# syzhang092218-source/dgppo

Measured on AMD Instinct MI355X. Metric: env-steps/sec whole node, LidarSpread n=8 4096 envs, 1/2/4/8 GPUs, higher is better.
Workload: dtype f32

## Files before the change

dgppo_amd/csrc/attn.hip:

```cpp
#include "nn_attn.h"

static int32_t attn_check(const dgppo_env_cfg* cfg, int F, int H, int Kp, int G, AttnArgs& a) {
  int32_t rc = dgppo_validate_cfg(cfg);
  if (rc) return rc;
  a.t = make_topo(*cfg);
  DGPPO_REQUIRE(F >= 1 && F <= 64 && H >= 1 && H <= 8, "attn: bad F=%d H=%d", F, H);
  DGPPO_REQUIRE(Kp >= F + H * (F + 4) + 1, "attn: Kp=%d too small", Kp);
  DGPPO_REQUIRE(G >= 0, "attn: G < 0");
  a.F = F; a.H = H; a.Kp = Kp; a.G = G;
  return 0;
}

enum class AttnFamily { SLOT8, BD, MFMA, VALU, TILED };
size_t attn_image_bytes(const Topo& t, int F, int H, bool bwd) {
  if (bwd)
    return sizeof(float) * ((size_t)t.Ns * (F + 1) + (size_t)t.n * H * (F + 1) + (size_t)t.n * t.S * 4 + 2 * (size_t)t.n * t.S * H +
                            (size_t)t.n * H * (F + 5));
  return sizeof(float) * ((size_t)t.Ns * (F + 1) + (size_t)t.n * H * (F + 1) + (size_t)t.n * t.S * 5 + (size_t)t.n * t.S * H);
}
static AttnFamily attn_family(const Topo& t, int F, int H, int Kp, bool bwd, bool dXa) {
  int PS = 0;
  bool hits = false;
  if (attn_image_bytes(t, F, H, bwd) > 64 * 1024) return AttnFamily::TILED;
  if ((Kp & 3) == 0 && attn_slot8_shape(t, F, H) && !(bwd && dXa)) return AttnFamily::SLOT8;
// ... 26 lines not shown
}
static void attn_set_bwd(AttnArgs& a, const float* dzcat, const float* attn, const float* qt, const float* Xa, const float* Xo,
                         const float* efeat, float* dqt, float* dXa, float* dXo) {
  a.dzcat = dzcat; a.attn = (float*)attn; a.qt = qt; a.Xa = Xa; a.Xo = Xo; a.efeat = efeat; a.dqt = dqt; a.dXa = dXa; a.dXo = dXo;
}

extern "C" int32_t dgppo_attn_fwd(const dgppo_env_cfg* cfg, int32_t F, int32_t H, int32_t Kp, const float* qt,
                                  const float* Xa, const float* Xo, const float* efeat, const float* emask, float* zcat,
                                  float* attn, int32_t G, void* stream) {
  AttnArgs a{};
  int32_t rc = attn_check(cfg, F, H, Kp, G, a);
  if (rc) return rc;
  if (G == 0) return 0;
  DGPPO_REQUIRE(qt && Xa && efeat && emask && zcat, "attn_fwd: NULL operand");
  DGPPO_REQUIRE(a.t.Ns == a.t.n || Xo, "attn_fwd: Xo is NULL");
  attn_set_fwd(a, qt, Xa, Xo, efeat, emask, zcat, attn);
  return attn_launch(attn_family(a.t, F, H, Kp, false, false), a, stream, false, "attn_fwd");
}

extern "C" int32_t dgppo_attn_bwd(const dgppo_env_cfg* cfg, int32_t F, int32_t H, int32_t Kp, const float* dzcat,
                                  const float* attn, const float* qt, const float* Xa, const float* Xo,
                                  const float* efeat, float* dqt, float* dXa, float* dXo, int32_t relu_xo, int32_t G,
                                  void* stream) {
  AttnArgs a{};
  int32_t rc = attn_check(cfg, F, H, Kp, G, a);
  if (rc) return rc;
  if (G == 0) return 0;
  DGPPO_REQUIRE(dzcat && attn && qt && Xa && efeat && dqt, "attn_bwd: NULL operand");
  DGPPO_REQUIRE(a.t.Ns == a.t.n || Xo, "attn_bwd: Xo is NULL");
  DGPPO_REQUIRE(!(dXo && !dXa), "attn_bwd: dXo needs dXa");
  attn_set_bwd(a, dzcat, attn, qt, Xa, Xo, efeat, dqt, dXa, dXo);
  const AttnFamily fam = attn_family(a.t, F, H, Kp, true, dXa != nullptr);
  a.relu_xo = (relu_xo && dXo && fam == AttnFamily::BD) ? 1 : 0;
  rc = attn_launch(fam, a, stream, true, "attn_bwd");
  if (rc) return rc;
  if (relu_xo && dXo && !a.relu_xo)
    return dgppo_relu_bwd(dXo, Xo, (int64_t)G * (a.t.Ns - a.t.n) * F, stream);
  return 0;
}

static bool attn_xo_ok(const Topo& t, int F, int H, int Kp) {
  return t.Ns > t.n && attn_family(t, F, H, Kp, true, true) == AttnFamily::BD;
}
extern "C" int32_t dgppo_attn_xo_supported(const dgppo_env_cfg* cfg, int32_t F, int32_t H, int32_t Kp) {
  AttnArgs a{};
  if (attn_check(cfg, F, H, Kp, 0, a)) return 0;
  return attn_xo_ok(a.t, F, H, Kp) ? 1 : 0;
}
static int32_t attn_set_xo(AttnArgs& a, const float* Xo_raw, const float* Wo, int ldwo, const float* bo, const char* who) {
  DGPPO_REQUIRE(attn_xo_ok(a.t, a.F, a.H, a.Kp), "%s: no fused kernel for this topology (ask dgppo_attn_xo_supported)", who);
  a.Xo_raw = Xo_raw; a.Wo = Wo; a.ldwo = ldwo; a.bo = bo;
  return 0;
}
extern "C" int32_t dgppo_attn_fwd_xo(const dgppo_env_cfg* cfg, int32_t F, int32_t H, int32_t Kp, const float* qt, const float* Xa,
                                     const float* Xo_raw, const float* Wo, int32_t ldwo, const float* bo, const float* efeat,
                                     const float* emask, float* zcat, float* attn, int32_t G, void* stream) {
  AttnArgs a{};
  int32_t rc = attn_check(cfg, F, H, Kp, G, a);
  if (rc) return rc;
  if (G == 0) return 0;
  DGPPO_REQUIRE(qt && Xa && Xo_raw && Wo && bo && efeat && emask && zcat, "attn_fwd_xo: NULL operand");
  DGPPO_REQUIRE(ldwo >= 32, "attn_fwd_xo: ldwo=%d < 32", ldwo);
  rc = attn_set_xo(a, Xo_raw, Wo, ldwo, bo, "attn_fwd_xo");
  if (rc) return rc;
  attn_set_fwd(a, qt, Xa, nullptr, efeat, emask, zcat, attn);
  return attn_launch(AttnFamily::BD, a, stream, false, "attn_fwd_xo");
}
extern "C" int32_t dgppo_attn_bwd_xo(const dgppo_env_cfg* cfg, int32_t F, int32_t H, int32_t Kp, const float* dzcat,
                                     const float* attn, const float* qt, const float* Xa, const float* Xo_raw, const float* Wo,
                                     int32_t ldwo, const float* bo, const float* efeat, float* dqt, float* dXa, float* dXo,
                                     int32_t relu_xo, int32_t G, void* stream) {
  AttnArgs a{};
  int32_t rc = attn_check(cfg, F, H, Kp, G, a);
  if (rc) return rc;
  if (G == 0) return 0;
  DGPPO_REQUIRE(dzcat && attn && qt && Xa && Xo_raw && Wo && bo && efeat && dqt, "attn_bwd_xo: NULL operand");
  DGPPO_REQUIRE(ldwo >= 32, "attn_bwd_xo: ldwo=%d < 32", ldwo);
  DGPPO_REQUIRE(!(dXo && !dXa), "attn_bwd_xo: dXo needs dXa");
  rc = attn_set_xo(a, Xo_raw, Wo, ldwo, bo, "attn_bwd_xo");
  if (rc) return rc;
  attn_set_bwd(a, dzcat, attn, qt, Xa, nullptr, efeat, dqt, dXa, dXo);
  a.relu_xo = (relu_xo && dXo) ? 1 : 0;
  return attn_launch(AttnFamily::BD, a, stream, true, "attn_bwd_xo");
}

static bool attn_rows_ok(const dgppo_env_cfg& c, const Topo& t, int F, int H, int Kp) {
  return attn_slot8_rows_ok(c, t, F, H) && attn_family(t, F, H, Kp, false, false) == AttnFamily::SLOT8 &&
         attn_family(t, F, H, Kp, true, false) == AttnFamily::SLOT8;
}
extern "C" int32_t dgppo_attn_rows_supported(const dgppo_env_cfg* cfg, int32_t F, int32_t H) {
  AttnArgs a{};
  const int Kp = (F + H * (F + 4) + 1 + 3) / 4 * 4;
  if (F < 1 || H < 1 || attn_check(cfg, F, H, Kp, 0, a)) return 0;
  return attn_rows_ok(*cfg, a.t, F, H, Kp) ? 1 : 0;
}
extern "C" int32_t dgppo_attn_fwd_rows(const dgppo_env_cfg* cfg, int32_t F, int32_t H, int32_t Kp, const float* qt,
                                       const float* Xa, const float* Xo, const float* emask, float* zcat, float* attn,
                                       int32_t G, void* stream) {
  AttnArgs a{};
  int32_t rc = attn_check(cfg, F, H, Kp, G, a);
  if (rc) return rc;
  DGPPO_REQUIRE(attn_rows_ok(*cfg, a.t, F, H, Kp), "attn_fwd_rows: no such kernel for this configuration (ask dgppo_attn_rows_supported)");
  if (G == 0) return 0;
  DGPPO_REQUIRE(qt && Xa && emask && zcat, "attn_fwd_rows: NULL operand");
  DGPPO_REQUIRE(a.t.Ns == a.t.n || Xo, "attn_fwd_rows: Xo is NULL");
  attn_set_fwd(a, qt, Xa, Xo, nullptr, emask, zcat, attn);
  return attn_launch(AttnFamily::SLOT8, a, stream, false, "attn_fwd_rows");
}
extern "C" int32_t dgppo_attn_bwd_rows(const dgppo_env_cfg* cfg, int32_t F, int32_t H, int32_t Kp, const float* dzcat,
                                       const float* attn, const float* qt, const float* emask, const float* Xa, const float* Xo,
                                       float* dqt, int32_t G, void* stream) {
  AttnArgs a{};
  int32_t rc = attn_check(cfg, F, H, Kp, G, a);
  if (rc) return rc;
  DGPPO_REQUIRE(attn_rows_ok(*cfg, a.t, F, H, Kp), "attn_bwd_rows: no such kernel for this configuration (ask dgppo_attn_rows_supported)");
  if (G == 0) return 0;
  DGPPO_REQUIRE(dzcat && Xa && dqt, "attn_bwd_rows: NULL operand");
  DGPPO_REQUIRE(attn || (qt && emask), "attn_bwd_rows: without attn the weights need qt and emask");
  DGPPO_REQUIRE(a.t.Ns == a.t.n || Xo, "attn_bwd_rows: Xo is NULL");
  attn_set_bwd(a, dzcat, attn, qt, Xa, Xo, nullptr, dqt, nullptr, nullptr);
  a.emask = emask;
  return attn_launch(AttnFamily::SLOT8, a, stream, true, "attn_bwd_rows");
}

extern "C" int64_t dgppo_attn_xo_workspace_bytes(int32_t G) { return G < 0 ? 0 : (int64_t)G * ABD_DW_STRIDE * (int64_t)sizeof(float); }
extern "C" int32_t dgppo_attn_bwd_xo_dw(const dgppo_env_cfg* cfg, int32_t F, int32_t H, int32_t Kp, const float* dzcat,
                                        const float* attn, const float* qt, const float* Xa, const float* Xo_raw, const float* Wo,
                                        int32_t ldwo, const float* bo, const float* efeat, float* dqt, float* dXa, float* dWo,
                                        int32_t lddwo, float* dbo, float* workspace, int64_t workspace_bytes, int32_t G,
                                        void* stream) {
  AttnArgs a{};
  int32_t rc = attn_check(cfg, F, H, Kp, G, a);
  if (rc) return rc;
  if (G == 0) return 0;
  DGPPO_REQUIRE(dzcat && attn && qt && Xa && Xo_raw && Wo && bo && efeat && dqt && dXa && dWo && dbo && workspace,
                "attn_bwd_xo_dw: NULL operand");
  DGPPO_REQUIRE(ldwo >= 32 && lddwo >= 32, "attn_bwd_xo_dw: ldwo=%d lddwo=%d < 32", ldwo, lddwo);
  DGPPO_REQUIRE(workspace_bytes >= dgppo_attn_xo_workspace_bytes(G) && (reinterpret_cast<uintptr_t>(workspace) & 15) == 0,
                "attn_bwd_xo_dw: workspace too small or not 16-byte aligned");
  rc = attn_set_xo(a, Xo_raw, Wo, ldwo, bo, "attn_bwd_xo_dw");
  if (rc) return rc;
  attn_set_bwd(a, dzcat, attn, qt, Xa, nullptr, efeat, dqt, dXa, nullptr);
  a.relu_xo = 1;
  a.dwo_slab = workspace;
  const bool launched = launch_attn_bd(a, (hipStream_t)stream, true);
  DGPPO_REQUIRE(launched, "attn_bwd_xo_dw: dispatch failed");
  launch_attn_xo_dw_reduce(workspace, G, dWo, lddwo, dbo, (hipStream_t)stream);
  DGPPO_LAUNCH_CHECK();
  return 0;
}
```

dgppo_amd/csrc/attn_bd.hip:

```cpp
#include "nn_attn.h"

#ifdef DGPPO_STAMPS
__device__ unsigned long long g_astamps[32];
#define ASTAMP(i) do { if (blockIdx.x == 0 && threadIdx.x == 0) g_astamps[i] = __builtin_amdgcn_s_memtime(); } while (0)
extern "C" int32_t dgppo_debug_stamps_attn(unsigned long long* out) {
  return (int32_t)hipMemcpyFromSymbol(out, HIP_SYMBOL(g_astamps), sizeof(unsigned long long) * 32);
}
#else
#define ASTAMP(i)
#endif

#define ABD_XL 36
#define ABD_DZL 40
__device__ inline f32x4g mfma4(float a_, float b_, f32x4g c_) { return __builtin_amdgcn_mfma_f32_4x4x1f32(a_, b_, c_, 0, 0, 0); }
__device__ inline const float* f4e(const float4& v) { return reinterpret_cast<const float*>(&v); }

__device__ inline int opaque_zero(int bits) {
  asm("v_and_b32 %0, 0, %0" : "+v"(bits));
  return bits;
}
__device__ inline int f4bits(const float4& v) { return __float_as_int(v.x) | __float_as_int(v.y) | __float_as_int(v.z) | __float_as_int(v.w); }

template <int PS, bool HITS> struct AbdLds {
  static constexpr int NSP = PS * 8, PC = NSP + (HITS ? 8 : 0), PL = PC + 4;
// ... 44 lines not shown
      v[ct] = __builtin_amdgcn_mfma_f32_16x16x4f32(ar[0], x.wo[0][ct], v[ct], 0, 0, 0);
      v[ct] = __builtin_amdgcn_mfma_f32_16x16x4f32(ar[1], x.wo[1][ct], v[ct], 0, 0, 0);
    }
  };
  if (first) {
#pragma unroll
    for (int t = 0; t < GT; ++t) {
      f32x4g v[2];
      tile(x.ag[t], v);
#pragma unroll
      for (int ct = 0; ct < 2; ++ct)
#pragma unroll
        for (int r = 0; r < 4; ++r) {
          const int o = t * 16 + lq * 4 + r;
          if (o < n_shared_other) XS[(n + o) * ABD_XL + ct * 16 + li] = relu_nan(v[ct][r] + x.bo[ct]);
        }
    }
  }
  if constexpr (HITS) {
#pragma unroll
    for (int t = 0; t < 4; ++t) {
      f32x4g v[2];
      tile(x.ah[t], v);
#pragma unroll
      for (int ct = 0; ct < 2; ++ct)
#pragma unroll
        for (int r = 0; r < 4; ++r) {
          const int hr = t * 16 + lq * 4 + r;
          XH[hr * ABD_XL + (hr >> 3) * 8 + ct * 16 + li] = relu_nan(v[ct][r] + x.bo[ct]);
        }
    }
  }
}
template <int GT> __device__ inline int abd_xo_bits(const AbdXoRegs<GT>& x, bool hits) {
  int b = 0;
#pragma unroll
  for (int t = 0; t < GT; ++t) b |= __float_as_int(x.ag[t][0]) | __float_as_int(x.ag[t][1]);
  if (hits) {
#pragma unroll
    for (int t = 0; t < 4; ++t) b |= __float_as_int(x.ah[t][0]) | __float_as_int(x.ah[t][1]);
  }
  b |= __float_as_int(x.wo[0][0]) | __float_as_int(x.wo[0][1]) | __float_as_int(x.wo[1][0]) | __float_as_int(x.wo[1][1]);
  b |= __float_as_int(x.bo[0]) | __float_as_int(x.bo[1]);
  return b;
}

template <int PS, bool HITS>
__device__ __forceinline__ int abd_slot(const Topo& t, int NSH, int ic, int p, int sub) {
  if (HITS && p == PS) return t.n + t.gs + sub;
  const int j = p * 8 + sub;
  return (j < NSH) ? slot_of(t, j, ic) : -1;
}

template <int PS, bool HITS, int AB, bool XOF>
__global__ void __launch_bounds__(128) attn_fwd_bd_kernel(AttnArgs a) {
  extern __shared__ float4 abd_sm[];
  using L = AbdLds<PS, HITS>;
  constexpr int F = 32, NSP = L::NSP, PC = L::PC, PL = L::PL, NPR = PS + (HITS ? 1 : 0), Wd = F + 4;
  const Topo& t = a.t;
  const int lane = threadIdx.x & 63, wave = threadIdx.x >> 6;
  const int g = __builtin_amdgcn_readfirstlane(blockIdx.x * 2 + wave);
  if (g >= a.G) return;
  const int n = t.n, S = t.S, Ns = t.Ns, H = a.H, Kp = a.Kp;
  const int NSH = HITS ? t.n + t.ng : Ns;
  const int kc = F + H * Wd;
  float* XS = reinterpret_cast<float*>(abd_sm) + wave * L::FWD;
  float* XH = XS + L::XS;
  float* QP = XH + L::XH;
  const float4* Xa4 = reinterpret_cast<const float4*>(a.Xa + (size_t)g * n * F);
  const float4* Xo4 = reinterpret_cast<const float4*>(a.Xo + (size_t)g * (Ns - n) * F);
  const float4* qt4 = reinterpret_cast<const float4*>(a.qt + (size_t)g * n * H * F);
  float* zc = a.zcat + (size_t)g * n * Kp;
  const int il = lane >> 3, sub = lane & 7, g2 = (lane >> 2) & 1, c = lane & 3, hA = lane & 3;
  ASTAMP(0);
  float4 vs[PS];
#pragma unroll
  for (int p = 0; p < PS; ++p) {
    const int row = p * 8 + il;
    const int ra = row < n ? row : n - 1, ro = (row < NSH ? row : NSH - 1) - n;
    const float4* src = (XOF || row < n || NSH == n) ? Xa4 + ra * 8 + sub : Xo4 + ro * 8 + sub;
    vs[p] = *src;
  }
  constexpr int GT = (NSP + 15) / 16;
  AbdXoRegs<GT> xo;
  const float* raw = XOF ? a.Xo_raw + (size_t)g * (Ns - n) * ABD_KR : nullptr;
  const int li_ = lane & 15, lq_ = lane >> 4;
  const float* mk = a.emask + (size_t)g * n * S;
  const float4* ef4 = reinterpret_cast<const float4*>(a.efeat + (size_t)g * n * S * 4);
  float* at = a.attn + (size_t)g * n * S * H;
#pragma unroll
  for (int ab = 0; ab < AB; ++ab) {
    const int i = ab * 8 + il;
    const bool live = i < n;
    const int ic = live ? i : n - 1;
    float4 vh[HITS ? 8 : 1], vq[4];
    if constexpr (XOF) abd_xo_load<GT, HITS>(xo, a, raw, NSH - n, t.ng, ab * 64, n * 8, li_, lq_, ab == 0);
    if constexpr (HITS && !XOF) {
#pragma unroll
      for (int k = 0; k < 8; ++k) {
        int hb = ab * 64 + k * 8 + il;
        hb = hb < n * 8 ? hb : n * 8 - 1;
        vh[k] = Xo4[(t.ng + hb) * 8 + sub];
      }
    }
#pragma unroll
    for (int k = 0; k < 4; ++k) {
      const int row = k * 8 + il;
      int ri = ab * 8 + (row >> 2), rh = row & 3;
      ri = ri < n ? ri : n - 1; rh = rh < H ? rh : H - 1;
      vq[k] = qt4[(ri * H + rh) * 8 + sub];
    }
    int slot[NPR];
    float mkv[NPR];
    float4 efv[NPR];
#pragma unroll
    for (int p = 0; p < NPR; ++p) {
      const int sl = abd_slot<PS, HITS>(t, NSH, ic, p, sub);
      slot[p] = live ? sl : -1;
      const int sc = sl < 0 ? 0 : sl;
      mkv[p] = mk[ic * S + sc];
      efv[p] = ef4[ic * S + sc];
    }
    ASTAMP(1);
    int pin = 0;
#pragma unroll
    for (int p = 0; p < NPR; ++p) pin |= __float_as_int(mkv[p]) | f4bits(efv[p]);
    if constexpr (XOF) pin |= abd_xo_bits<GT>(xo, HITS);
    const int pin0 = opaque_zero(pin);
    if (ab == 0) {
#pragma unroll
      for (int p = 0; p < PS; ++p) {
        float4 v = vs[p];
        if (XOF && p * 8 + il >= n) v = make_float4(0.f, 0.f, 0.f, 0.f);
        *reinterpret_cast<float4*>(XS + pin0 + (p * 8 + il) * ABD_XL + sub * 4) = v;
      }
    }
    if constexpr (XOF) abd_xo_emit<GT, HITS>(xo, XS + pin0, XH + pin0, n, NSH - n, li_, lq_, ab == 0);
    if constexpr (HITS && !XOF) {
#pragma unroll
      for (int k = 0; k < 8; ++k) *reinterpret_cast<float4*>(XH + pin0 + (k * 8 + il) * ABD_XL + k * 8 + sub * 4) = vh[k];
    }
#pragma unroll
    for (int k = 0; k < 4; ++k) *reinterpret_cast<float4*>(QP + pin0 + (k * 8 + il) * ABD_XL + sub * 4) = vq[k];
#pragma unroll
    for (int p = 0; p < NPR; ++p) mkv[p] = (slot[p] >= 0) ? mkv[p] : 0.0f;
    if constexpr (HITS) {
      if (mkv[PS] == 0.0f) {
#pragma unroll
        for (int k = 0; k < 8; ++k) *reinterpret_cast<float4*>(XH + lane * ABD_XL + il * 8 + k * 4) = make_float4(0.f, 0.f, 0.f, 0.f);
      }
    }
    ASTAMP(2);
    f32x4g acc[NPR];
#pragma unroll
    for (int p = 0; p < NPR; ++p) acc[p] = f32x4g{0.f, 0.f, 0.f, 0.f};
    {
      const float* qrow = QP + (il * 4 + hA) * ABD_XL;
#pragma unroll
      for (int k = 0; k < 8; ++k) {
        const float4 q = *reinterpret_cast<const float4*>(qrow + k * 4);
        float4 x[NPR];
#pragma unroll
        for (int p = 0; p < NPR; ++p) {
          if (HITS && p == PS) x[p] = *reinterpret_cast<const float4*>(XH + lane * ABD_XL + il * 8 + k * 4);
          else x[p] = *reinterpret_cast<const float4*>(XS + (p * 8 + sub) * ABD_XL + k * 4);
        }
#pragma unroll
        for (int u = 0; u < 4; ++u)
#pragma unroll
          for (int p = 0; p < NPR; ++p) acc[p] = mfma4(f4e(q)[u], f4e(x[p])[u], acc[p]);
      }
    }
    ASTAMP(3);
    float* PT = QP;
#pragma unroll
    for (int h = 0; h < 4; ++h) {
      if (h < H) {
        float l[NPR];
        float mx = -INFINITY;
#pragma unroll
        for (int p = 0; p < NPR; ++p) { l[p] = (mkv[p] != 0.0f) ? acc[p][h] : -INFINITY; mx = fmaxf(mx, l[p]); }
// ... 22 lines not shown
#pragma unroll
        for (int p = 0; p < NPR; ++p) acc[p][h] = 0.0f;
      }
#pragma unroll
      for (int p = 0; p < NPR; ++p) PT[(il * 4 + h) * PL + p * 8 + sub] = acc[p][h];
    }
    ASTAMP(4);
    {
      float pa[PC];
#pragma unroll
      for (int k = 0; k < PC / 4; ++k) {
        const float4 v = *reinterpret_cast<const float4*>(PT + (il * 4 + hA) * PL + k * 4);
        pa[k * 4] = v.x; pa[k * 4 + 1] = v.y; pa[k * 4 + 2] = v.z; pa[k * 4 + 3] = v.w;
      }
      f32x4g az[4];
#pragma unroll
      for (int q = 0; q < 4; ++q) az[q] = f32x4g{0.f, 0.f, 0.f, 0.f};
      const int fq = (g2 * 4 + c) * 4;
#pragma unroll
      for (int kk = 0; kk < NSP; ++kk) {
        const float4 b = *reinterpret_cast<const float4*>(XS + kk * ABD_XL + fq);
#pragma unroll
        for (int q = 0; q < 4; ++q) az[q] = mfma4(pa[kk], f4e(b)[q], az[q]);
      }
      if constexpr (HITS) {
#pragma unroll
        for (int m = 0; m < 8; ++m) {
          const float4 b = *reinterpret_cast<const float4*>(XH + (il * 8 + m) * ABD_XL + il * 8 + fq);
#pragma unroll
          for (int q = 0; q < 4; ++q) az[q] = mfma4(pa[NSP + m], f4e(b)[q], az[q]);
        }
      }
      if (live) {
#pragma unroll
        for (int h = 0; h < 4; ++h)
          if (h < H) *reinterpret_cast<float4*>(zc + i * Kp + F + h * Wd + fq) = make_float4(az[0][h], az[1][h], az[2][h], az[3][h]);
      }
    }
  }
  ASTAMP(5);
#pragma unroll
  for (int p = 0; p < PS; ++p) {
    const int row = p * 8 + il;
    if (row < n) *reinterpret_cast<float4*>(zc + row * Kp + sub * 4) = *reinterpret_cast<const float4*>(XS + row * ABD_XL + sub * 4);
  }
  {
    const int wpad = Kp - kc;
    for (int i = lane; i < n; i += 64)
      for (int cc = 0; cc < wpad; ++cc) zc[i * Kp + kc + cc] = (cc == 0) ? ones_col(a.t, mk + i * S) : 0.0f;
  }
  ASTAMP(6);
}

template <int PS, bool HITS, bool XOF>
struct AbdFwdRegs {
  float4 vs[PS], vq[4], vh[(HITS && !XOF) ? 8 : 1];
  AbdXoRegs<(PS * 8 + 15) / 16> xo;
  float mkv[PS + (HITS ? 1 : 0)];
  float4 efv[PS + (HITS ? 1 : 0)];
};
template <int PS, bool HITS, bool XOF>
__global__ void __launch_bounds__(128) attn_fwd_bdp_kernel(AttnArgs a) {
  extern __shared__ float4 abd_sm[];
  using L = AbdLds<PS, HITS>;
  constexpr int F = 32, NSP = L::NSP, PC = L::PC, PL = L::PL, NPR = PS + (HITS ? 1 : 0), Wd = F + 4, GT = (NSP + 15) / 16;
  const Topo& t = a.t;
  const int lane = threadIdx.x & 63, wave = threadIdx.x >> 6;
  int g = __builtin_amdgcn_readfirstlane(blockIdx.x * 2 + wave);
  const int stride = gridDim.x * 2;
  if (g >= a.G) return;
  const int n = t.n, S = t.S, Ns = t.Ns, H = a.H, Kp = a.Kp;
  const int NSH = HITS ? t.n + t.ng : Ns;
  const int kc = F + H * Wd;
  float* XS = reinterpret_cast<float*>(abd_sm) + wave * L::FWD;
  float* XH = XS + L::XS;
  float* QP = XH + L::XH;
  const int il = lane >> 3, sub = lane & 7, g2 = (lane >> 2) & 1, c = lane & 3, hA = lane & 3;
  const int li_ = lane & 15, lq_ = lane >> 4;
  const int i = il;
  const bool live = i < n;
  const int ic = live ? i : n - 1;
  int slot[NPR], sc[NPR];
#pragma unroll
  for (int p = 0; p < NPR; ++p) {
    const int sl = abd_slot<PS, HITS>(t, NSH, ic, p, sub);
    slot[p] = live ? sl : -1;
    sc[p] = sl < 0 ? 0 : sl;
  }
  using Regs = AbdFwdRegs<PS, HITS, XOF>;
  auto load = [&](int gg, Regs& R) {
    const float4* Xa4 = reinterpret_cast<const float4*>(a.Xa + (size_t)gg * n * F);
    const float4* Xo4 = reinterpret_cast<const float4*>(a.Xo + (size_t)gg * (Ns - n) * F);
    const float4* qt4 = reinterpret_cast<const float4*>(a.qt + (size_t)gg * n * H * F);
#pragma unroll
    for (int p = 0; p < PS; ++p) {
      const int row = p * 8 + il;
      const int ra = row < n ? row : n - 1, ro = (row < NSH ? row : NSH - 1) - n;
      const float4* src = (XOF || row < n || NSH == n) ? Xa4 + ra * 8 + sub : Xo4 + ro * 8 + sub;
      R.vs[p] = *src;
    }
    if constexpr (XOF) abd_xo_load<GT, HITS>(R.xo, a, a.Xo_raw + (size_t)gg * (Ns - n) * ABD_KR, NSH - n, t.ng, 0, n * 8, li_, lq_, true);
    if constexpr (HITS && !XOF) {
#pragma unroll
      for (int k = 0; k < 8; ++k) {
        int hb = k * 8 + il;
        hb = hb < n * 8 ? hb : n * 8 - 1;
        R.vh[k] = Xo4[(t.ng + hb) * 8 + sub];
      }
    }
#pragma unroll
    for (int k = 0; k < 4; ++k) {
      const int row = k * 8 + il;
      int ri = row >> 2, rh = row & 3;
      ri = ri < n ? ri : n - 1; rh = rh < H ? rh : H - 1;
      R.vq[k] = qt4[(ri * H + rh) * 8 + sub];
    }
    const float* mk = a.emask + (size_t)gg * n * S;
    const float4* ef4 = reinterpret_cast<const float4*>(a.efeat + (size_t)gg * n * S * 4);
#pragma unroll
    for (int p = 0; p < NPR; ++p) {
      R.mkv[p] = mk[ic * S + sc[p]];
      R.efv[p] = ef4[ic * S + sc[p]];
    }
  };
  auto stage = [&](Regs& R) {
    int pin = 0;
#pragma unroll
    for (int p = 0; p < NPR; ++p) pin |= __float_as_int(R.mkv[p]) | f4bits(R.efv[p]);
    if constexpr (XOF) pin |= abd_xo_bits<GT>(R.xo, HITS);
    const int pin0 = opaque_zero(pin);
#pragma unroll
    for (int p = 0; p < PS; ++p) {
      float4 v = R.vs[p];
      if (XOF && p * 8 + il >= n) v = make_float4(0.f, 0.f, 0.f, 0.f);
      *reinterpret_cast<float4*>(XS + pin0 + (p * 8 + il) * ABD_XL + sub * 4) = v;
    }
    if constexpr (XOF) abd_xo_emit<GT, HITS>(R.xo, XS + pin0, XH + pin0, n, NSH - n, li_, lq_, true);
    if constexpr (HITS && !XOF) {
#pragma unroll
      for (int k = 0; k < 8; ++k) *reinterpret_cast<float4*>(XH + pin0 + (k * 8 + il) * ABD_XL + k * 8 + sub * 4) = R.vh[k];
    }
#pragma unroll
    for (int k = 0; k < 4; ++k) *reinterpret_cast<float4*>(QP + pin0 + (k * 8 + il) * ABD_XL + sub * 4) = R.vq[k];
#pragma unroll
    for (int p = 0; p < NPR; ++p) R.mkv[p] = (slot[p] >= 0) ? R.mkv[p] : 0.0f;
    if constexpr (HITS) {
      if (R.mkv[PS] == 0.0f) {
#pragma unroll
        for (int k = 0; k < 8; ++k) *reinterpret_cast<float4*>(XH + lane * ABD_XL + il * 8 + k * 4) = make_float4(0.f, 0.f, 0.f, 0.f);
      }
    }
  };
  auto compute = [&](int gg, const Regs& R) {
    float* zc = a.zcat + (size_t)gg * n * Kp;
    float* at = a.attn + (size_t)gg * n * S * H;
    f32x4g acc[NPR];
#pragma unroll
    for (int p = 0; p < NPR; ++p) acc[p] = f32x4g{0.f, 0.f, 0.f, 0.f};
    {
      const float* qrow = QP + (il * 4 + hA) * ABD_XL;
#pragma unroll
      for (int k = 0; k < 8; ++k) {
        const float4 q = *reinterpret_cast<const float4*>(qrow + k * 4);
        float4 x[NPR];
#pragma unroll
        for (int p = 0; p < NPR; ++p) {
          if (HITS && p == PS) x[p] = *reinterpret_cast<const float4*>(XH + lane * ABD_XL + il * 8 + k * 4);
          else x[p] = *reinterpret_cast<const float4*>(XS + (p * 8 + sub) * ABD_XL + k * 4);
        }
#pragma unroll
        for (int u = 0; u < 4; ++u)
#pragma unroll
          for (int p = 0; p < NPR; ++p) acc[p] = mfma4(f4e(q)[u], f4e(x[p])[u], acc[p]);
      }
    }
    float* PT = QP;
#pragma unroll
    for (int h = 0; h < 4; ++h) {
      if (h < H) {
        float l[NPR];
        float mx = -INFINITY;
#pragma unroll
        for (int p = 0; p < NPR; ++p) { l[p] = (R.mkv[p] != 0.0f) ? acc[p][h] : -INFINITY; mx = fmaxf(mx, l[p]); }
// ... 32 lines not shown
        const float4 v = *reinterpret_cast<const float4*>(PT + (il * 4 + hA) * PL + k * 4);
        pa[k * 4] = v.x; pa[k * 4 + 1] = v.y; pa[k * 4 + 2] = v.z; pa[k * 4 + 3] = v.w;
      }
      f32x4g az[4];
#pragma unroll
      for (int q = 0; q < 4; ++q) az[q] = f32x4g{0.f, 0.f, 0.f, 0.f};
      const int fq = (g2 * 4 + c) * 4;
#pragma unroll
      for (int kk = 0; kk < NSP; ++kk) {
        const float4 b = *reinterpret_cast<const float4*>(XS + kk * ABD_XL + fq);
#pragma unroll
        for (int q = 0; q < 4; ++q) az[q] = mfma4(pa[kk], f4e(b)[q], az[q]);
      }
      if constexpr (HITS) {
#pragma unroll
        for (int m = 0; m < 8; ++m) {
          const float4 b = *reinterpret_cast<const float4*>(XH + (il * 8 + m) * ABD_XL + il * 8 + fq);
#pragma unroll
          for (int q = 0; q < 4; ++q) az[q] = mfma4(pa[NSP + m], f4e(b)[q], az[q]);
        }
      }
      if (live) {
#pragma unroll
        for (int h = 0; h < 4; ++h)
          if (h < H) *reinterpret_cast<float4*>(zc + i * Kp + F + h * Wd + fq) = make_float4(az[0][h], az[1][h], az[2][h], az[3][h]);
      }
    }
#pragma unroll
    for (int p = 0; p < PS; ++p) {
      const int row = p * 8 + il;
      if (row < n) *reinterpret_cast<float4*>(zc + row * Kp + sub * 4) = *reinterpret_cast<const float4*>(XS + row * ABD_XL + sub * 4);
    }
    {
      const int wpad = Kp - kc;
      for (int ii = lane; ii < n; ii += 64)
        for (int cc = 0; cc < wpad; ++cc) zc[ii * Kp + kc + cc] = (cc == 0) ? ones_col(a.t, a.emask + ((size_t)gg * n + ii) * a.t.S) : 0.0f;
    }
  };
  Regs cur;
  load(g, cur);
  for (;;) {
    stage(cur);
    const int gn = g + stride;
    const bool more = gn < a.G;
    Regs nxt;
    if (more) load(gn, nxt);
    compute(g, cur);
    if (!more) break;
    cur = nxt;
    g = gn;
  }
}

template <int PS, bool HITS, int AB, bool XOF>
__global__ void __launch_bounds__(64) attn_bwd_bd_kernel(AttnArgs a) {
  extern __shared__ float4 abd_sm[];
  using L = AbdLds<PS, HITS>;
  constexpr int F = 32, NSP = L::NSP, PC = L::PC, PL = L::PL, PTL = L::PTL, NPR = PS + (HITS ? 1 : 0), Wd = F + 4;
  constexpr int RTS = (NSP + 15) / 16;
  const Topo& t = a.t;
  const int lane = threadIdx.x & 63;
  const int g = blockIdx.x;
  if (g >= a.G) return;
  const int n = t.n, S = t.S, Ns = t.Ns, H = a.H, Kp = a.Kp;
  const int NSH = HITS ? t.n + t.ng : Ns;
  float* XS = reinterpret_cast<float*>(abd_sm);
  float* XH = XS + L::XS;
  float* DZ = XH + L::XH;
  float* PT = DZ + L::DZ;
  float* DL = PT + L::PT;
  const float4* Xa4 = reinterpret_cast<const float4*>(a.Xa + (size_t)g * n * F);
  const float4* Xo4 = reinterpret_cast<const float4*>(a.Xo + (size_t)g * (Ns - n) * F);
  const float* qt = a.qt + (size_t)g * n * H * F;
  const float* dzc = a.dzcat + (size_t)g * n * Kp;
  const bool want_dx = a.dXa != nullptr;
  const int il = lane >> 3, sub = lane & 7, g2 = (lane >> 2) & 1, c = lane & 3, hA = lane & 3;
  const int li = lane & 15, lq = lane >> 4;
  float4 vs[PS];
#pragma unroll
  for (int p = 0; p < PS; ++p) {
    const int row = p * 8 + il;
    const int ra = row < n ? row : n - 1, ro = (row < NSH ? row : NSH - 1) - n;
    const float4* src = (XOF || row < n || NSH == n) ? Xa4 + ra * 8 + sub : Xo4 + ro * 8 + sub;
    vs[p] = *src;
  }
  constexpr int GT = (NSP + 15) / 16;
  AbdXoRegs<GT> xo;
  const float* raw = XOF ? a.Xo_raw + (size_t)g * (Ns - n) * ABD_KR : nullptr;
  const int li_ = lane & 15, lq_ = lane >> 4;
  float dir[RTS][2][4];
#pragma unroll
  for (int rt = 0; rt < RTS; ++rt)
#pragma unroll
    for (int ft = 0; ft < 2; ++ft)
#pragma unroll
      for (int r = 0; r < 4; ++r) {
        const int node = rt * 16 + lq * 4 + r;
        dir[rt][ft][r] = dzc[(node < n ? node : n - 1) * Kp + ft * 16 + li];
      }
  f32x4g dxs[RTS][2];
#pragma unroll
  for (int rt = 0; rt < RTS; ++rt)
#pragma unroll
    for (int ft = 0; ft < 2; ++ft) dxs[rt][ft] = f32x4g{0.f, 0.f, 0.f, 0.f};
  f32x4g dwacc[2] = {f32x4g{0.f, 0.f, 0.f, 0.f}, f32x4g{0.f, 0.f, 0.f, 0.f}};
  float rbg[NSP / 4];
  const float4* ef4 = reinterpret_cast<const float4*>(a.efeat + (size_t)g * n * S * 4);
  const float* at = a.attn + (size_t)g * n * S * H;
#pragma unroll
  for (int ab = 0; ab < AB; ++ab) {
    const int i = ab * 8 + il;
    const bool live = i < n;
    const int ic = live ? i : n - 1;
    float4 vh[HITS ? 8 : 1], vz[5];
    if constexpr (XOF) abd_xo_load<GT, HITS>(xo, a, raw, NSH - n, t.ng, ab * 64, n * 8, li_, lq_, ab == 0);
    float rbh[HITS ? 16 : 1];
    if constexpr (XOF && HITS) {
#pragma unroll
      for (int s_ = 0; s_ < 16; ++s_) {
        int hb = ab * 64 + s_ * 4 + lq;
        hb = hb < n * 8 ? hb : n * 8 - 1;
        rbh[s_] = raw[(t.ng + hb) * ABD_KR + (li & 7)];
      }
    }
    if constexpr (XOF) {
      if (ab == 0) {
#pragma unroll
        for (int s_ = 0; s_ < NSP / 4; ++s_) {
          int o = s_ * 4 + lq;
          o = o < NSH - n ? o : NSH - n - 1;
          o = o < 0 ? 0 : o;
          rbg[s_] = raw[o * ABD_KR + (li & 7)];
        }
      }
    }
    if constexpr (HITS && !XOF) {
#pragma unroll
      for (int k = 0; k < 8; ++k) {
        int hb = ab * 64 + k * 8 + il;
        hb = hb < n * 8 ? hb : n * 8 - 1;
        vh[k] = Xo4[(t.ng + hb) * 8 + sub];
      }
    }
#pragma unroll
    for (int k = 0; k < 5; ++k) {
      int tt = k * 64 + lane;
      tt = tt < 288 ? tt : 287;
      const int row = tt / 9, ch = tt - row * 9;
      int ri = ab * 8 + (row >> 2), rh = row & 3;
      ri = ri < n ? ri : n - 1; rh = rh < H ? rh : H - 1;
      vz[k] = *reinterpret_cast<const float4*>(dzc + ri * Kp + F + rh * Wd + ch * 4);
    }
    int slot[NPR];
    float4 efv[NPR];
    float av[NPR][4];
#pragma unroll
    for (int p = 0; p < NPR; ++p) {
      const int sl = abd_slot<PS, HITS>(t, NSH, ic, p, sub);
      slot[p] = live ? sl : -1;
      const int sc = sl < 0 ? 0 : sl;
      efv[p] = ef4[ic * S + sc];
#pragma unroll
      for (int h = 0; h < 4; ++h) av[p][h] = at[(ic * S + sc) * H + (h < H ? h : H - 1)];
    }
    float4 q8[4][2];
    if constexpr (HITS) {
#pragma unroll
      for (int h = 0; h < 4; ++h) {
        const float4* qr = reinterpret_cast<const float4*>(qt + (size_t)(ic * H + (h < H ? h : H - 1)) * F + c * 8);
        q8[h][0] = qr[0]; q8[h][1] = qr[1];
      }
    }
    float bQ[8][2];
#pragma unroll
    for (int ks = 0; ks < 8; ++ks) {
      const int ri = ab * 8 + ks;
      const float* qr = qt + (size_t)((ri < n ? ri : n - 1) * H + (lq < H ? lq : H - 1)) * F;
#pragma unroll
      for (int ft = 0; ft < 2; ++ft) bQ[ks][ft] = qr[ft * 16 + li];
    }
    int pin = 0;
#pragma unroll
    for (int p = 0; p < NPR; ++p) {
      pin |= f4bits(efv[p]);
#pragma unroll
      for (int h = 0; h < 4; ++h) pin |= __float_as_int(av[p][h]);
    }
    if constexpr (HITS) {
#pragma unroll
      for (int h = 0; h < 4; ++h) pin |= f4bits(q8[h][0]) | f4bits(q8[h][1]);
    }
#pragma unroll
    for (int ks = 0; ks < 8; ++ks) pin |= __float_as_int(bQ[ks][0]) | __float_as_int(bQ[ks][1]);
    if (ab == 0) {
#pragma unroll
      for (int rt = 0; rt < RTS; ++rt)
#pragma unroll
        for (int ft = 0; ft < 2; ++ft)
#pragma unroll
          for (int r = 0; r < 4; ++r) pin |= __float_as_int(dir[rt][ft][r]);
    }
    if constexpr (XOF) pin |= abd_xo_bits<GT>(xo, HITS);
    if constexpr (XOF && HITS) {
#pragma unroll
      for (int s_ = 0; s_ < 16; ++s_) pin |= __float_as_int(rbh[s_]);
    }
    if constexpr (XOF) {
      if (ab == 0) {
#pragma unroll
        for (int s_ = 0; s_ < NSP / 4; ++s_) pin |= __float_as_int(rbg[s_]);
      }
    }
    const int pin0 = opaque_zero(pin);
    if (ab == 0) {
#pragma unroll
      for (int p = 0; p < PS; ++p) {
        float4 v = vs[p];
        if (XOF && p * 8 + il >= n) v = make_float4(0.f, 0.f, 0.f, 0.f);
        *reinterpret_cast<float4*>(XS + pin0 + (p * 8 + il) * ABD_XL + sub * 4) = v;
      }
    }
    if constexpr (XOF) abd_xo_emit<GT, HITS>(xo, XS + pin0, XH + pin0, n, NSH - n, li_, lq_, ab == 0);
    if constexpr (HITS && !XOF) {
#pragma unroll
      for (int k = 0; k < 8; ++k) *reinterpret_cast<float4*>(XH + pin0 + (k * 8 + il) * ABD_XL + k * 8 + sub * 4) = vh[k];
    }
#pragma unroll
    for (int k = 0; k < 5; ++k) {
      const int tt = k * 64 + lane, row = tt / 9, ch = tt - row * 9;
      if (tt < 288) *reinterpret_cast<float4*>(DZ + pin0 + row * ABD_DZL + ch * 4) = vz[k];
    }
#pragma unroll
    for (int p = 0; p < NPR; ++p)
#pragma unroll
      for (int h = 0; h < 4; ++h) av[p][h] = (slot[p] >= 0 && h < H) ? av[p][h] : 0.0f;
    if constexpr (HITS) {
      if (av[PS][0] == 0.0f && av[PS][1] == 0.0f && av[PS][2] == 0.0f && av[PS][3] == 0.0f) {
#pragma unroll
        for (int k = 0; k < 8; ++k) *reinterpret_cast<float4*>(XH + lane * ABD_XL + il * 8 + k * 4) = make_float4(0.f, 0.f, 0.f, 0.f);
      }
    }
    f32x4g acc[NPR];
#pragma unroll
    for (int p = 0; p < NPR; ++p) acc[p] = f32x4g{0.f, 0.f, 0.f, 0.f};
    {
      const float* zrow = DZ + (il * 4 + hA) * ABD_DZL;
#pragma unroll
      for (int k = 0; k < 8; ++k) {
        const float4 q = *reinterpret_cast<const float4*>(zrow + k * 4);
        float4 x[NPR];
#pragma unroll
        for (int p = 0; p < NPR; ++p) {
          if (HITS && p == PS) x[p] = *reinterpret_cast<const float4*>(XH + lane * ABD_XL + il * 8 + k * 4);
          else x[p] = *reinterpret_cast<const float4*>(XS + (p * 8 + sub) * ABD_XL + k * 4);
        }
#pragma unroll
        for (int u = 0; u < 4; ++u)
#pragma unroll
          for (int p = 0; p < NPR; ++p) acc[p] = mfma4(f4e(q)[u], f4e(x[p])[u], acc[p]);
      }
    }
#pragma unroll
    for (int h = 0; h < 4; ++h) {
      const float4 dze = *reinterpret_cast<const float4*>(DZ + (il * 4 + h) * ABD_DZL + F);
      float dot = 0.0f;
#pragma unroll
// ... 136 lines not shown
          const int node = rt * 16 + lq * 4 + r;
          xm[rt][ft][r] = (node < NSP) ? XS[node * ABD_XL + ft * 16 + li] : 0.0f;
        }
#pragma unroll
    for (int rt = 0; rt < RTS; ++rt)
#pragma unroll
      for (int ft = 0; ft < 2; ++ft)
#pragma unroll
        for (int r = 0; r < 4; ++r) {
          const int node = rt * 16 + lq * 4 + r, f = ft * 16 + li;
          float v = dxs[rt][ft][r];
          if (node < n) a.dXa[((size_t)g * n + node) * F + f] = v + dir[rt][ft][r];
          else if (XOF && a.dwo_slab != nullptr) {
            if (node < NSP) XS[node * ABD_XL + f] = (node < NSH && xm[rt][ft][r] > 0.0f) ? v : 0.0f;
          } else if (node < NSH && a.dXo != nullptr) {
            if (a.relu_xo) v = (xm[rt][ft][r] > 0.0f) ? v : 0.0f;
            a.dXo[((size_t)g * (Ns - n) + (node - n)) * F + f] = v;
          }
        }
    if constexpr (XOF) {
      if (a.dwo_slab != nullptr) {
        const int nsho = NSH - n;
#pragma unroll
        for (int s_ = 0; s_ < NSP / 4; ++s_) {
          const int o = s_ * 4 + lq;
          const float bv = li < 8 ? rbg[s_] : (li == 8 ? 1.0f : 0.0f);
#pragma unroll
          for (int ft = 0; ft < 2; ++ft) {
            const int node = n + o;
            const float av_ = (o < nsho && node < NSP) ? XS[(node < NSP ? node : NSP - 1) * ABD_XL + ft * 16 + li] : 0.0f;
            dwacc[ft] = __builtin_amdgcn_mfma_f32_16x16x4f32(av_, bv, dwacc[ft], 0, 0, 0);
          }
        }
        if (li <= 8) {
          float* o = a.dwo_slab + (size_t)g * ABD_DW_STRIDE + li * 32 + lq * 4;
#pragma unroll
          for (int ft = 0; ft < 2; ++ft)
            *reinterpret_cast<float4*>(o + ft * 16) = make_float4(dwacc[ft][0], dwacc[ft][1], dwacc[ft][2], dwacc[ft][3]);
        }
      }
    }
  }
}

bool attn_bd_shape(const Topo& t, int F, int H, int& PS, bool& hits) {
  if (F != 32 || H < 1 || H > 4 || t.n > 16) return false;
  const int n_priv = t.Ns - t.n - t.ng;
  hits = t.lidar && n_priv > 0;
  if (hits && (t.per != 8 || n_priv != t.n * 8)) return false;
  const int nsh = hits ? t.n + t.ng : t.Ns;
  PS = (nsh + 7) / 8;
  return PS >= 1 && PS <= 4;
}
template <int PS, bool HITS, int AB, bool XOF>
static void launch_attn_bd_x(const AttnArgs& a, hipStream_t s, bool bwd) {
  using L = AbdLds<PS, HITS>;
  if (bwd) { hipLaunchKernelGGL((attn_bwd_bd_kernel<PS, HITS, AB, XOF>), dim3(a.G), dim3(64), sizeof(float) * L::BWD, s, a); return; }
  if constexpr (AB == 1) {
    static thread_local int cap = 0;
    if (cap == 0) {
      int per_cu = 0, dev = 0, cus = 256;
      if (hipOccupancyMaxActiveBlocksPerMultiprocessor(&per_cu, reinterpret_cast<const void*>(&attn_fwd_bdp_kernel<PS, HITS, XOF>), 128,
                                                       sizeof(float) * 2 * L::FWD) != hipSuccess || per_cu < 1) per_cu = 1;
      if (hipGetDevice(&dev) != hipSuccess || hipDeviceGetAttribute(&cus, hipDeviceAttributeMultiprocessorCount, dev) != hipSuccess ||
          cus < 1) cus = 256;
      cap = per_cu * cus;
    }
    if ((a.G + 1) / 2 > 2 * cap) {
      hipLaunchKernelGGL((attn_fwd_bdp_kernel<PS, HITS, XOF>), dim3(cap), dim3(128), sizeof(float) * 2 * L::FWD, s, a);
      return;
    }
  }
  hipLaunchKernelGGL((attn_fwd_bd_kernel<PS, HITS, AB, XOF>), dim3((a.G + 1) / 2), dim3(128), sizeof(float) * 2 * L::FWD, s, a);
}
template <int PS, bool HITS, int AB>
static void launch_attn_bd_one(const AttnArgs& a, hipStream_t s, bool bwd) {
  if (a.Xo_raw != nullptr) launch_attn_bd_x<PS, HITS, AB, true>(a, s, bwd);
  else launch_attn_bd_x<PS, HITS, AB, false>(a, s, bwd);
}
bool launch_attn_bd(const AttnArgs& a, hipStream_t s, bool bwd) {
  int PS = 0;
  bool hits = false;
  if (!attn_bd_shape(a.t, a.F, a.H, PS, hits)) return false;
  const int AB = (a.t.n + 7) / 8;
  switch ((PS * 2 + (hits ? 1 : 0)) * 4 + AB) {
#define DGPPO_BD(P, HT, B) case ((P) * 2 + (HT)) * 4 + (B): launch_attn_bd_one<P, (HT) != 0, B>(a, s, bwd); return true;
    DGPPO_BD(1, 0, 1) DGPPO_BD(1, 1, 1) DGPPO_BD(2, 0, 1) DGPPO_BD(2, 1, 1) DGPPO_BD(2, 0, 2) DGPPO_BD(2, 1, 2)
    DGPPO_BD(3, 0, 1) DGPPO_BD(3, 1, 1) DGPPO_BD(3, 0, 2) DGPPO_BD(3, 1, 2)
    DGPPO_BD(4, 0, 1) DGPPO_BD(4, 1, 1) DGPPO_BD(4, 0, 2) DGPPO_BD(4, 1, 2)
#undef DGPPO_BD
    default: return false;
  }
}

__global__ void __launch_bounds__(320) attn_xo_dw_reduce_kernel(const float* slab, int G, float* dWo, int lddwo, float* dbo) {
  const int e = threadIdx.x;
  if (e >= 288) return;
  const int per = (G + gridDim.x - 1) / gridDim.x;
  const int g0 = blockIdx.x * per, g1 = min(G, g0 + per);
  float sacc[8] = {0.f, 0.f, 0.f, 0.f, 0.f, 0.f, 0.f, 0.f};
  int g = g0;
  for (; g + 7 < g1; g += 8) {
#pragma unroll
    for (int u = 0; u < 8; ++u) sacc[u] += slab[(size_t)(g + u) * ABD_DW_STRIDE + e];
  }
  for (; g < g1; ++g) sacc[0] += slab[(size_t)g * ABD_DW_STRIDE + e];
  const float sum = ((sacc[0] + sacc[1]) + (sacc[2] + sacc[3])) + ((sacc[4] + sacc[5]) + (sacc[6] + sacc[7]));
  if (g0 >= g1) return;
  if (e < 256) atomicAdd(dWo + (size_t)(e >> 5) * lddwo + (e & 31), sum);
  else atomicAdd(dbo + (e - 256), sum);
}
void launch_attn_xo_dw_reduce(const float* slab, int G, float* dWo, int lddwo, float* dbo, hipStream_t s) {
  int blocks = (G + 31) / 32;
  blocks = blocks < 1 ? 1 : (blocks > 1024 ? 1024 : blocks);
  hipLaunchKernelGGL(attn_xo_dw_reduce_kernel, dim3(blocks), dim3(320), 0, s, slab, G, dWo, lddwo, dbo);
}
```

dgppo_amd/csrc/attn_slot8.hip:

```cpp
#include "nn_attn.h"


template <int SJ>
__device__ inline void slot8_weights(const float4 (&q)[2], const float4 (&x)[SJ][2], const bool (&ok)[SJ], float (&w)[SJ]) {
#pragma clang fp contract(off)
  float mx = -INFINITY;
#pragma unroll
  for (int j = 0; j < SJ; ++j) {
    float acc = q[0].x * x[j][0].x;
    acc = fmaf(q[0].y, x[j][0].y, acc); acc = fmaf(q[0].z, x[j][0].z, acc); acc = fmaf(q[0].w, x[j][0].w, acc);
    acc = fmaf(q[1].x, x[j][1].x, acc); acc = fmaf(q[1].y, x[j][1].y, acc);
    acc = fmaf(q[1].z, x[j][1].z, acc); acc = fmaf(q[1].w, x[j][1].w, acc);
    w[j] = ok[j] ? acc : -INFINITY;
    mx = fmaxf(mx, w[j]);
  }
  mx = grp8_max(mx);
  float den = 0.0f;
#pragma unroll
  for (int j = 0; j < SJ; ++j) {
    const float ev = (w[j] == -INFINITY) ? 0.0f : __expf(w[j] - mx);
    w[j] = ev;
    den += ev;
  }
  den = grp8_sum(den);
  const float inv = (den > 0.0f) ? 1.0f / den : 0.0f;
#pragma unroll
  for (int j = 0; j < SJ; ++j) w[j] *= inv;
}
__device__ inline float4 slot8_edge(const Topo& t, int sl, float4 xi, float4 xs) {
  const bool hit = t.lidar && sl >= t.n + t.gs;
  return make_float4(__fsub_rn(xi.x, xs.x), __fsub_rn(xi.y, xs.y), hit ? 0.0f : __fsub_rn(xi.z, xs.z), hit ? 0.0f : __fsub_rn(xi.w, xs.w));
}

template <int H, int NPA, int SJ, bool ROWS>
__global__ void __launch_bounds__(256) attn_fwd_slot8_kernel(AttnArgs a) {
  constexpr int F = 8, Wd = F + 4;
  const Topo& t = a.t;
  const int lane = threadIdx.x & 63, wave = threadIdx.x >> 6, sub = lane & 7, grp = lane >> 3;
  const int g = __builtin_amdgcn_readfirstlane(blockIdx.x * 4 + wave);
  if (g >= a.G) return;
  const int n = t.n, S = t.S, Ns = t.Ns, Kp = a.Kp, kc = F + H * Wd;
  const float* Xa = a.Xa + (size_t)g * n * F;
  const float* Xo = a.Xo + (size_t)g * (Ns - n) * F - (size_t)n * F;
  const float* qt = a.qt + (size_t)g * n * H * F;
  const float* ef = ROWS ? nullptr : a.efeat + (size_t)g * n * S * 4;
  const float* mk = a.emask + (size_t)g * n * S;
  float* zc = a.zcat + (size_t)g * n * Kp;
  float* at = a.attn + (size_t)g * n * S * H;
  for (int idx = lane; idx < n * 2; idx += 64)
    *reinterpret_cast<float4*>(zc + (idx >> 1) * Kp + 4 * (idx & 1)) = reinterpret_cast<const float4*>(Xa)[idx];
  for (int i = lane; i < n; i += 64)
    for (int c = kc; c < Kp; ++c) zc[i * Kp + c] = (c == kc) ? ones_col(a.t, mk + i * S) : 0.0f;
#pragma unroll
  for (int p = 0; p < NPA; ++p) {
    const int ia = grp + 8 * p;
    const bool live = ia < n;
    const int i = live ? ia : n - 1;
    float4 q[H][2], x[SJ][2], e[SJ];
    float m[SJ];
    bool ok[SJ];
#pragma unroll
    for (int h = 0; h < H; ++h) {
      const float4* qp = reinterpret_cast<const float4*>(qt + (i * H + h) * F);
      q[h][0] = qp[0]; q[h][1] = qp[1];
    }
    float4 xi;
    if constexpr (ROWS) xi = *reinterpret_cast<const float4*>(Xa + i * F);
#pragma unroll
    for (int j = 0; j < SJ; ++j) {
      int sl = sub + 8 * j;
      sl = sl < S ? sl : S - 1;
      const int nd = sender_node(t, i, sl);
      const float4* xp = reinterpret_cast<const float4*>((nd < n ? Xa : Xo) + (size_t)nd * F);
      x[j][0] = xp[0]; x[j][1] = xp[1];
      if constexpr (ROWS) e[j] = slot8_edge(t, sl, xi, x[j][0]);
      else e[j] = reinterpret_cast<const float4*>(ef)[i * S + sl];
      m[j] = mk[i * S + sl];
    }
#pragma unroll
    for (int j = 0; j < SJ; ++j) ok[j] = live && (sub + 8 * j) < S && m[j] != 0.0f;
    float av[H][SJ];
#pragma unroll
    for (int h = 0; h < H; ++h) slot8_weights<SJ>(q[h], x, ok, av[h]);
#pragma unroll
    for (int j = 0; j < SJ; ++j) {
      const int sl = sub + 8 * j;
      if (live && sl < S) {
#pragma unroll
        for (int h = 0; h < H; ++h) if (a.attn != nullptr) at[(i * S + sl) * H + h] = av[h][j];
      }
    }
#pragma unroll
    for (int h = 0; h < H; ++h) {
      float z[Wd];
#pragma unroll
      for (int c = 0; c < Wd; ++c) z[c] = 0.0f;
#pragma unroll
      for (int j = 0; j < SJ; ++j) {
        const float w = av[h][j];
        if (w != 0.0f) {
          z[0] = fmaf(w, x[j][0].x, z[0]); z[1] = fmaf(w, x[j][0].y, z[1]); z[2] = fmaf(w, x[j][0].z, z[2]); z[3] = fmaf(w, x[j][0].w, z[3]);
          z[4] = fmaf(w, x[j][1].x, z[4]); z[5] = fmaf(w, x[j][1].y, z[5]); z[6] = fmaf(w, x[j][1].z, z[6]); z[7] = fmaf(w, x[j][1].w, z[7]);
          z[8] = fmaf(w, e[j].x, z[8]); z[9] = fmaf(w, e[j].y, z[9]); z[10] = fmaf(w, e[j].z, z[10]); z[11] = fmaf(w, e[j].w, z[11]);
        }
      }
#pragma unroll
      for (int c = 0; c < Wd; ++c) z[c] = grp8_sum(z[c]);
      if (live && sub == h) {
        float4* o = reinterpret_cast<float4*>(zc + i * Kp + F + h * Wd);
        o[0] = make_float4(z[0], z[1], z[2], z[3]);
        o[1] = make_float4(z[4], z[5], z[6], z[7]);
        o[2] = make_float4(z[8], z[9], z[10], z[11]);
      }
    }
  }
}

template <int H, int NPA, int SJ, bool ROWS, bool RECOMP>
__global__ void __launch_bounds__(256) attn_bwd_slot8_kernel(AttnArgs a) {
  constexpr int F = 8, Wd = F + 4;
  const Topo& t = a.t;
  const int lane = threadIdx.x & 63, wave = threadIdx.x >> 6, sub = lane & 7, grp = lane >> 3;
  const int g = __builtin_amdgcn_readfirstlane(blockIdx.x * 4 + wave);
  if (g >= a.G) return;
  const int n = t.n, S = t.S, Ns = t.Ns, Kp = a.Kp;
  const float* Xa = a.Xa + (size_t)g * n * F;
  const float* Xo = a.Xo + (size_t)g * (Ns - n) * F - (size_t)n * F;
  const float* ef = ROWS ? nullptr : a.efeat + (size_t)g * n * S * 4;
  const float* at = RECOMP ? nullptr : a.attn + (size_t)g * n * S * H;
  const float* qt = RECOMP ? a.qt + (size_t)g * n * H * F : nullptr;
  const float* mk = RECOMP ? a.emask + (size_t)g * n * S : nullptr;
  const float* dzc = a.dzcat + (size_t)g * n * Kp;
  float* dq = a.dqt + (size_t)g * n * H * F;
#pragma unroll
  for (int p = 0; p < NPA; ++p) {
    const int ia = grp + 8 * p;
    const bool live = ia < n;
    const int i = live ? ia : n - 1;
    float4 dz[H][3], x[SJ][2], e[SJ];
    float av[H][SJ];
    float m[SJ];
    float4 xi;
    if constexpr (ROWS) xi = *reinterpret_cast<const float4*>(Xa + i * F);
#pragma unroll
    for (int j = 0; j < SJ; ++j) {
      int sl = sub + 8 * j;
      const bool in = live && sl < S;
      sl = sl < S ? sl : S - 1;
      const int nd = sender_node(t, i, sl);
      const float4* xp = reinterpret_cast<const float4*>((nd < n ? Xa : Xo) + (size_t)nd * F);
      x[j][0] = xp[0]; x[j][1] = xp[1];
      if constexpr (ROWS) e[j] = slot8_edge(t, sl, xi, x[j][0]);
      else e[j] = reinterpret_cast<const float4*>(ef)[i * S + sl];
      if constexpr (RECOMP) {
        m[j] = mk[i * S + sl];
      } else {
#pragma unroll
        for (int h = 0; h < H; ++h) {
          const float w = at[(i * S + sl) * H + h];
          av[h][j] = in ? w : 0.0f;
        }
      }
    }
    if constexpr (RECOMP) {
      bool ok[SJ];
#pragma unroll
      for (int j = 0; j < SJ; ++j) ok[j] = live && (sub + 8 * j) < S && m[j] != 0.0f;
#pragma unroll
      for (int h = 0; h < H; ++h) {
        float4 q[2];
        const float4* qp = reinterpret_cast<const float4*>(qt + (i * H + h) * F);
        q[0] = qp[0]; q[1] = qp[1];
        slot8_weights<SJ>(q, x, ok, av[h]);
      }
      __builtin_amdgcn_sched_barrier(0);
    }
#pragma unroll
    for (int h = 0; h < H; ++h) {
      const float4* zp = reinterpret_cast<const float4*>(dzc + i * Kp + F + h * Wd);
      dz[h][0] = zp[0]; dz[h][1] = zp[1]; dz[h][2] = zp[2];
    }
#pragma unroll
    for (int h = 0; h < H; ++h) {
      float dA[SJ];
      float dot = 0.0f;
#pragma unroll
      for (int j = 0; j < SJ; ++j) {
        float acc = 0.0f;
        if (av[h][j] != 0.0f) {
          acc = dz[h][0].x * x[j][0].x;
          acc = fmaf(dz[h][0].y, x[j][0].y, acc); acc = fmaf(dz[h][0].z, x[j][0].z, acc); acc = fmaf(dz[h][0].w, x[j][0].w, acc);
          acc = fmaf(dz[h][1].x, x[j][1].x, acc); acc = fmaf(dz[h][1].y, x[j][1].y, acc);
          acc = fmaf(dz[h][1].z, x[j][1].z, acc); acc = fmaf(dz[h][1].w, x[j][1].w, acc);
          acc = fmaf(dz[h][2].x, e[j].x, acc); acc = fmaf(dz[h][2].y, e[j].y, acc);
          acc = fmaf(dz[h][2].z, e[j].z, acc); acc = fmaf(dz[h][2].w, e[j].w, acc);
          dot = fmaf(av[h][j], acc, dot);
        }
        dA[j] = acc;
      }
      dot = grp8_sum(dot);
      float o[F];
#pragma unroll
      for (int c = 0; c < F; ++c) o[c] = 0.0f;
#pragma unroll
      for (int j = 0; j < SJ; ++j) {
// ... 51 lines not shown
```

dgppo_amd/csrc/env_step.hip:

```cpp
#include "env_step.h"

template <int SD>
__global__ void env_step_kernel(StepArgs a) {
  extern __shared__ float smem[];
  const dgppo_env_cfg& c = a.cfg;
  const int b = blockIdx.x;
  const int tid = threadIdx.x, nt = blockDim.x;
  const int n = c.n_agents, ng = c.n_goals, no = c.n_obs, R = c.n_rays, k = c.top_k;
  const bool lidar = cfg_is_lidar(c), spread = cfg_is_spread(c);
  const int ostride = lidar ? DGPPO_RECT_STRIDE : SD;
  const int n_on = cfg_obs_nodes(c);
  const int kk = lidar ? (no > 0 ? k : 0) : 0;
  constexpr int ND = SD + 3;

  float* s_seg = smem;
  float* s_agent = s_seg + (lidar ? no * 16 : 0);
  float* s_next = s_agent + n * SD;
  float* s_goal = s_next + n * SD;
  float* s_act = s_goal + ng * SD;
  float* s_obst = s_act + n * 2;
  float* s_hpre = s_obst + no * ostride;
  float* s_hnext = s_hpre + n * kk * 2;
  float* s_alpha = s_hnext + n * kk * 2;
  float* s_fa = s_alpha + (lidar ? n * R : 0);
// ... 666 lines not shown
    }
    case FAMILY_GENERIC: {
      int work = cfg->n_agents * (lidar ? cfg->n_rays : 1);
      const int E = cfg_num_edges(*cfg);
      if (gout && E > work) work = E;
      int threads = ((work + 63) / 64) * 64;
      if (threads < 64) threads = 64;
      if (threads > 512) threads = 512;
      if (cfg->state_dim == 5) hipLaunchKernelGGL(env_step_kernel<5>, dim3(B), dim3(threads), smem, s, a);
      else hipLaunchKernelGGL(env_step_kernel<4>, dim3(B), dim3(threads), smem, s, a);
      break;
    }
  }
  DGPPO_LAUNCH_CHECK();
  return 0;
}

extern "C" int32_t dgppo_env_step(const dgppo_env_cfg* cfg, const float* agent, const float* action, const float* goal,
                                  const float* obst, const float* hits, const float* ray_cos, const float* ray_sin,
                                  float* next_agent, float* next_hits, float* reward, float* cost,
                                  const dgppo_graph_out* gout, int32_t B, void* stream) {
  if (!cfg) { dgppo_set_error("cfg is NULL"); return -1; }
  const int mode = action ? MODE_STEP : MODE_SENSE;
  return launch_step(cfg, mode, agent, action, goal, obst, hits, ray_cos, ray_sin, next_agent, next_hits, reward, cost,
                     gout, B, stream);
}

static bool act_step_ok(const dgppo_env_cfg& c, int Fp, int H) {
  const bool lidar32 = cfg_is_lidar(c) && cfg_is_base_kind(c) && c.n_obs > 0 && c.n_rays == 32;
  return lidar32 && c.top_k == 8 && c.eye_offset >= c.comm_radius && c.node_dim <= 8 && Fp == 8 && H == 3 && lidar_wave_has_act_instance(c);
}

extern "C" int32_t dgppo_env_act_step_feats_supported(const dgppo_env_cfg* cfg, int32_t Fp, int32_t H) {
  if (!cfg || dgppo_validate_cfg(cfg) != 0 || cfg_is_vmas(*cfg)) return 0;
  return act_step_ok(*cfg, Fp, H) ? 1 : 0;
}

extern "C" int32_t dgppo_env_act_step_feats(const dgppo_env_cfg* cfg, const float* agent, const float* goal, const float* obst,
                                            const float* hits, const float* ray_cos, const float* ray_sin, const float* ms,
                                            const float* eps, int32_t sample, float* action, float* log_pi, float* next_agent,
                                            float* next_hits, float* reward, float* cost, float* Xa, float* Xo, float* efeat,
                                            float* emask, int32_t Fp, const float* Mcat, const float* cvec, float* qt0, int32_t H,
                                            int32_t max_blocks, int32_t B, void* stream) {
  if (!cfg) { dgppo_set_error("cfg is NULL"); return -1; }
  int32_t rc = dgppo_validate_cfg(cfg);
  if (rc) return rc;
  DGPPO_REFUSE_VMAS(cfg, "dgppo_env_act_step_feats", "dgppo_vmas_step");
  DGPPO_REQUIRE(act_step_ok(*cfg, Fp, H), "env_act_step_feats: no kernel for this configuration, Fp=%d, H=%d (ask dgppo_env_act_step_feats_supported)", Fp, H);
  DGPPO_REQUIRE(B >= 0 && max_blocks >= 0, "env_act_step_feats: B and max_blocks must be >= 0 (got %d, %d)", B, max_blocks);
  if (B == 0) return 0;
  DGPPO_REQUIRE(agent && goal && obst && hits && ray_cos && ray_sin, "env_act_step_feats: NULL state operand");
  DGPPO_REQUIRE(ms && action && next_agent && next_hits && reward && cost, "env_act_step_feats: NULL operand");
  DGPPO_REQUIRE(!sample || (eps && log_pi), "env_act_step_feats(sample): eps and log_pi must not be NULL");
  DGPPO_REQUIRE(!Xa || (Xo && efeat && emask), "env_act_step_feats: Xa needs Xo, efeat and emask");
  DGPPO_REQUIRE(!qt0 || (Mcat && cvec), "env_act_step_feats: qt0 needs Mcat and cvec");
  auto al16 = [](const void* p) { return (((uintptr_t)p) & 15) == 0; };
  DGPPO_REQUIRE(al16(agent) && al16(goal) && al16(obst) && al16(hits) && al16(next_agent) && al16(next_hits),
                "env_act_step_feats: the record operands must be 16-byte aligned");
  DGPPO_REQUIRE(al16(Xa) && al16(Xo) && al16(efeat) && al16(emask) && al16(qt0),
                "env_act_step_feats: Xa, Xo, efeat, emask and qt0 must be 16-byte aligned");
  DGPPO_REQUIRE((((uintptr_t)ms | (uintptr_t)eps | (uintptr_t)action | (uintptr_t)log_pi | (uintptr_t)Mcat | (uintptr_t)cvec) & 3) == 0,
                "env_act_step_feats: operands must be 4-byte aligned");
  StepArgs a;
  a.cfg = *cfg;
  a.agent = agent; a.action = nullptr; a.goal = goal; a.obst = obst; a.hits = hits;
  a.ray_cos = ray_cos; a.ray_sin = ray_sin;
  a.next_agent = next_agent; a.next_hits = next_hits; a.reward = reward; a.cost = cost;
  a.has_graph = 0;
  a.g = dgppo_graph_out{};
  a.mode = MODE_STEP;
  a.B = B;
  a.rcp_n = fdiv_rcp(cfg->n_agents); a.rcp_k = fdiv_rcp(cfg->top_k); a.rcp_no = fdiv_rcp(cfg->n_obs);
  a.rcp_no4 = fdiv_rcp(4 * cfg->n_obs);
  a.thr2_comm = sqrt_threshold(cfg->comm_radius);
  a.thr2_lidar = sqrt_threshold(cfg->lidar_mask_radius);
  ActFeatArgs f;
  f.ms = ms; f.eps = eps; f.action = action; f.log_pi = log_pi; f.sample = sample ? 1 : 0;
  f.Xa = Xa; f.Xo = Xo; f.efeat = efeat; f.emask = emask; f.Mcat = Mcat; f.cvec = cvec; f.qt0 = qt0; f.max_blocks = max_blocks;
  launch_lidar_wave_act(a, f, (hipStream_t)stream);
  DGPPO_LAUNCH_CHECK();
  return 0;
}

extern "C" int32_t dgppo_graph_materialize(const dgppo_env_cfg* cfg, const float* agent, const float* goal,
                                           const float* obst, const float* hits, const dgppo_graph_out* gout, int32_t B,
                                           void* stream) {
  if (!cfg) { dgppo_set_error("cfg is NULL"); return -1; }
  return launch_step(cfg, MODE_GRAPH, agent, nullptr, goal, obst, hits, nullptr, nullptr, nullptr, nullptr, nullptr, nullptr,
                     gout, B, stream);
}
```

dgppo_amd/csrc/env_wave.hip:

```cpp
#include "env_step.h"
#include "nn_head.h"
#include <type_traits>

#ifndef DGPPO_WAVE_WPE
#define DGPPO_WAVE_WPE 5
#endif
#ifndef DGPPO_WAVE_WPE_COMPACT
#define DGPPO_WAVE_WPE_COMPACT 6
#endif
#ifndef DGPPO_WAVE_UNROLL_O
#define DGPPO_WAVE_UNROLL_O 8
#endif
#ifndef DGPPO_WAVE_UNROLL_P3
#define DGPPO_WAVE_UNROLL_P3 1
#endif
#define DGPPO_PRAGMA_(x) _Pragma(#x)
#define DGPPO_PRAGMA(x) DGPPO_PRAGMA_(x)

namespace {

#define WSYNC() asm volatile("" ::: "memory")
#ifdef DGPPO_STAMPS
__device__ unsigned long long g_wstamps[64];
__device__ unsigned long long g_wspan[3 * 8192];
// ... 783 lines not shown
        const int node = 2 * NA + q;
        if (has_graph) { L.nodes[node * ND] = hx; L.nodes[node * ND + 1] = hy; }
      }
    }
    WSYNC();
    PHASE("P4_compact", 7);
    if (a.next_hits != nullptr) {
      float4* o4 = reinterpret_cast<float4*>(a.next_hits + (size_t)b * NA * K * 2);
      for (int i = lane; i < NA * K * 2 / 4; i += 64) o4[i] = reinterpret_cast<const float4*>(L.hits)[i];
    }
    if constexpr (FUSE) {
      if (f.Xa != nullptr) {
#pragma unroll
        for (int q0 = 0; q0 < 2 * NA * K; q0 += 64) {
          const int q = q0 + lane;
          if (q < 2 * NA * K) {
            const int h = q >> 1, col0 = (q & 1) * 4;
            float v[4];
#pragma unroll
            for (int k = 0; k < 4; ++k) {
              const int col = col0 + k;
              v[k] = (col < 2) ? L.hits[h * 2 + (col < 2 ? col : 0)] : ((col == SD) ? 1.0f : 0.0f);
            }
            *reinterpret_cast<float4*>(f.Xo + ((size_t)b * (NA + NA * K) + NA + h) * ACT_FP + col0) = make_float4(v[0], v[1], v[2], v[3]);
          }
        }
        constexpr int S = NA + GS + K, NE = NA * S;
        static_assert(NE % 4 == 0, "masks leave as float4");
#pragma unroll
        for (int base = 0; base < NE; base += 64) {
          const int idx = base + lane;
          bool mask = false;
          if (idx < NE) {
            const int i = idx / S, s = idx - i * S;
            const float4 fi = reinterpret_cast<const float4*>(fa_ptr)[i];
            const float px = L.next[i * SD], py = L.next[i * SD + 1];
            float4 e;
            if (s < NA) {
              const float4 fj = reinterpret_cast<const float4*>(fa_ptr)[s];
              e = make_float4(fi.x - fj.x, fi.y - fj.y, fi.z - fj.z, fi.w - fj.w);
              const float dx = px - L.next[s * SD], dy = py - L.next[s * SD + 1];
              mask = (i != s) && (dx * dx + dy * dy < a.thr2_comm);
            } else if (s < NA + GS) {
              const int gi = SPREAD ? (s - NA) : i;
              const float4 fg = reinterpret_cast<const float4*>(fg_ptr)[gi];
              e = make_float4(fi.x - fg.x, fi.y - fg.y, fi.z - fg.z, fi.w - fg.w);
              mask = true;
            } else {
              const int m = s - NA - GS;
              const float lx = px - L.hits[(i * K + m) * 2], ly = py - L.hits[(i * K + m) * 2 + 1];
              e = make_float4(lx, ly, 0.0f, 0.0f);
              mask = lx * lx + ly * ly < a.thr2_lidar;
            }
            reinterpret_cast<float4*>(f.efeat)[(size_t)b * NE + idx] = e;
          }
          const unsigned long long bits = __builtin_amdgcn_ballot_w64(mask);
          const int i4 = base + 4 * lane;
          if (lane < 16 && i4 < NE) {
            const unsigned mb = (unsigned)(bits >> (4 * lane));
            *reinterpret_cast<float4*>(f.emask + (size_t)b * NE + i4) =
                make_float4((mb & 1u) ? 1.0f : 0.0f, (mb & 2u) ? 1.0f : 0.0f, (mb & 4u) ? 1.0f : 0.0f, (mb & 8u) ? 1.0f : 0.0f);
          }
        }
      }
      WSYNC();
    }
    if (!has_graph) continue;
    PHASE("P5_graph", 8);
    {
      float4* edges = reinterpret_cast<float4*>(a.g.edges) + (size_t)b * E;
      int32_t* recv = a.g.receivers + (size_t)b * E;
      int32_t* send = a.g.senders + (size_t)b * E;
#pragma unroll
      for (int q0 = 0; q0 < NA * K; q0 += 64) {
        const int q = q0 + lane;
        if (q < NA * K) {
          const int i = q / K;
          const float lx = L.next[i * SD] - L.hits[q * 2], ly = L.next[i * SD + 1] - L.hits[q * 2 + 1];
          const bool mask = lx * lx + ly * ly < a.thr2_lidar;
          edges[NA * NA + NA * GS + q] = make_float4(lx, ly, 0.0f, 0.0f);
          recv[NA * NA + NA * GS + q] = mask ? i : PAD;
          send[NA * NA + NA * GS + q] = mask ? 2 * NA + q : PAD;
        }
      }
      float* nodes = a.g.nodes + (size_t)b * N * ND;
#pragma unroll
      for (int q0 = 0; q0 < N * ND; q0 += 64) {
        const int q = q0 + lane;
        if (q < N * ND) nodes[q] = L.nodes[q];
      }
      if constexpr (SD == 4) {
        float4* st4 = reinterpret_cast<float4*>(a.g.states + (size_t)b * N * SD);
#pragma unroll
        for (int q0 = 0; q0 < N; q0 += 64) {
          const int node = q0 + lane;
          if (node < N) {
            const float* row = L.nodes + node * ND;
            st4[node] = (node == PAD) ? make_float4(-1.0f, -1.0f, -1.0f, -1.0f) : make_float4(row[0], row[1], row[2], row[3]);
          }
        }
      } else {
        float* st = a.g.states + (size_t)b * N * SD;
#pragma unroll
        for (int q0 = 0; q0 < N * SD; q0 += 64) {
          const int q = q0 + lane;
          if (q < N * SD) {
            const int node = q / SD, d = q - node * SD;
// ... 123 lines not shown
```

dgppo_amd/csrc/graph_feats.hip:

```cpp
#include "graph_topo.h"

struct FeatArgs {
  dgppo_env_cfg cfg;
  Topo t;
  const float* agent; long agent_se, agent_st;
  const float* goal;
  const float* obst;
  const float* hits; long hits_se, hits_st;
  const int32_t* env_ids;
  int n_env, n_time;
  float* Xa;
  float* Xo;
  float* efeat;
  float* emask;
  int Fp;
  int vecX, vecM;
  uint32_t rcp_fp, rcp_fq, rcp_S;
};

#define GF_PF 8
#define GF_WAVE_SYNC()                                  \
  do {                                                  \
    __builtin_amdgcn_fence(__ATOMIC_SEQ_CST, "wavefront"); \
    __builtin_amdgcn_wave_barrier();                    \
// ... 72 lines not shown
        node_src(nd, src, ns, one);
        float v[4];
#pragma unroll
        for (int k = 0; k < 4; ++k) {
          const int col = col0 + k;
          v[k] = (col < ns) ? src[col] : ((col == one) ? 1.0f : 0.0f);
        }
        float* dst = (nd < n) ? a.Xa + ((size_t)g * n + nd) * Fp + col0 : a.Xo + ((size_t)g * (t.Ns - n) + (nd - n)) * Fp + col0;
        *reinterpret_cast<float4*>(dst) = make_float4(v[0], v[1], v[2], v[3]);
      }
    } else {
      for (int idx = lane; idx < t.Ns * Fp; idx += 64) {
        const int nd = (int)__umulhi((uint32_t)idx, a.rcp_fp), col = idx - nd * Fp;
        const float* src; int ns, one;
        node_src(nd, src, ns, one);
        const float v = (col < ns) ? src[col] : ((col == one) ? 1.0f : 0.0f);
        if (nd < n) a.Xa[((size_t)g * n + nd) * Fp + col] = v;
        else a.Xo[((size_t)g * (t.Ns - n) + (nd - n)) * Fp + col] = v;
      }
    }
    const int nE = n * S;
    for (int base = 0; base < nE; base += 64) {
      const int idx = base + lane;
      bool mask = false;
      if (idx < nE) {
        const int i = (int)__umulhi((uint32_t)idx, a.rcp_S), s = idx - i * S;
        float4 f;
        const float4 fi = feat4<SD>(s_ag + i * SD);
        const float px = s_ag[i * SD], py = s_ag[i * SD + 1];
        if (s < n) {
          const float4 fj = feat4<SD>(s_ag + s * SD);
          f = make_float4(__fsub_rn(fi.x, fj.x), __fsub_rn(fi.y, fj.y), __fsub_rn(fi.z, fj.z), __fsub_rn(fi.w, fj.w));
          float d = __fadd_rn(dist_rn(__fsub_rn(px, s_ag[s * SD]), __fsub_rn(py, s_ag[s * SD + 1])), (i == s) ? c.eye_offset : 0.0f);
          mask = d < c.comm_radius;
        } else if (s < n + t.gs) {
          const int gi = t.spread ? (s - n) : i;
          const float4 fg = feat4<SD>(s_go + gi * SD);
          f = make_float4(__fsub_rn(fi.x, fg.x), __fsub_rn(fi.y, fg.y), __fsub_rn(fi.z, fg.z), __fsub_rn(fi.w, fg.w));
          mask = true;
        } else {
          const int m = s - n - t.gs;
          if (t.lidar) {
            const float* hp = s_ob + (i * t.per + m) * 2;
            const float lx = __fsub_rn(px, hp[0]), ly = __fsub_rn(py, hp[1]);
            f = make_float4(lx, ly, 0.0f, 0.0f);
            mask = dist_rn(lx, ly) < c.lidar_mask_radius;
          } else {
            const float* xo = s_ob + m * SD;
            const float* xi = s_ag + i * SD;
            f = make_float4(__fsub_rn(xi[0], xo[0]), __fsub_rn(xi[1], xo[1]), __fsub_rn(xi[2], xo[2]), __fsub_rn(xi[3], xo[3]));
            mask = dist_rn(__fsub_rn(xi[0], xo[0]), __fsub_rn(xi[1], xo[1])) < c.obs_mask_radius;
          }
        }
        reinterpret_cast<float4*>(a.efeat)[(size_t)g * nE + idx] = f;
        if (!a.vecM) a.emask[(size_t)g * nE + idx] = mask ? 1.0f : 0.0f;
      }
      if (a.vecM) {
        const unsigned long long bits = __ballot(mask);
        const int i4 = base + 4 * lane;
        if (lane < 16 && i4 < nE) {
          const unsigned b = (unsigned)(bits >> (4 * lane));
          *reinterpret_cast<float4*>(a.emask + (size_t)g * nE + i4) =
              make_float4((b & 1u) ? 1.0f : 0.0f, (b & 2u) ? 1.0f : 0.0f, (b & 4u) ? 1.0f : 0.0f, (b & 8u) ? 1.0f : 0.0f);
        }
      }
    }
    GF_WAVE_SYNC();
    if (!more) break;
    g = gn;
    gn += stride;
  }
#undef GF_EACH
#undef GF_REQUEST
#undef GF_COMMIT
}

static int feats_grid_cap(const void* fn, int wpb, size_t smem) {
  static thread_local const void* k_fn = nullptr;
  static thread_local int k_wpb = 0, k_cap = 0;
  static thread_local size_t k_smem = 0;
  if (fn == k_fn && wpb == k_wpb && smem == k_smem) return k_cap;
  int per_cu = 0, dev = 0, cus = 256;
  if (hipOccupancyMaxActiveBlocksPerMultiprocessor(&per_cu, fn, 64 * wpb, smem) != hipSuccess || per_cu < 1) per_cu = 1;
  if (hipGetDevice(&dev) != hipSuccess ||
      hipDeviceGetAttribute(&cus, hipDeviceAttributeMultiprocessorCount, dev) != hipSuccess || cus < 1) cus = 256;
  k_fn = fn; k_wpb = wpb; k_smem = smem; k_cap = per_cu * cus;
  return k_cap;
}

extern "C" int32_t dgppo_graph_feats(const dgppo_env_cfg* cfg, const float* agent, int64_t agent_se, int64_t agent_st,
                                     const float* goal, const float* obst, const float* hits, int64_t hits_se,
                                     int64_t hits_st, const int32_t* env_ids, int32_t n_env, int32_t n_time, float* Xa,
                                     float* Xo, float* efeat, float* emask, int32_t Fp, void* stream) {
  int32_t rc = dgppo_validate_cfg(cfg);
  if (rc) return rc;
  DGPPO_REFUSE_VMAS(cfg, "dgppo_graph_feats", "dgppo_vmas_graph_feats");
  DGPPO_REQUIRE(n_env >= 0 && n_time >= 0, "graph_feats: negative counts");
  if (n_env == 0 || n_time == 0) return 0;
  DGPPO_REQUIRE(agent && goal && Xa && efeat && emask, "graph_feats: NULL operand");
  DGPPO_REQUIRE(Fp >= cfg->node_dim && Fp <= 32, "graph_feats: Fp must be in [node_dim, 32]");
  FeatArgs a;
  a.cfg = *cfg; a.t = make_topo(*cfg);
  const int n_on = a.t.Ns - a.t.n - a.t.ng;
  DGPPO_REQUIRE(n_on == 0 || Xo, "graph_feats: Xo is NULL");
  DGPPO_REQUIRE(a.t.Ns == a.t.n || Xo, "graph_feats: Xo is NULL");
  if (n_on > 0) {
    if (a.t.lidar) DGPPO_REQUIRE(hits, "graph_feats: hits is NULL");
    else DGPPO_REQUIRE(obst, "graph_feats: obst is NULL");
  }
  DGPPO_REQUIRE(((uintptr_t)efeat & 15) == 0, "graph_feats: efeat must be 16-byte aligned");
  a.agent = agent; a.agent_se = agent_se; a.agent_st = agent_st; a.goal = goal; a.obst = obst;
  a.hits = hits; a.hits_se = hits_se; a.hits_st = hits_st; a.env_ids = env_ids; a.n_env = n_env; a.n_time = n_time;
  a.Xa = Xa; a.Xo = Xo; a.efeat = efeat; a.emask = emask; a.Fp = Fp;
  a.rcp_fp = (uint32_t)((0x100000000ull + (uint64_t)Fp - 1) / (uint64_t)Fp);
  a.rcp_S = (uint32_t)((0x100000000ull + (uint64_t)a.t.S - 1) / (uint64_t)a.t.S);
  DGPPO_REQUIRE(Fp >= 2 && a.t.S >= 2 && (long)a.t.Ns * Fp < 65536 && (long)a.t.n * a.t.S < 65536, "graph_feats: sizes out of range");
  a.vecX = (Fp % 4 == 0 && ((uintptr_t)Xa & 15) == 0 && ((uintptr_t)Xo & 15) == 0) ? 1 : 0;
  a.vecM = ((a.t.n * a.t.S) % 4 == 0 && ((uintptr_t)emask & 15) == 0) ? 1 : 0;
  a.rcp_fq = a.vecX ? (uint32_t)((0x100000000ull + (uint64_t)(Fp / 4) - 1) / (uint64_t)(Fp / 4)) : 0u;
  const int SD = cfg->state_dim;
  const size_t rec = sizeof(float) * ((size_t)a.t.n * SD + (size_t)a.t.ng * SD + (size_t)n_on * (a.t.lidar ? 2 : SD));
  int wpb = 4;
  while (wpb > 1 && rec * wpb > 65536) wpb >>= 1;
  const long G = (long)n_env * n_time;
  const void* fn = SD == 5 ? reinterpret_cast<const void*>(&graph_feats_kernel<5>) : reinterpret_cast<const void*>(&graph_feats_kernel<4>);
  const int cap = feats_grid_cap(fn, wpb, rec * wpb);
  const long wgs = (G + wpb - 1) / wpb;
  const dim3 grid((unsigned)(wgs < cap ? wgs : cap)), block(64 * wpb);
  if (SD == 5) hipLaunchKernelGGL(graph_feats_kernel<5>, grid, block, rec * wpb, (hipStream_t)stream, a);
  else hipLaunchKernelGGL(graph_feats_kernel<4>, grid, block, rec * wpb, (hipStream_t)stream, a);
  DGPPO_LAUNCH_CHECK();
  return 0;
}
```

dgppo_amd/csrc/nn_attn.h:

```cpp
#pragma once
#include "graph_topo.h"

__device__ inline int slot_of(const Topo& t, int nd, int i) {
  if (nd < t.n) return nd;
  if (nd < t.n + t.ng) {
    const int g = nd - t.n;
    return t.spread ? t.n + g : (g == i ? t.n : -1);
  }
  const int q = nd - t.n - t.ng;
  if (t.lidar) return (q / t.per == i) ? t.n + t.gs + (q - i * t.per) : -1;
  return t.n + t.gs + q;
}

__device__ inline float ones_col(const Topo& t, const float* mrow) {
  if (t.gs > 0) return 1.0f;
  for (int s = 0; s < t.S; ++s)
    if (mrow[s] != 0.0f) return 1.0f;
  return 0.0f;
}

#define ABD_DW_STRIDE 320
struct AttnArgs {
  Topo t;
  int F, H, Kp;
  const float* qt;
  const float* Xa;
  const float* Xo;
  const float* efeat;
  const float* emask;
  float* zcat;
  float* attn;
  const float* dzcat;
  float* dqt;
  float* dXa;
  float* dXo;
  int relu_xo;
  int G;
  const float* Xo_raw; const float* Wo; const float* bo; int ldwo;
  float* dwo_slab;
  int TI;
};

using f32x4g = __attribute__((ext_vector_type(4))) float;

template <typename FA, typename FB, typename FC>
__device__ inline void mfma_tiles(int RTn, int CTn, int K4, int wave, int lane, FA fa, FB fb, FC fc) {
  const int li = lane & 15, lq = lane >> 4;
  for (int tile = wave; tile < RTn * CTn; tile += 4) {
    const int rt = tile / CTn, ct = tile - rt * CTn;
    f32x4g acc = {0.f, 0.f, 0.f, 0.f};
    int k4 = 0;
    for (; k4 + 4 <= K4; k4 += 4) {
      float av[4], bv[4];
#pragma unroll
      for (int u = 0; u < 4; ++u) { av[u] = fa(rt * 16 + li, (k4 + u) * 4 + lq); bv[u] = fb((k4 + u) * 4 + lq, ct * 16 + li); }
#pragma unroll
      for (int u = 0; u < 4; ++u) acc = __builtin_amdgcn_mfma_f32_16x16x4f32(av[u], bv[u], acc, 0, 0, 0);
    }
    for (; k4 < K4; ++k4) acc = __builtin_amdgcn_mfma_f32_16x16x4f32(fa(rt * 16 + li, k4 * 4 + lq), fb(k4 * 4 + lq, ct * 16 + li), acc, 0, 0, 0);
#pragma unroll
    for (int r = 0; r < 4; ++r) fc(rt * 16 + lq * 4 + r, ct * 16 + li, acc[r]);
  }
}

__device__ inline void put4(float* d, float4 v) { d[0] = v.x; d[1] = v.y; d[2] = v.z; d[3] = v.w; }

template <int CTRL> __device__ inline float dpp_f(float v) {
  return __int_as_float(__builtin_amdgcn_update_dpp(0, __float_as_int(v), CTRL, 0xf, 0xf, false));
}
__device__ inline float grp8_sum(float v) {
  v += dpp_f<0xB1>(v);
  v += dpp_f<0x4E>(v);
  v += dpp_f<0x141>(v);
  return v;
}
__device__ inline float grp8_max(float v) {
  v = fmaxf(v, dpp_f<0xB1>(v));
  v = fmaxf(v, dpp_f<0x4E>(v));
  v = fmaxf(v, dpp_f<0x141>(v));
  return v;
}

#pragma GCC visibility push(hidden)
size_t attn_image_bytes(const Topo& t, int F, int H, bool bwd);
size_t attn_mfma_smem(const Topo& t, int F, int H, bool bwd);
void launch_attn_wg(const AttnArgs& a, hipStream_t s, bool bwd, bool mfma);
bool attn_slot8_shape(const Topo& t, int F, int H);
bool attn_slot8_rows_ok(const dgppo_env_cfg& c, const Topo& t, int F, int H);
bool launch_attn_slot8(const AttnArgs& a, hipStream_t s, bool bwd);
bool attn_bd_shape(const Topo& t, int F, int H, int& PS, bool& hits);
bool launch_attn_bd(const AttnArgs& a, hipStream_t s, bool bwd);
void launch_attn_xo_dw_reduce(const float* slab, int G, float* dWo, int lddwo, float* dbo, hipStream_t s);
int32_t launch_attn_tiled(AttnArgs& a, hipStream_t s, bool bwd);
#pragma GCC visibility pop
```

dgppo_amd/engine.py:

```python
from __future__ import annotations

import dataclasses
from typing import Callable, Dict, Optional

import numpy as np
import os
import torch

from . import _native as N
from . import nets
from . import ops_algo as OA
from . import ops_env as OE
from . import ops_nn as K
from .utils import checkpoint as CK


@dataclasses.dataclass
class Hyper:
    gamma: float = 0.99
    gae_lambda: float = 0.95
    clip_eps: float = 0.25
    coef_ent: float = 1e-2
    max_grad_norm: float = 2.0
    lr_actor: float = 3e-4
# ... 75 lines not shown


class OptState:
    def __init__(self, n: int, device):
        self.m = torch.zeros(n, device=device)
        self.v = torch.zeros(n, device=device)
        self.state = torch.zeros(N.OPT_STATE_FLOATS, device=device)


class Engine:
    def __init__(self, cfg: N.EnvCfg, hyper: Hyper, device, T: int = 128,
                 allreduce: Optional[Callable[[torch.Tensor], None]] = None, world: int = 1, prepass_graphs: int = 1 << 20,
                 use_graphs: bool = False, multi_stream: bool = False, algo: str = "dgppo", rank: int = 0,
                 fused_step: bool = True, lean_attn0: bool = True):
        self.cfg, self.hp, self.device, self.T = cfg, hyper, device, T
        assert algo in ("dgppo", "informarl", "hcbfcrpo", "informarl_lagr"), algo
        self.algo = algo
        self.use_graphs = use_graphs and os.environ.get("DGPPO_HIPGRAPH", "1") != "0"
        self.multi_stream = multi_stream and os.environ.get("DGPPO_MULTI_STREAM", "1") != "0"
        self._side_streams = None
        self.fused_step = bool(fused_step) and OE.act_step_feats_supported(cfg, nets.input_width(cfg), nets.H_HEADS)
        self.lean_attn0 = bool(lean_attn0)
        self._ro_cache: Dict[tuple, dict] = {}
        self._upd_graph: dict = {}
        self.n_cost = cfg.n_cost
        spec = [("policy", "policy", hyper.actor_gnn_layers, 2), ("Vl", "Vl", hyper.Vl_gnn_layers, 1)]
        if algo == "dgppo":
            spec.append(("Vh", "Vh", hyper.Vh_gnn_layers, self.n_cost))
        elif algo == "informarl_lagr":
            spec.append(("Vh", "Vhg", hyper.Vh_gnn_layers, self.n_cost))
        def rnn_kw(name):
            if not hyper.use_rnn:
                return dict(rnn="none", rnn_layers=0)
            if name == "Vh" and algo == "dgppo":
                return dict(rnn="gru", rnn_layers=1)
            return dict(rnn="lstm" if hyper.use_lstm else "gru", rnn_layers=hyper.rnn_layers)
        sizes = [nets.make_layout(kind, cfg.node_dim, layers, n_out, **rnn_kw(k)).size for k, kind, layers, n_out in spec]
        offs, tot = [], 0
        for sz in sizes:
            offs.append(tot)
            tot += (sz + 3) // 4 * 4
        self.flat_grads = torch.zeros(tot + 4 * 8, device=device)
        self.n_reduced = tot + 3 * 8
        self.stats = self.flat_grads[tot:tot + 32].view(4, 8)
        built = {k: nets.Net(kind, cfg, layers, n_out, device, grads=self.flat_grads[o:o + sz], lean_attn0=self.lean_attn0, **rnn_kw(k))
                 for (k, kind, layers, n_out), o, sz in zip(spec, offs, sizes)}
        if algo == "informarl_lagr":
            self.lagr = torch.full((cfg.n_agents, self.n_cost), float(hyper.lagr_init), device=device)
            self.lagr_sums = torch.zeros(cfg.n_agents * self.n_cost, device=device)
        self.policy, self.Vl, self.Vh = built["policy"], built["Vl"], built.get("Vh")
        self.HC = self.policy.carry_dim
        self.opt = {k: OptState(net.layout.size, device) for k, net in self.nets.items()}
        self.arena = nets.Arena(device)
        self.allreduce = allreduce
        self.world, self.rank = int(world), int(rank)
        assert self.world >= 1 and (allreduce is not None or self.world == 1), "world > 1 needs an allreduce"
        assert 0 <= self.rank < self.world, f"rank {rank} outside world {world}"
        self.prepass_graphs = int(os.environ.get("DGPPO_PREPASS_GRAPHS", prepass_graphs))
        self.lam_pow = OA.lam_pow_table(hyper.gae_lambda, T, device)
        self.eps_hat = torch.zeros(cfg.n_agents, 2, device=device)
        self.reset_failed = torch.zeros(1, dtype=torch.int32, device=device)
        self.grad_hook: Optional[Callable[[str, nets.Net, int], None]] = None
        self._mb = 0

    @property
    def nets(self) -> Dict[str, nets.Net]:
        d = {"policy": self.policy, "Vl": self.Vl}
        if self.Vh is not None:
            d["Vh"] = self.Vh
        return d

    def set_entropy_noise(self, seed: int):
        OE.randn(seed, 0, self.eps_hat.view(-1))

    _CFG_IDENTITY = ("kind", "n_agents", "n_obs", "n_rays", "top_k", "node_dim", "n_cost")

    def _identity(self) -> dict:
        ident = {"algo": CK.encode_str(self.algo)}
        ident.update({f"cfg.{k}": int(getattr(self.cfg, k)) for k in self._CFG_IDENTITY})
        for f in dataclasses.fields(Hyper):
            v = getattr(self.hp, f.name)
            ident[f"hyper.{f.name}"] = int(v) if isinstance(v, (bool, int)) else float(v)
        ident["T"], ident["world"] = int(self.T), int(self.world)
        ident.update({f"size.{k}": int(net.layout.size) for k, net in self.nets.items()})
        return ident

    def _state_tensors(self) -> Dict[str, torch.Tensor]:
        t = {}
        for k, net in self.nets.items():
            opt = self.opt[k]
            t.update({f"{k}/params": net.params, f"{k}/m": opt.m, f"{k}/v": opt.v, f"{k}/state": opt.state})
        t["eps_hat"] = self.eps_hat
        if self.algo == "informarl_lagr":
            t["lagr"] = self.lagr
        return t

    def state_dict(self) -> dict:
        out = {"identity": self._identity()}
        for path, x in self._state_tensors().items():
            node = out
            *dirs, leaf = path.split("/")
            for d in dirs:
                node = node.setdefault(d, {})
            node[leaf] = x.detach().cpu().numpy().copy()
        return out

    def load_state_dict(self, d: dict) -> None:
        mine, theirs = self._identity(), d.get("identity", {})
        show = lambda v: repr(CK.decode_str(v)) if isinstance(v, np.ndarray) else repr(v)
        for k, v in mine.items():
            if k not in theirs:
                raise ValueError(f"state dict does not fit this engine: it has no identity field '{k}'")
            if not np.array_equal(np.asarray(v), np.asarray(theirs[k])):
                raise ValueError(f"state dict does not fit this engine: '{k}' is {show(theirs[k])} there, {show(v)} here")
        src = {}
        for path, x in self._state_tensors().items():
            node = d
            for part in path.split("/"):
                node = node.get(part) if isinstance(node, dict) else None
            if not isinstance(node, np.ndarray) or node.dtype != np.float32 or node.shape != tuple(x.shape):
                raise ValueError(f"state dict does not fit this engine: '{path}' is not a float32 array of shape {tuple(x.shape)}")
            src[path] = node
        for path, x in self._state_tensors().items():
            x.copy_(torch.from_numpy(src[path]).to(self.device))
        for net in self.nets.values():
            net.prepare()

    def _feats(self, tag, st: OE.State, n_env, n_time=1, slots=1, env_ids=None):
        f = nets.GraphFeats(self.cfg, n_env * n_time, self.arena, tag)
        return f.compute_record(st.step, slots, st.env, env_ids, n_env, n_time)

    def _rollout_steps(self, ro: RolloutData, eps, B: int, stochastic: bool, start: int = 0):
        cfg, T, n = self.cfg, ro.T, self.cfg.n_agents
        tag = "ro" if stochastic else "rod"
        if self.fused_step:
            pol, R = self.policy, B * n
            feats = self._feats(tag, ro.states_tm[start], B)
            Mcat, cvec = pol.pp("gnn0.Mcat"), pol.pp("gnn0.cvec")
            qt0 = pol.arena.get(f"{tag}.qt0", R, Mcat.shape[1])
            K.dense_fwd(feats.Xa, Mcat, cvec, qt0)
            for t in range(start, T):
                act = pol.forward(feats, n_seq=R, T=1, h0=ro.rnn_tm[t].view(R, self.HC), tag=tag,
                                  hs_out=ro.rnn_tm[t + 1].view(R, self.HC), train=False, qt0=qt0)
                nxt = dict(Xa=feats.Xa, Xo=feats.Xo, efeat=feats.efeat, emask=feats.emask, Fp=feats.Fp, Mcat=Mcat, cvec=cvec,
                           qt0=qt0, H=nets.H_HEADS) if t + 1 < T else {}
                OE.act_step_feats(cfg, ro.states_tm[t], act["ms"], eps[t] if stochastic else None, ro.action_tm[t],
                                  ro.log_pi_tm[t] if stochastic else None, ro.states_tm[t + 1], ro.reward_tm[t], ro.cost_tm[t],
                                  **nxt)
                feats.edges_from_rows = cfg.state_dim == 4
            return
        for t in range(start, T):
            feats = self._feats(tag, ro.states_tm[t], B)
            act = self.policy.forward(feats, n_seq=B * n, T=1, h0=ro.rnn_tm[t].view(B * n, self.HC), tag=tag,
                                      hs_out=ro.rnn_tm[t + 1].view(B * n, self.HC), train=False)
            a_t = ro.action_tm[t].view(B * n, 2)
            if stochastic:
                K.policy_head(act["ms"], eps[t], None, a_t, ro.log_pi_tm[t].view(B * n), None, n, 0)
            else:
                K.policy_head(act["ms"], None, None, a_t, None, None, n, 1)
            OE.step(cfg, ro.states_tm[t], ro.action_tm[t], ro.states_tm[t + 1], ro.reward_tm[t], ro.cost_tm[t])

    def rollout(self, seeds: torch.Tensor, stochastic: bool, noise_seed: int = 0) -> RolloutData:
        cfg, T = self.cfg, self.T
        B = int(seeds.shape[0])
        n = cfg.n_agents
        slot = None
        if self.use_graphs:
            slot = self._ro_cache.setdefault((B, stochastic), {"ro": None, "graph": None, "gen": -1, "calls": 0})
            if slot["ro"] is None:
                slot["ro"] = RolloutData(cfg, B, T, self.device, stochastic, self.HC)
            ro = slot["ro"]
            ro._env_major = False
        else:
            ro = RolloutData(cfg, B, T, self.device, stochastic, self.HC)
        OE.reset(cfg, seeds, ro.states_tm[0], self.reset_failed)
        ro.rnn_tm[0].zero_()
        eps = None
        if stochastic:
            eps = self.arena.get("ro.eps", T, B * n, 2)
            OE.randn_rows(noise_seed, eps.view(T, B * n * 2), self.world * B * n * 2, self.rank * B * n * 2)
        if slot is None:
            self._rollout_steps(ro, eps, B, stochastic)
# ... 897 lines not shown
```

dgppo_amd/nets.py:

```python
from __future__ import annotations

import math
from typing import Dict, List, Optional, Tuple

import numpy as np
import torch

from . import _native as N
from . import ops_nn as K

H_HEADS = 3
MSG_DIM = 32
OUT_DIM = 64
HID = 64


def _ceil4(x):
    return (x + 3) // 4 * 4


class Layout:
    def __init__(self):
        self.entries: Dict[str, Tuple[int, Tuple[int, ...]]] = {}
        self.size = 0
# ... 19 lines not shown
                        ("We", (4, hd)), ("Wu", (f, d)), ("bu", (d,))):
            L.add(f"gnn{l}.{nm}", *shp)
        f = d
    for i in (1, 2):
        L.add(f"mlp.W{i}", 2 * HID if (kind == "Vhg" and i == 1) else HID, HID)
        L.add(f"mlp.b{i}", HID)
        L.add(f"mlp.g{i}", HID)
        L.add(f"mlp.be{i}", HID)
    assert rnn in ("gru", "lstm", "none"), rnn
    for l in range(rnn_layers if rnn == "lstm" else 0):
        L.add(f"lstm{l}.Wi", HID, 4 * HID)
        L.add(f"lstm{l}.Wh", HID, 4 * HID)
        L.add(f"lstm{l}.bh", 4 * HID)
    for l in range(rnn_layers if rnn == "gru" else 0):
        pre = "gru" if l == 0 else f"gru{l}"
        L.add(f"{pre}.Wi", HID, 3 * HID)
        L.add(f"{pre}.bi", 3 * HID)
        L.add(f"{pre}.Wh", HID, 3 * HID)
        L.add(f"{pre}.bhn", HID)
    if kind == "policy":
        L.add("head.Ws", HID, HID)
        L.add("head.bs", HID)
        L.add("head.Wms", HID, 2 * n_out)
        L.add("head.bms", 2 * n_out)
    else:
        L.add("head.Wo", HID, n_out)
        L.add("head.bo", n_out)
    return L


class Arena:

    def __init__(self, device):
        self.device = device
        self.bufs: Dict[str, torch.Tensor] = {}
        self.generation = 0

    def get(self, name: str, *shape, dtype=torch.float32, zero=False) -> torch.Tensor:
        n = math.prod(shape)
        b = self.bufs.get(name)
        if b is None or b.numel() < n or b.dtype != dtype:
            if b is not None:
                self.generation += 1
            b = torch.empty(max(n, 1), dtype=dtype, device=self.device)
            self.bufs[name] = b
        v = b[:n].view(shape)
        if zero:
            v.zero_()
        return v


class GraphFeats:

    def __init__(self, cfg: N.EnvCfg, G: int, arena: Arena, tag: str):
        self.cfg, self.G = cfg, G
        n, S = cfg.n_agents, cfg.fan_in
        self.n_other = cfg.num_nodes - 1 - n
        self.Fp = input_width(cfg)
        self.Xa = arena.get(f"{tag}.Xa0", G * n, self.Fp)
        self.Xo = arena.get(f"{tag}.Xo0", max(G * self.n_other, 1), self.Fp)[:G * self.n_other]
        self.efeat = arena.get(f"{tag}.efeat", G * n, S, 4)
        self.emask = arena.get(f"{tag}.emask", G * n, S)
        self.edges_from_rows = False

    def compute(self, agent, agent_se, agent_st, goal, obst, hits, hits_se, hits_st, env_ids, n_env, n_time):
        assert n_env * n_time == self.G
        K.graph_feats(self.cfg, agent, agent_se, agent_st, goal, obst, hits, hits_se, hits_st, env_ids, n_env, n_time,
                      self.Xa, self.Xo if self.n_other > 0 else None, self.efeat, self.emask, self.Fp)
        self.edges_from_rows = self.cfg.state_dim == 4
        return self

    def compute_record(self, step, slots: int, env, env_ids, n_env, n_time):
        cfg, n = self.cfg, self.cfg.n_agents
        se, st = slots, int(slots > 1)
        if cfg.is_vmas:
            return self.compute_vmas(step["agent"], se * n * 4, st * n * 4, step["body"], se * 4, st * 4, env["scene"], env_ids,
                                     n_env, n_time)
        ia, ih = n * cfg.state_dim, n * cfg.top_k * 2
        return self.compute(step["agent"], se * ia, st * ia, env["goal"], env.get("obst"), step.get("hits"), se * ih, st * ih,
                            env_ids, n_env, n_time)

    def compute_sweep(self, step, env, frame_ids, n_frames, agent_id, xs, ys, ray_cos=None, ray_sin=None, hits_out=None,
                      frame_max=None):
        cfg, n = self.cfg, self.cfg.n_agents
        if cfg.is_vmas:
            raise ValueError("compute_sweep: VMASReverseTransport has no sweep entry point")
        K.graph_feats_sweep(cfg, step["agent"], n * cfg.state_dim, env["goal"], env.get("obst"), step.get("hits"),
                            n * cfg.top_k * 2, ray_cos, ray_sin, frame_ids, n_frames, agent_id, xs, ys, self.Xa,
                            self.Xo if self.n_other > 0 else None, self.efeat, self.emask, self.Fp, hits_out, frame_max)
        self.edges_from_rows = False
        return self

    def compute_action_sweep(self, step, env, frame_ids, n_frames, agent_id, us, vs, frame_max=None):
        cfg, n = self.cfg, self.cfg.n_agents
        if cfg.is_vmas:
            raise ValueError("compute_action_sweep: VMASReverseTransport has no sweep entry point")
        K.graph_feats_action_sweep(cfg, step["agent"], n * cfg.state_dim, env["goal"], env.get("obst"), step.get("hits"),
                                   n * cfg.top_k * 2, frame_ids, n_frames, agent_id, us, vs, self.Xa,
                                   self.Xo if self.n_other > 0 else None, self.efeat, self.emask, self.Fp, frame_max)
        self.edges_from_rows = False
        return self

    def compute_team_action_sweep(self, st, nst, a_pol, us, vs):
        if self.cfg.is_vmas:
            raise ValueError("compute_team_action_sweep: VMASReverseTransport has no sweep entry point")
        K.graph_feats_team_action_sweep(self.cfg, st.step["agent"], nst.step["agent"], st.env["goal"], st.env.get("obst"),
                                        nst.step.get("hits"), a_pol, us, vs, self.Xa, self.Xo if self.n_other > 0 else None,
                                        self.efeat, self.emask, self.Fp)
        self.edges_from_rows = False
        return self

    def compute_vmas(self, agent, agent_se, agent_st, body, body_se, body_st, scene, env_ids, n_env, n_time):
        assert n_env * n_time == self.G
        K.vmas_graph_feats(self.cfg, agent, agent_se, agent_st, body, body_se, body_st, scene, env_ids, n_env, n_time,
                           self.Xa, self.efeat, self.emask, self.Fp)
        self.edges_from_rows = False
        return self


def input_width(cfg: N.EnvCfg) -> int:
    return _ceil4(cfg.node_dim) if cfg.is_vmas else 8


class Net:

    def __init__(self, kind: str, cfg: N.EnvCfg, gnn_layers: int, n_out: int, device, grads: Optional[torch.Tensor] = None,
                 rnn: str = "gru", rnn_layers: int = 1, lean_attn0: bool = True):
        assert kind in ("policy", "Vl", "Vh", "Vhg")
        self.kind, self.cfg, self.gnn_layers, self.n_out, self.device = kind, cfg, gnn_layers, n_out, device
        self.rnn, self.rnn_layers = rnn, (rnn_layers if rnn != "none" else 0)
        self.lean_attn0 = bool(lean_attn0) and K.attn_rows_supported(cfg, input_width(cfg), H_HEADS)
        self.carry_dim = HID * max(self.rnn_layers, 1) * (2 if rnn == "lstm" else 1)
        self.layout = make_layout(kind, cfg.node_dim, gnn_layers, n_out, rnn, rnn_layers)
        self.params = torch.zeros(self.layout.size, device=device)
        if grads is None:
            grads = torch.zeros(self.layout.size, device=device)
        assert grads.shape == (self.layout.size,) and grads.is_contiguous() and grads.data_ptr() % 16 == 0
        self.grads = grads
        self.arena = Arena(device)
        self.ws_arena = Arena(device)
        self._views: Dict[tuple, torch.Tensor] = {}
        self.dims = []
        f = cfg.node_dim
        for l in range(gnn_layers):
            d = OUT_DIM if l == gnn_layers - 1 else MSG_DIM
            fp = input_width(cfg) if l == 0 else f
            kp = _ceil4(fp + H_HEADS * (fp + 4) + 1)
            self.dims.append((f, fp, d, kp))
            f = d
        self.prep_layout = Layout()
        for l, (f, fp, d, kp) in enumerate(self.dims):
            self.prep_layout.add(f"gnn{l}.Mcat", fp, H_HEADS * fp)
            self.prep_layout.add(f"gnn{l}.cvec", H_HEADS * fp)
            self.prep_layout.add(f"gnn{l}.Wout", kp, d)
        self.prep = torch.zeros(self.prep_layout.size, device=device)
        self.prep_grads = torch.zeros(self.prep_layout.size, device=device)

    def _cached(self, kind: str, layout, flat, name):
        key = (kind, name)
        v = self._views.get(key)
        if v is None:
            v = self._views[key] = layout.view(flat, name)
        return v

    def p(self, name):
        return self._cached("p", self.layout, self.params, name)

    def g(self, name):
        return self._cached("g", self.layout, self.grads, name)

    def pp(self, name):
        return self._cached("pp", self.prep_layout, self.prep, name)

    def pg(self, name):
        return self._cached("pg", self.prep_layout, self.prep_grads, name)

    def prepare(self):
        for l, (f, fp, d, kp) in enumerate(self.dims):
            q = lambda nm: self.p(f"gnn{l}.{nm}")
            K.gnn_prep(q("Wq"), q("bq"), q("Wk"), q("Wv"), q("bv"), q("We"), q("Wu"), self.pp(f"gnn{l}.Mcat"),
                       self.pp(f"gnn{l}.cvec"), self.pp(f"gnn{l}.Wout"), f, fp, d, H_HEADS, kp)

    def _xo_fusable(self, l: int) -> bool:
        if l != 0 or self.gnn_layers != 2:
            return False
        key = "_xo_ok"
        if not hasattr(self, key):
            f1, fp1, d1, kp1 = self.dims[1]
            setattr(self, key, self.dims[0][1] == 8 and self.dims[0][2] == 32 and fp1 == 32 and
                    K.attn_xo_supported(self.cfg, fp1, H_HEADS, kp1))
        return getattr(self, key)

    def zero_grads(self):
        self.grads.zero_()

    def forward(self, feats: GraphFeats, n_seq: int, T: int, h0: Optional[torch.Tensor], tag: str = "f",
                hs_out: Optional[torch.Tensor] = None, train: bool = True, qt0: Optional[torch.Tensor] = None):
        cfg, G, A = self.cfg, feats.G, self.arena
        n = cfg.n_agents
        R = G * n
        Ro = G * feats.n_other
        act = {"feats": feats, "G": G, "n_seq": n_seq, "T": T}
        Xa, Xo = feats.Xa, feats.Xo
        xo_fused = None
        for l, (f, fp, d, kp) in enumerate(self.dims):
            if l == 0 and qt0 is not None:
                assert tuple(qt0.shape) == (R, H_HEADS * fp), (tuple(qt0.shape), R, H_HEADS * fp)
                qt = qt0
            else:
                qt = A.get(f"{tag}.qt{l}", R, H_HEADS * fp)
                K.dense_fwd(Xa, self.pp(f"gnn{l}.Mcat"), self.pp(f"gnn{l}.cvec"), qt)
            zcat = A.get(f"{tag}.zcat{l}", R, kp)
            lean = l == 0 and self.lean_attn0 and feats.edges_from_rows
            attn = A.get(f"{tag}.attn{l}", R, cfg.fan_in, H_HEADS) if train and not lean else None
            if lean:
                K.attn_fwd_rows(cfg, fp, H_HEADS, kp, qt, Xa, Xo if Ro > 0 else None, feats.emask, zcat, None, G)
            elif xo_fused is not None:
                K.attn_fwd_xo(cfg, fp, H_HEADS, kp, qt, Xa, xo_fused[0], xo_fused[1], xo_fused[2], feats.efeat, feats.emask, zcat, attn, G)
            else:
                K.attn_fwd(cfg, fp, H_HEADS, kp, qt, Xa, Xo if Ro > 0 else None, feats.efeat, feats.emask, zcat, attn, G)
            act[f"xo_fused{l}"] = xo_fused
            xo_fused = None
            Xa_n = A.get(f"{tag}.Xa{l + 1}", R, d)
            K.dense_fwd(zcat, self.pp(f"gnn{l}.Wout"), self.p(f"gnn{l}.bu"), Xa_n, act=1)
            act[f"Xa{l}"], act[f"Xo{l}"], act[f"qt{l}"], act[f"zcat{l}"], act[f"attn{l}"] = Xa, Xo, qt, zcat, attn
            act[f"lean{l}"] = lean
            if l < self.gnn_layers - 1 and Ro > 0:
                if self._xo_fusable(l):
                    xo_fused = (Xo, self.pp(f"gnn{l}.Wout")[:fp], self.p(f"gnn{l}.bu"))
                    Xo = None
                else:
                    Xo_n = A.get(f"{tag}.Xo{l + 1}", Ro, d)
                    K.dense_fwd(Xo, self.pp(f"gnn{l}.Wout")[:fp], self.p(f"gnn{l}.bu"), Xo_n, act=1)
                    Xo = Xo_n
            Xa = Xa_n
        act[f"Xa{self.gnn_layers}"] = Xa
        if self.kind == "Vl":
            pooled = A.get(f"{tag}.pool", G, OUT_DIM)
            K.mean_agents(Xa, pooled, G, n, OUT_DIM)
            x, Rh, n_inner = pooled, G, 1
        else:
            x, Rh, n_inner = Xa, R, n
        if self.kind == "Vhg":
            pooled = A.get(f"{tag}.pool", G, OUT_DIM)
            K.mean_agents(Xa, pooled, G, n, OUT_DIM)
            xcat = A.get(f"{tag}.xcat", R, 2 * OUT_DIM)
            xcat[:, :OUT_DIM].copy_(Xa)
            xcat.view(G, n, 2 * OUT_DIM)[:, :, OUT_DIM:].copy_(pooled.view(G, 1, OUT_DIM).expand(G, n, OUT_DIM))
            x = xcat
        act["Rh"], act["n_inner"], act["mlp_in"] = Rh, n_inner, x
        gi = A.get(f"{tag}.gi", Rh, 3 * HID)
        if self.kind == "Vhg" or self.rnn != "gru":
            sv = {nm: A.get(f"{tag}.{nm}", Rh, w) for nm, w in (("p1", HID), ("y1", HID), ("st1", 2), ("p2", HID), ("y2", HID), ("st2", 2))}
            K.dense_fwd(x, self.p("mlp.W1"), self.p("mlp.b1"), sv["p1"])
            K.ln_relu_fwd(sv["p1"], self.p("mlp.g1"), self.p("mlp.be1"), sv["y1"], sv["st1"])
            K.dense_fwd(sv["y1"], self.p("mlp.W2"), self.p("mlp.b2"), sv["p2"])
            K.ln_relu_fwd(sv["p2"], self.p("mlp.g2"), self.p("mlp.be2"), sv["y2"], sv["st2"])
            if self.rnn == "gru":
                K.dense_fwd(sv["y2"], self.p("gru.Wi"), self.p("gru.bi"), gi)
            act.update(sv)
        else:
            saves = None
            if train:
                saves = tuple(A.get(f"{tag}.{nm}{i}", Rh, w) for i in (1, 2) for nm, w in (("p", HID), ("y", HID), ("st", 2)))
                for i in (1, 2):
                    act[f"p{i}"], act[f"y{i}"], act[f"st{i}"] = saves[3 * (i - 1):3 * i]
            K.mlp_gi_fwd(x, self.p("mlp.W1"), self.p("mlp.b1"), self.p("mlp.g1"), self.p("mlp.be1"), self.p("mlp.W2"),
                         self.p("mlp.b2"), self.p("mlp.g2"), self.p("mlp.be2"), self.p("gru.Wi"), self.p("gru.bi"), gi, saves)
        assert n_seq * T == Rh, (n_seq, T, Rh)
        L, CD = self.rnn_layers, self.carry_dim
        h0_blocks = isinstance(h0, K.H0Blocks)
        if h0_blocks:
            assert self.rnn == "gru" and L == 1 and T == 1 and not train and self.kind != "policy", \
                "a blocked h0 serves the one-cell GRU value nets' T = 1 inference pass"
        elif h0 is not None:
            assert tuple(h0.shape) == (n_seq, CD), (tuple(h0.shape), n_seq, CD)
        if hs_out is not None:
            assert tuple(hs_out.shape) == (Rh, CD), (tuple(hs_out.shape), Rh, CD)
        act["gi"] = gi
# ... 187 lines not shown
                dx = A.get(f"{tag}.dy" if l == 0 else f"{tag}.dx{l}", Rh, HID)
                K.dense_fwd(dgi, self.p(f"{pre}.Wi"), None, dx, trans_w=True)
                dhs = dx
            dy = dhs
        x_in = {1: act["mlp_in"], 2: act["y1"]}
        top = act[f"Xa{self.gnn_layers}"]
        if fused_trunk:
            dy = A.get(f"{tag}.dyy1", Rh, HID)
            K.mlp_gi_bwd_w(dgi0, self.p("gru.Wi"), self.p("mlp.W2"), self.p("mlp.W1"), self.p("mlp.g2"), self.p("mlp.g1"),
                           act["p2"], act["y2"], act["st2"], act["p1"], act["y1"], act["st1"], x_in[1],
                           top if self.kind in ("policy", "Vh") else None, dy,
                           self.g("mlp.g2"), self.g("mlp.be2"), self.g("mlp.g1"), self.g("mlp.be1"),
                           self.g("mlp.W2"), self.g("mlp.b2"), self.g("mlp.W1"), self.g("mlp.b1"))
        for i in (() if fused_trunk else (2, 1)):
            dpre = A.get(f"{tag}.dpre{i}", Rh, HID)
            K.ln_relu_bwd(act[f"p{i}"], act[f"y{i}"], act[f"st{i}"], self.p(f"mlp.g{i}"), dy, dpre, self.g(f"mlp.g{i}"),
                          self.g(f"mlp.be{i}"))
            K.dense_bwd_w(x_in[i], dpre, self.g(f"mlp.W{i}"), self.g(f"mlp.b{i}"))
            dy = A.get(f"{tag}.dyy{i}", Rh, HID if not (self.kind == "Vhg" and i == 1) else 2 * HID)
            K.dense_fwd(dpre, self.p(f"mlp.W{i}"), None, dy, trans_w=True,
                        relu_mask=top if (i == 1 and self.kind in ("policy", "Vh")) else None)
        if self.kind == "Vl":
            dXa = A.get(f"{tag}.dXaL", R, OUT_DIM)
            K.mean_agents(dy, dXa, G, n, OUT_DIM, backward=True, relu_mask=top)
        elif self.kind == "Vhg":
            dXa = A.get(f"{tag}.dXaL", R, OUT_DIM)
            dXa.copy_(dy[:, :OUT_DIM])
            dglob = A.get(f"{tag}.dglob", R, OUT_DIM)
            dglob.copy_(dy[:, OUT_DIM:])
            dpool = A.get(f"{tag}.dpool", G, OUT_DIM)
            K.mean_agents(dglob, dpool, G, n, OUT_DIM)
            K.mean_agents(dpool, dXa, G, n, OUT_DIM, backward=2, relu_mask=top)
        else:
            dXa = dy
        dXo = None
        for l in range(self.gnn_layers - 1, -1, -1):
            f, fp, d, kp = self.dims[l]
            dz = A.get(f"{tag}.dz{l}", R, kp)
            K.dense_bwd_xw(act[f"zcat{l}"], dXa, self.pp(f"gnn{l}.Wout"), dz, self.pg(f"gnn{l}.Wout"), self.g(f"gnn{l}.bu"))
            if dXo is not None:
                K.dense_bwd_w(act[f"Xo{l}"], dXo, self.pg(f"gnn{l}.Wout")[:fp], self.g(f"gnn{l}.bu"))
            dqt = A.get(f"{tag}.dqt{l}", R, H_HEADS * fp)
            need_dx = l > 0
            dXa_l = A.get(f"{tag}.dXa{l}", R, fp) if need_dx else None
            dXo_prev = dXo
            dXo_l = A.get(f"{tag}.dXo{l}", Ro, fp) if (need_dx and Ro > 0) else None
            more_dXo = dXo_prev is not None and dXo_l is not None
            xf = act.get(f"xo_fused{l}")
            if act.get(f"lean{l}"):
                K.attn_bwd_rows(cfg, fp, H_HEADS, kp, dz, None, act[f"qt{l}"], feats.emask, act[f"Xa{l}"],
                                act[f"Xo{l}"] if Ro > 0 else None, dqt, G)
            elif xf is not None and dXa_l is not None and not more_dXo:
                ws = A.get(f"{tag}.xo_ws", K.attn_xo_workspace_floats(G), 1).view(-1)
                K.attn_bwd_xo_dw(cfg, fp, H_HEADS, kp, dz, act[f"attn{l}"], act[f"qt{l}"], act[f"Xa{l}"], xf[0], xf[1], xf[2],
                                 feats.efeat, dqt, dXa_l, self.pg(f"gnn{l - 1}.Wout")[:self.dims[l - 1][1]], self.g(f"gnn{l - 1}.bu"), ws, G)
                dXo_l = None
            elif xf is not None:
                K.attn_bwd_xo(cfg, fp, H_HEADS, kp, dz, act[f"attn{l}"], act[f"qt{l}"], act[f"Xa{l}"], xf[0], xf[1], xf[2],
                              feats.efeat, dqt, dXa_l, dXo_l, G, relu_xo=(dXo_l is not None and not more_dXo))
            else:
                K.attn_bwd(cfg, fp, H_HEADS, kp, dz, act[f"attn{l}"], act[f"qt{l}"], act[f"Xa{l}"],
                           act[f"Xo{l}"] if Ro > 0 else None, feats.efeat, dqt, dXa_l, dXo_l, G,
                           relu_xo=(dXo_l is not None and not more_dXo))
            if need_dx:
                K.dense_bwd_xw(act[f"Xa{l}"], dqt, self.pp(f"gnn{l}.Mcat"), dXa_l, self.pg(f"gnn{l}.Mcat"), self.pg(f"gnn{l}.cvec"),
                               accumulate_mask=True)
            else:
                K.dense_bwd_w(act[f"Xa{l}"], dqt, self.pg(f"gnn{l}.Mcat"), self.pg(f"gnn{l}.cvec"))
            if need_dx:
                if more_dXo:
                    K.dense_fwd(dXo_prev, self.pp(f"gnn{l}.Wout")[:fp], None, dXo_l, accumulate=True, trans_w=True,
                                relu_mask=act[f"Xo{l}"])
            dXa, dXo = dXa_l, dXo_l

    def load_tree(self, tree: dict):
        t = tree["params"]
        to = lambda x: torch.as_tensor(np.asarray(x), dtype=torch.float32).to(self.device)
        if self.kind == "policy":
            base, gnn, head_name = t["PolicyNet_0"], t["PolicyNet_0"]["GraphTransformerGNN_0"], "PolicyGNNHead"
        else:
            base, gnn, head_name = t, t["GraphTransformerGNN_0"], "ValueGNNHead"
        for l in range(self.gnn_layers):
            gl = gnn[f"GraphTransformer_{l}"]
            for nm, dn, key in (("Wq", "Dense_0", "kernel"), ("bq", "Dense_0", "bias"), ("Wk", "Dense_1", "kernel"),
                                ("bk", "Dense_1", "bias"), ("Wv", "Dense_2", "kernel"), ("bv", "Dense_2", "bias"),
                                ("We", "Dense_3", "kernel"), ("Wu", "Dense_4", "kernel"), ("bu", "Dense_4", "bias")):
                self.p(f"gnn{l}.{nm}").copy_(to(gl[dn][key]))
        hd = base[head_name]
        for i in (1, 2):
            self.p(f"mlp.W{i}").copy_(to(hd[f"Dense_{i - 1}"]["kernel"]))
            self.p(f"mlp.b{i}").copy_(to(hd[f"Dense_{i - 1}"]["bias"]))
            self.p(f"mlp.g{i}").copy_(to(hd[f"LayerNorm_{i - 1}"]["scale"]))
            self.p(f"mlp.be{i}").copy_(to(hd[f"LayerNorm_{i - 1}"]["bias"]))
        for l in range(self.rnn_layers if self.rnn == "lstm" else 0):
            lc = base["RNN_0"][f"LSTMCell_{3 * l + 2}"]
            self.p(f"lstm{l}.Wi").copy_(torch.cat([to(lc[k]["kernel"]) for k in ("ii", "if", "ig", "io")], dim=1))
            self.p(f"lstm{l}.Wh").copy_(torch.cat([to(lc[k]["kernel"]) for k in ("hi", "hf", "hg", "ho")], dim=1))
            self.p(f"lstm{l}.bh").copy_(torch.cat([to(lc[k]["bias"]) for k in ("hi", "hf", "hg", "ho")]))
        for l in range(self.rnn_layers if self.rnn == "gru" else 0):
            pre = "gru" if l == 0 else f"gru{l}"
            gr = base["RNN_0"][f"GRUCell_{2 * l + 1}"]
            self.p(f"{pre}.Wi").copy_(torch.cat([to(gr[k]["kernel"]) for k in ("ir", "iz", "in")], dim=1))
            self.p(f"{pre}.bi").copy_(torch.cat([to(gr[k]["bias"]) for k in ("ir", "iz", "in")]))
            self.p(f"{pre}.Wh").copy_(torch.cat([to(gr[k]["kernel"]) for k in ("hr", "hz", "hn")], dim=1))
            self.p(f"{pre}.bhn").copy_(to(gr["hn"]["bias"]))
        if self.kind == "policy":
            self.p("head.Ws").copy_(to(t["ScaleHid"]["kernel"]))
            self.p("head.bs").copy_(to(t["ScaleHid"]["bias"]))
            self.p("head.Wms").copy_(torch.cat([to(t["OutputDenseMean"]["kernel"]), to(t["OutputDenseStdTrans"]["kernel"])], 1))
# ... 48 lines not shown
```

dgppo_amd/ops_env.py:

```python
from __future__ import annotations

import ctypes as C
from typing import Dict, Optional

import numpy as np
import torch

from . import _native as N


STEP_FIELDS, ENV_FIELDS = ("agent", "hits", "body"), ("goal", "obst", "scene")


def record_fields(cfg: N.EnvCfg) -> tuple[Dict[str, tuple], Dict[str, tuple]]:
    n, sd = cfg.n_agents, cfg.state_dim
    if cfg.is_vmas:
        return {"agent": (n, 4), "body": (4,)}, {"scene": (8,)}
    step, env = {"agent": (n, sd)}, {"goal": (cfg.n_goals, sd)}
    if cfg.is_lidar and cfg.n_obs > 0:
        step["hits"] = (n, cfg.top_k, 2)
    if cfg.n_obs > 0:
        env["obst"] = (cfg.n_obs, cfg.obst_stride)
    return step, env

# ... 201 lines not shown
def sense(cfg: N.EnvCfg, st: State, graph: Optional[Dict[str, torch.Tensor]] = None):
    s, e = st.step, st.env
    if "hits" not in s:
        s["hits"] = torch.empty(s["agent"].shape[:-2] + record_fields(cfg)[0]["hits"], device=s["agent"].device)
    rc, rs = _rays(cfg, s["agent"].device)
    env_step(cfg, s["agent"], None, e["goal"], e.get("obst"), None, rc, rs, None, s["hits"], None, None, graph)


def reset(cfg: N.EnvCfg, seeds: torch.Tensor, st: State, n_failed: torch.Tensor = None,
          graph: Optional[Dict[str, torch.Tensor]] = None):
    if cfg.is_vmas:
        vmas_reset(cfg, seeds, st.agent, st.body, st.scene, n_failed)
    else:
        env_reset(cfg, seeds, st.agent, st.goal, st.obst, n_failed)
    if "hits" in st.step:
        sense(cfg, st, graph)
    elif graph is not None:
        materialize(cfg, st, graph)


def step(cfg: N.EnvCfg, st: State, action, nst: State, reward, cost, graph: Optional[Dict[str, torch.Tensor]] = None):
    s, e, ns = st.step, st.env, nst.step
    if cfg.is_vmas:
        return vmas_step(cfg, s["agent"], s["body"], e["scene"], action, ns["agent"], ns["body"], reward, cost, graph)
    rc, rs = _rays(cfg, s["agent"].device)
    env_step(cfg, s["agent"], action, e["goal"], e.get("obst"), s.get("hits"), rc, rs, ns["agent"], ns.get("hits"), reward,
             cost, graph)


def act_step_feats_supported(cfg: N.EnvCfg, Fp: int, H: int) -> bool:
    return bool(N.lib().dgppo_env_act_step_feats_supported(C.byref(cfg), C.c_int32(Fp), C.c_int32(H)))


def act_step_feats(cfg: N.EnvCfg, st: State, ms, eps, action, log_pi, nst: State, reward, cost, Xa=None, Xo=None, efeat=None,
                   emask=None, Fp: int = 8, Mcat=None, cvec=None, qt0=None, H: int = 3, max_blocks: int = 0):
    s, e, ns = st.step, st.env, nst.step
    agent = s["agent"]
    B, n = agent.shape[0], cfg.n_agents
    rc, rs = _rays(cfg, agent.device)
    sample = eps is not None
    N.expect_shape(ms, (B * n, 4), "ms")
    N.expect_shape(action, (B, n, 2), "action")
    N.expect_shape(ns["agent"], (B, n, cfg.state_dim), "next_agent")
    N.expect_shape(ns["hits"], (B, n, cfg.top_k, 2), "next_hits")
    N.expect_shape(reward, (B,), "reward")
    N.expect_shape(cost, (B, n, cfg.n_cost), "cost")
    if sample:
        N.expect_shape(eps, (B * n, 2), "eps")
        N.expect_shape(log_pi, (B, n), "log_pi")
    if Xa is not None:
        S = cfg.fan_in
        N.expect_shape(Xa, (B * n, Fp), "Xa")
        N.expect_shape(Xo, (B * (cfg.num_nodes - 1 - n), Fp), "Xo")
        N.expect_shape(efeat, (B * n, S, 4), "efeat")
        N.expect_shape(emask, (B * n, S), "emask")
    if qt0 is not None:
        N.expect_shape(Mcat, (Fp, H * Fp), "Mcat")
        N.expect_shape(cvec, (H * Fp,), "cvec")
        N.expect_shape(qt0, (B * n, H * Fp), "qt0")
    rc_ = N.lib().dgppo_env_act_step_feats(
        C.byref(cfg), N.ptr(agent, name="agent"), N.ptr(e["goal"], name="goal"), N.ptr(e.get("obst"), name="obst"),
        N.ptr(s.get("hits"), name="hits"), N.ptr(rc, name="ray_cos"), N.ptr(rs, name="ray_sin"), N.ptr(ms, name="ms"),
        N.ptr(eps, name="eps"), C.c_int32(1 if sample else 0), N.ptr(action, name="action"),
        N.ptr(log_pi if sample else None, name="log_pi"), N.ptr(ns["agent"], name="next_agent"),
        N.ptr(ns["hits"], name="next_hits"), N.ptr(reward, name="reward"), N.ptr(cost, name="cost"), N.ptr(Xa, name="Xa"),
        N.ptr(Xo if Xa is not None else None, name="Xo"), N.ptr(efeat if Xa is not None else None, name="efeat"),
        N.ptr(emask if Xa is not None else None, name="emask"), C.c_int32(Fp), N.ptr(Mcat, name="Mcat"),
        N.ptr(cvec, name="cvec"), N.ptr(qt0, name="qt0"), C.c_int32(H), C.c_int32(max_blocks), C.c_int32(B), N.stream_ptr())
    N.check(rc_, "dgppo_env_act_step_feats")


def sweep_fork(cfg: N.EnvCfg, step: Dict[str, torch.Tensor], env: Dict[str, torch.Tensor], frame_ids, n_frames: int,
               agent_id: int, xs, ys, out: State, carry=None, carry_st: int = 0, carry_out=None, frame_max=None):
    from . import ops_nn as K
    fn = "sweep_fork"
    if cfg.is_vmas:
        raise ValueError(f"{fn}: VMASReverseTransport has no sweep entry point")
    n, sd, k = cfg.n_agents, cfg.state_dim, cfg.top_k
    agent, hits, obst, goal = step["agent"], step.get("hits"), env.get("obst"), env["goal"]
    nx, ny, ids, ids_dev, last = K._sweep_grid(fn, cfg, frame_ids, n_frames, agent_id, xs, ys, frame_max)
    G = n_frames * ny * nx
    rc, rs = _rays(cfg, agent.device)
    cast = K._sweep_record(fn, cfg, agent, n * sd, obst, hits, n * k * 2, rc, rs, last, None, G)
    N.expect_shape(goal, (cfg.n_goals, sd), "goal")
    o_step, o_env = out.step, out.env
    for fields, held in zip(record_fields(cfg), (o_step, o_env)):
        for name, shape in fields.items():
            if held.get(name) is None:
                raise ValueError(f"{fn}: out has no {name}")
            N.expect_shape(held[name], (G,) + shape, f"out.{name}")
    HC = 0
    if carry is not None:
        if carry_out is None or carry_out.ndim != 2 or carry_out.shape[0] != G * n:
            raise ValueError(f"{fn}: carry_out must be [G * n, HC] = [{G * n}, HC]")
        HC = int(carry_out.shape[1])
        K._check_strided(fn, "carry", carry, 0, int(carry_st), (n, HC), None, 1, last + 1)
    if ids is not None:
        ids_dev = torch.from_numpy(ids.astype(np.int32)).to(agent.device)
    raw = lambda t_: C.c_void_p(t_.data_ptr())
    rc_ = N.lib().dgppo_env_sweep_fork(
        C.byref(cfg), raw(agent), n * sd, N.ptr(goal, name="goal"), N.ptr(obst, name="obst"), raw(hits) if cast else None,
        n * k * 2, N.ptr(rc if cast else None, name="ray_cos"), N.ptr(rs if cast else None, name="ray_sin"),
        N.ptr(ids_dev, torch.int32, "frame_ids"), n_frames, int(agent_id), N.ptr(xs, name="xs"), nx, N.ptr(ys, name="ys"), ny,
        raw(carry) if carry is not None else None, int(carry_st), HC, N.ptr(o_step["agent"], name="out.agent"),
        N.ptr(o_env["goal"], name="out.goal"), N.ptr(o_env.get("obst"), name="out.obst"),
        N.ptr(o_step.get("hits") if cast else None, name="out.hits"),
        N.ptr(carry_out if carry is not None else None, name="carry_out"), N.stream_ptr())
# ... 124 lines not shown
```

dgppo_amd/ops_nn.py:

```python
from __future__ import annotations

import ctypes as C
from typing import Optional

import numpy as np
import torch

from . import _native as N

FLOPS = [0.0]


def _mat(t: torch.Tensor, name: str):
    if t.dim() != 2:
        raise ValueError(f"{name} must be 2-D, got {tuple(t.shape)}")
    if not t.is_cuda:
        raise RuntimeError(f"{name} must live on the GPU (the HIP path has no CPU fallback)")
    if t.dtype != torch.float32:
        raise TypeError(f"{name} must be float32")
    if t.shape[1] > 1 and t.stride(1) != 1:
        raise ValueError(f"{name} must have unit inner stride")
    ld = t.stride(0) if t.shape[0] > 1 else max(t.shape[1], t.stride(0))
    return C.c_void_p(t.data_ptr()), int(ld), int(t.shape[0]), int(t.shape[1])

# ... 177 lines not shown

def dense_bwd_xw(X, dY, W, dX, dW, db=None, accumulate_mask: bool = False):
    xp, ldx, M, K = _mat(X, "X")
    yp, ldy, My, Ncol = _mat(dY, "dY")
    pp, ldp, Kp, Np = _mat(W, "W")
    dxp, lddx, Mx, Kx = _mat(dX, "dX")
    wp, ldw, Kw, Nw = _mat(dW, "dW")
    if My != M or (Kw, Nw) != (K, Ncol) or (Kp, Np) != (K, Ncol) or (Mx, Kx) != (M, K):
        raise ValueError(f"dense_bwd_xw: shape mismatch X{tuple(X.shape)} dY{tuple(dY.shape)} W{tuple(W.shape)} "
                         f"dX{tuple(dX.shape)} dW{tuple(dW.shape)}")
    if db is not None:
        N.expect_shape(db, (Ncol,), "db")
    FLOPS[0] += 4.0 * M * K * Ncol
    batch = BwdWBatch._active.get((X.device.index, torch.cuda.current_stream(X.device).cuda_stream))
    lib = N.lib()
    if batch is not None:
        lib.dgppo_dense_bwd_w_workspace_bytes.restype = C.c_int64
        ws = batch.region(min(int(lib.dgppo_dense_bwd_w_workspace_bytes(C.c_int32(K), C.c_int32(Ncol))), 64 << 20))
        d = ReduceDesc()
        pend = C.byref(d)
    else:
        ws = _bwd_w_workspace(X.device, K, Ncol)
        pend = None
    rc = lib.dgppo_dense_bwd_xw(xp, ldx, yp, ldy, pp, ldp, dxp, lddx, int(bool(accumulate_mask)), wp, ldw, _p(db, "db"), M, K,
                                Ncol, _p(ws, "workspace"), C.c_int64(ws.numel() * 4), pend, N.stream_ptr())
    N.check(rc, "dgppo_dense_bwd_xw")
    if batch is not None and d.pending:
        batch.descs.append(d)


def _check_strided(fn: str, name: str, t_, se: int, st: int, inner: tuple, env_ids, n_env: int, n_time: int):
    if not (t_.is_cuda and t_.dtype == torch.float32):
        raise ValueError(f"{fn}: {name} must be a float32 CUDA tensor")
    want, acc = [], 1
    for d in reversed(inner):
        want.append(acc)
        acc *= d
    if tuple(t_.shape[-len(inner):]) != tuple(inner) or list(t_.stride()[-len(inner):]) != want[::-1]:
        raise ValueError(f"{fn}: the trailing {inner} block of {name} must be dense (got shape {tuple(t_.shape)}, "
                         f"strides {t_.stride()})")
    avail = t_.untyped_storage().nbytes() // 4 - t_.storage_offset()
    if env_ids is None and (n_env - 1) * se + (n_time - 1) * st + acc > avail:
        raise ValueError(f"{fn}: {name}: the strides reach beyond its storage")


def graph_feats(cfg: N.EnvCfg, agent, agent_se, agent_st, goal, obst, hits, hits_se, hits_st, env_ids, n_env, n_time,
                Xa, Xo, efeat, emask, Fp):
    G = n_env * n_time
    n, S = cfg.n_agents, cfg.fan_in
    n_other = cfg.num_nodes - 1 - n
    N.expect_shape(Xa, (G * n, Fp), "Xa")
    if n_other > 0:
        N.expect_shape(Xo, (G * n_other, Fp), "Xo")
    N.expect_shape(efeat, (G * n, S, 4), "efeat")
    N.expect_shape(emask, (G * n, S), "emask")
    _check_strided("graph_feats", "agent", agent, agent_se, agent_st, (n, cfg.state_dim), env_ids, n_env, n_time)
    if hits is not None:
        _check_strided("graph_feats", "hits", hits, hits_se, hits_st, (n, cfg.top_k, 2), env_ids, n_env, n_time)
    rc = N.lib().dgppo_graph_feats(
        C.byref(cfg), C.c_void_p(agent.data_ptr()), C.c_int64(agent_se), C.c_int64(agent_st), _p(goal, "goal"),
        _p(obst, "obst") if (obst is not None and not cfg.is_lidar) else C.c_void_p(0),
        C.c_void_p(hits.data_ptr()) if hits is not None else C.c_void_p(0), C.c_int64(hits_se), C.c_int64(hits_st),
        _p(env_ids, "env_ids", torch.int32), C.c_int32(n_env), C.c_int32(n_time), _p(Xa, "Xa"), _p(Xo, "Xo"),
        _p(efeat, "efeat"), _p(emask, "emask"), C.c_int32(Fp), N.stream_ptr())
    N.check(rc, "dgppo_graph_feats")


def sweep_axis(x, name: str, device) -> torch.Tensor:
    if torch.is_tensor(x):
        t_ = x.to(device=device, dtype=torch.float32).contiguous()
        ok = t_.ndim == 1 and t_.numel() > 0 and bool(torch.isfinite(t_).all())
    else:
        a = np.ascontiguousarray(np.asarray(x, dtype=np.float32))
        ok = a.ndim == 1 and a.size > 0 and bool(np.isfinite(a).all())
        t_ = torch.from_numpy(a).to(device) if ok else None
    if not ok:
        raise ValueError(f"graph_feats_sweep: {name} must be a non-empty 1-D array of finite coordinates")
    return t_


def _sweep_grid(fn: str, cfg: N.EnvCfg, frame_ids, n_frames, agent_id, xs, ys, frame_max, names=("xs", "ys")):
    n = cfg.n_agents
    if not 0 <= int(agent_id) < n:
        raise ValueError(f"{fn}: agent_id {agent_id} outside [0, {n})")
    for name, t_ in zip(names, (xs, ys)):
        if not (torch.is_tensor(t_) and t_.is_cuda and t_.dtype == torch.float32 and t_.ndim == 1 and t_.is_contiguous()):
            raise ValueError(f"{fn}: {name} must be a dense 1-D float32 CUDA tensor (sweep_axis)")
        if t_.numel() == 0:
            raise ValueError(f"{fn}: {name} is empty")
    ids = ids_dev = None
    if torch.is_tensor(frame_ids):
        if frame_max is None or n_frames < 1 or tuple(frame_ids.shape) != (n_frames,):
            raise ValueError(f"{fn}: a device frame_ids needs its shape (n_frames,) and frame_max")
        ids_dev, last = frame_ids, int(frame_max)
    elif frame_ids is not None:
        ids = np.asarray(frame_ids, dtype=np.int64).reshape(-1)
        if ids.size != n_frames or n_frames == 0 or ids.min() < 0:
            raise ValueError(f"{fn}: frame_ids must hold n_frames >= 1 frame numbers >= 0")
        last = int(ids.max())
    else:
        if n_frames < 1:
            raise ValueError(f"{fn}: n_frames must be >= 1")
        last = n_frames - 1
    return int(xs.numel()), int(ys.numel()), ids, ids_dev, last


def _sweep_record(fn: str, cfg: N.EnvCfg, agent, agent_st, obst, hits, hits_st, ray_cos, ray_sin, last, hits_out, G) -> bool:
# ... 320 lines not shown


def _wo_ld(Wo):
    if Wo.dim() != 2 or Wo.shape[0] != 8 or Wo.shape[1] < 32 or Wo.stride(1) != 1:
        raise ValueError(f"Wo must be [8, >= 32] with contiguous rows, got {tuple(Wo.shape)} strides {Wo.stride()}")
    return int(Wo.stride(0))


def attn_fwd_xo(cfg, F, H, Kp, qt, Xa, Xo_raw, Wo, bo, efeat, emask, zcat, attn, G):
    n, S = cfg.n_agents, cfg.fan_in
    N.expect_shape(qt, (G * n, H * F), "qt")
    N.expect_shape(Xa, (G * n, F), "Xa")
    N.expect_shape(zcat, (G * n, Kp), "zcat")
    N.expect_shape(Xo_raw, (G * (cfg.num_nodes - 1 - n), 8), "Xo_raw")
    N.expect_shape(bo, (32,), "bo")
    if attn is not None:
        N.expect_shape(attn, (G * n, S, H), "attn")
    FLOPS[0] += 2.0 * G * n * H * S * (2 * F + 4) + 2.0 * G * (cfg.num_nodes - 1 - n) * 8 * 32
    rc = N.lib().dgppo_attn_fwd_xo(C.byref(cfg), F, H, Kp, _p(qt), _p(Xa), _p(Xo_raw), _wo_ptr(Wo),
                                   _wo_ld(Wo), _p(bo), _p(efeat), _p(emask), _p(zcat), _p(attn), G, N.stream_ptr())
    N.check(rc, "dgppo_attn_fwd_xo")


def attn_bwd_xo(cfg, F, H, Kp, dzcat, attn, qt, Xa, Xo_raw, Wo, bo, efeat, dqt, dXa, dXo, G, relu_xo: bool = False):
    n = cfg.n_agents
    N.expect_shape(dzcat, (G * n, Kp), "dzcat")
    N.expect_shape(dqt, (G * n, H * F), "dqt")
    N.expect_shape(Xo_raw, (G * (cfg.num_nodes - 1 - n), 8), "Xo_raw")
    if dXa is not None:
        N.expect_shape(dXa, (G * n, F), "dXa")
    FLOPS[0] += 4.0 * G * n * H * cfg.fan_in * (2 * F + 4) + 2.0 * G * (cfg.num_nodes - 1 - n) * 8 * 32
    rc = N.lib().dgppo_attn_bwd_xo(C.byref(cfg), F, H, Kp, _p(dzcat), _p(attn), _p(qt), _p(Xa), _p(Xo_raw),
                                   _wo_ptr(Wo), _wo_ld(Wo), _p(bo), _p(efeat), _p(dqt), _p(dXa), _p(dXo),
                                   int(relu_xo), G, N.stream_ptr())
    N.check(rc, "dgppo_attn_bwd_xo")


def attn_xo_workspace_floats(G: int) -> int:
    return int(N.lib().dgppo_attn_xo_workspace_bytes(int(G))) // 4


def attn_bwd_xo_dw(cfg, F, H, Kp, dzcat, attn, qt, Xa, Xo_raw, Wo, bo, efeat, dqt, dXa, dWo, dbo, workspace, G):
    n = cfg.n_agents
    N.expect_shape(dzcat, (G * n, Kp), "dzcat")
    N.expect_shape(dqt, (G * n, H * F), "dqt")
    N.expect_shape(dXa, (G * n, F), "dXa")
    N.expect_shape(Xo_raw, (G * (cfg.num_nodes - 1 - n), 8), "Xo_raw")
    N.expect_shape(dbo, (32,), "dbo")
    FLOPS[0] += 4.0 * G * n * H * cfg.fan_in * (2 * F + 4) + 4.0 * G * (cfg.num_nodes - 1 - n) * 8 * 32
    rc = N.lib().dgppo_attn_bwd_xo_dw(C.byref(cfg), F, H, Kp, _p(dzcat), _p(attn), _p(qt), _p(Xa), _p(Xo_raw), _wo_ptr(Wo), _wo_ld(Wo),
                                      _p(bo), _p(efeat), _p(dqt), _p(dXa), _wo_ptr(dWo), _wo_ld(dWo), _p(dbo), _p(workspace),
                                      C.c_int64(workspace.numel() * 4), G, N.stream_ptr())
    N.check(rc, "dgppo_attn_bwd_xo_dw")


def gnn_prep(Wq, bq, Wk, Wv, bv, We, Wu, Mcat, cvec, Wout, F, Fp, D, H, Kp):
    rc = N.lib().dgppo_gnn_prep(_p(Wq), _p(bq), _p(Wk), _p(Wv), _p(bv), _p(We), _p(Wu), _p(Mcat), _p(cvec), _p(Wout),
                                F, Fp, D, H, Kp, N.stream_ptr())
    N.check(rc, "dgppo_gnn_prep")


def gnn_unprep(dMcat, dcvec, dWout, Wq, bq, Wk, dWq, dbq, dWk, dWv, dbv, dWe, dWu, F, Fp, D, H, Kp):
    rc = N.lib().dgppo_gnn_unprep(_p(dMcat), _p(dcvec), _p(dWout), _p(Wq), _p(bq), _p(Wk), _p(dWq), _p(dbq), _p(dWk),
                                  _p(dWv), _p(dbv), _p(dWe), _p(dWu), F, Fp, D, H, Kp, N.stream_ptr())
    N.check(rc, "dgppo_gnn_unprep")


def ln_relu_fwd(x, gamma, beta, y, stats):
    M = x.shape[0]
    N.expect_shape(x, (M, 64), "x")
    N.expect_shape(y, (M, 64), "y")
    rc = N.lib().dgppo_ln_relu_fwd(_p(x), _p(gamma), _p(beta), _p(y), _p(stats), M, N.stream_ptr())
    N.check(rc, "dgppo_ln_relu_fwd")


def ln_relu_bwd(x, y, stats, gamma, dy, dx, dgamma, dbeta):
    M = x.shape[0]
    rc = N.lib().dgppo_ln_relu_bwd(_p(x), _p(y), _p(stats), _p(gamma), _p(dy), _p(dx), _p(dgamma), _p(dbeta), M,
                                   N.stream_ptr())
    N.check(rc, "dgppo_ln_relu_bwd")


def gru_fwd(gi, Wh, bhn, h0, hs, hprev, gates, n_seq, T, n_inner):
    rows = n_seq * T
    N.expect_shape(gi, (rows, 192), "gi")
    N.expect_shape(hs, (rows, 64), "hs")
    N.expect_shape(Wh, (64, 192), "Wh")
    if h0 is not None:
        N.expect_shape(h0, (n_seq, 64), "h0")
    FLOPS[0] += 2.0 * rows * 64 * 192
    rc = N.lib().dgppo_gru_fwd(_p(gi), _p(Wh), _p(bhn), _p(h0), _p(hs), _p(hprev), _p(gates), n_seq, T, n_inner,
                               N.stream_ptr())
    N.check(rc, "dgppo_gru_fwd")


class H0Blocks:

    def __init__(self, base: torch.Tensor, rows_per_block: int, block_stride: int, n_blocks: int):
        assert base.dtype == torch.float32 and base.is_cuda
        st = base.untyped_storage()
        last = base.storage_offset() + (n_blocks - 1) * block_stride + rows_per_block * 64
        assert n_blocks >= 1 and last * 4 <= st.nbytes(), "H0Blocks: the blocks leave the storage of base"
        self.base, self.rows_per_block, self.block_stride, self.n_blocks = base, int(rows_per_block), int(block_stride), int(n_blocks)

    @property
    def n_seq(self) -> int:
# ... 259 lines not shown
```

include/dgppo_hip.h:

```cpp
#ifndef DGPPO_HIP_H
#define DGPPO_HIP_H

#include <stdint.h>

#ifdef __cplusplus
extern "C" {
#endif

#define DGPPO_ABI_VERSION 3

enum {
  DGPPO_ENV_LIDAR_SPREAD = 0,
  DGPPO_ENV_LIDAR_TARGET = 1,
  DGPPO_ENV_LIDAR_BICYCLE_TARGET = 2,
  DGPPO_ENV_MPE_SPREAD = 3,
  DGPPO_ENV_MPE_TARGET = 4,
  DGPPO_ENV_LIDAR_LINE = 5,
  DGPPO_ENV_MPE_LINE = 6,
  DGPPO_ENV_MPE_FORMATION = 7,
  DGPPO_ENV_MPE_CORRIDOR = 8,
  DGPPO_ENV_MPE_CONNECT_SPREAD = 9,
  DGPPO_ENV_VMAS_REVERSE_TRANSPORT = 10
};
enum {
// ... 181 lines not shown
                            int32_t n_cost, const float* us, int32_t nu, const float* vs, int32_t nv, float dt, float alpha,
                            float margin, float* action, int32_t* index, int32_t* flag, float* h, void* stream);

int32_t dgppo_env_sweep_fork(const dgppo_env_cfg* cfg, const float* agent, int64_t agent_st, const float* goal,
                             const float* obst, const float* hits, int64_t hits_st, const float* ray_cos, const float* ray_sin,
                             const int32_t* frame_ids, int32_t n_frames, int32_t agent_id, const float* xs, int32_t nx,
                             const float* ys, int32_t ny, const float* carry, int64_t carry_st, int32_t HC, float* agent_out,
                             float* goal_out, float* obst_out, float* hits_out, float* carry_out, void* stream);

int32_t dgppo_constraint_return(const float* cost, int64_t cost_st, int32_t K, int32_t G, int32_t n_agents, int32_t nh,
                                float gamma, float one_minus_gamma, float* value, float* worst, void* stream);

int32_t dgppo_env_team_action_fork(const dgppo_env_cfg* cfg, const float* agent, const float* goal, const float* obst,
                                   const float* hits, const float* a_pol, const float* carry, int32_t HC, int32_t n_env,
                                   const float* us, int32_t nu, const float* vs, int32_t nv, float* agent_out, float* goal_out,
                                   float* obst_out, float* hits_out, float* action_out, float* carry_out, void* stream);

int32_t dgppo_lookahead_select(const float* cost, int64_t cost_st, int32_t K, int32_t n_env, int32_t n_agents, int32_t n_cost,
                               const float* a_pol, const float* us, int32_t nu, const float* vs, int32_t nv, float margin,
                               float* action, int32_t* index, int32_t* flag, float* s, void* stream);

int32_t dgppo_env_action_sweep_fork(const dgppo_env_cfg* cfg, const float* agent, int64_t agent_st, const float* goal,
                                    const float* obst, const float* hits, int64_t hits_st, const float* action, int64_t action_st,
                                    const float* carry, int64_t carry_st, int32_t HC, const int32_t* frame_ids, int32_t n_frames,
                                    int32_t agent_id, const float* us, int32_t nu, const float* vs, int32_t nv, float* agent_out,
                                    float* goal_out, float* obst_out, float* hits_out, float* action_out, float* carry_out,
                                    void* stream);

int32_t dgppo_attn_fwd(const dgppo_env_cfg* cfg, int32_t F, int32_t H, int32_t Kp, const float* qt, const float* Xa,
                       const float* Xo, const float* efeat, const float* emask, float* zcat, float* attn, int32_t G,
                       void* stream);
int32_t dgppo_attn_bwd(const dgppo_env_cfg* cfg, int32_t F, int32_t H, int32_t Kp, const float* dzcat,
                       const float* attn, const float* qt, const float* Xa, const float* Xo, const float* efeat,
                       float* dqt, float* dXa, float* dXo, int32_t relu_xo, int32_t G, void* stream);
int32_t dgppo_attn_rows_supported(const dgppo_env_cfg* cfg, int32_t F, int32_t H);
int32_t dgppo_attn_fwd_rows(const dgppo_env_cfg* cfg, int32_t F, int32_t H, int32_t Kp, const float* qt, const float* Xa,
                            const float* Xo, const float* emask, float* zcat, float* attn, int32_t G, void* stream);
int32_t dgppo_attn_bwd_rows(const dgppo_env_cfg* cfg, int32_t F, int32_t H, int32_t Kp, const float* dzcat, const float* attn,
                            const float* qt, const float* emask, const float* Xa, const float* Xo, float* dqt, int32_t G,
                            void* stream);
int32_t dgppo_attn_xo_supported(const dgppo_env_cfg* cfg, int32_t F, int32_t H, int32_t Kp);
int32_t dgppo_attn_fwd_xo(const dgppo_env_cfg* cfg, int32_t F, int32_t H, int32_t Kp, const float* qt, const float* Xa,
                          const float* Xo_raw, const float* Wo, int32_t ldwo, const float* bo, const float* efeat,
                          const float* emask, float* zcat, float* attn, int32_t G, void* stream);
int32_t dgppo_attn_bwd_xo(const dgppo_env_cfg* cfg, int32_t F, int32_t H, int32_t Kp, const float* dzcat,
                          const float* attn, const float* qt, const float* Xa, const float* Xo_raw, const float* Wo,
                          int32_t ldwo, const float* bo, const float* efeat, float* dqt, float* dXa, float* dXo,
                          int32_t relu_xo, int32_t G, void* stream);
int64_t dgppo_attn_xo_workspace_bytes(int32_t G);
int32_t dgppo_attn_bwd_xo_dw(const dgppo_env_cfg* cfg, int32_t F, int32_t H, int32_t Kp, const float* dzcat,
                             const float* attn, const float* qt, const float* Xa, const float* Xo_raw, const float* Wo,
                             int32_t ldwo, const float* bo, const float* efeat, float* dqt, float* dXa, float* dWo,
                             int32_t lddwo, float* dbo, float* workspace, int64_t workspace_bytes, int32_t G, void* stream);

int32_t dgppo_gnn_prep(const float* Wq, const float* bq, const float* Wk, const float* Wv, const float* bv,
                       const float* We, const float* Wu, float* Mcat, float* cvec, float* Wout, int32_t F, int32_t Fp,
                       int32_t D, int32_t H, int32_t Kp, void* stream);
int32_t dgppo_gnn_unprep(const float* dMcat, const float* dcvec, const float* dWout, const float* Wq, const float* bq,
                         const float* Wk, float* dWq, float* dbq, float* dWk, float* dWv, float* dbv, float* dWe,
                         float* dWu, int32_t F, int32_t Fp, int32_t D, int32_t H, int32_t Kp, void* stream);

int32_t dgppo_ln_relu_fwd(const float* x, const float* gamma, const float* beta, float* y, float* stats, int32_t M,
                          void* stream);
int32_t dgppo_ln_relu_bwd(const float* x, const float* y, const float* stats, const float* gamma, const float* dy,
                          float* dx, float* dgamma, float* dbeta, int32_t M, void* stream);

int32_t dgppo_gru_fwd(const float* gi, const float* Wh, const float* bhn, const float* h0, float* hs, float* hprev,
                      float* gates, int32_t n_seq, int32_t T, int32_t n_inner, void* stream);
int32_t dgppo_gru_fwd_h0_blocks(const float* gi, const float* Wh, const float* bhn, const float* h0,
                                int32_t rows_per_block, int64_t block_stride, float* hs, float* hprev, float* gates,
                                int32_t n_seq, int32_t T, int32_t n_inner, void* stream);
int32_t dgppo_gru_bwd(const float* dhs, const float* Wh, const float* hprev, const float* gates, float* dgi,
                      float* dgh, int32_t n_seq, int32_t T, int32_t n_inner, void* stream);
int32_t dgppo_gru_bwd_dhn(const float* dhs, const float* Wh, const float* hprev, const float* gates, float* dgi,
                          float* dhn, int32_t n_seq, int32_t T, int32_t n_inner, void* stream);
int64_t dgppo_gru_bwd_w_workspace_bytes(void);
int32_t dgppo_gru_bwd_w(const float* x, int32_t ldx, const float* hprev, int32_t ldh, const float* dgi, const float* dhn,
                        float* dWi, int32_t ldwi, float* dbi, float* dWh, int32_t ldwh, float* dbhn, int32_t M,
                        float* workspace, int64_t workspace_bytes, dgppo_reduce_desc* pending, void* stream);
int32_t dgppo_gru_bwd_w_t1(const float* x, int32_t ldx, const float* h0, int32_t ldh, const float* dhs, const float* gates,
                           float* dgi, float* dWi, int32_t ldwi, float* dbi, float* dWh, int32_t ldwh, float* dbhn, int32_t M,
                           float* workspace, int64_t workspace_bytes, dgppo_reduce_desc* pending, void* stream);

int32_t dgppo_lstm_fwd(const float* zi, const float* Wh, const float* bh, const float* c0, const float* h0, float* cs,
                       float* hs, float* cprev, float* hprev, float* gates, int32_t n_seq, int32_t T, int32_t n_inner,
                       void* stream);
int32_t dgppo_lstm_bwd(const float* dhs, const float* Wh, const float* cprev, const float* gates, float* dz,
                       int32_t n_seq, int32_t T, int32_t n_inner, void* stream);

int32_t dgppo_policy_head(const float* ms, const float* eps, const float* action_in, float* action, float* log_pi,
                          float* entropy, int32_t rows, int32_t n_agents, int32_t mode, const float* log_pi_old,
                          const float* adv, float* dms, float* stats, float clip_eps, float coef_ent, void* stream);

int32_t dgppo_value_loss(const float* v, const float* target, float* dv, float* stats, int32_t count, void* stream);
int32_t dgppo_mean_agents(const float* x, float* y, int32_t G, int32_t n, int32_t D, int32_t backward,
                          const float* relu_mask, void* stream);
int32_t dgppo_relu_bwd(float* dy, const float* y, int64_t count, void* stream);


int32_t dgppo_gae(const float* costs, const float* rewards, const float* Vh, const float* Vl, const float* lam_pow,
                  float gamma, float one_minus_gamma, float one_minus_lam, float* Qh, float* Ql, int32_t B, int32_t T,
                  int32_t n, int32_t nh, void* stream);
int32_t dgppo_advantage(const float* Ql, const float* Vl, const float* Vh, float dt, float alpha, float cbf_eps,
                        float cbf_weight, float* adv, float* stats, int32_t B, int32_t T, int32_t n, int32_t nh,
                        void* stream);
int32_t dgppo_advantage_lagr(const float* Ql, const float* Vl, const float* Qh, const float* Vh, const float* lagr,
// ... 27 lines not shown
```

Baseline: 4.597 million.

## Derive edge features from raw node rows inside fused BD attention kernels

Adds a ROWS mode to the fused BD attention forward and backward kernels. Per-edge features are computed on the fly from the raw sender and receiver rows (Xa_raw, Xo_raw) instead of being read from a materialized efeat tensor. This drops the efeat buffer traffic and possibly the kernel that builds it, at the cost of extra arithmetic and gathers in the kernel and new dispatch paths in the Python model code. The new path is used only when the configuration check passes for the topology.

```diff
diff --git a/dgppo_amd/csrc/attn.hip b/dgppo_amd/csrc/attn.hip
--- a/dgppo_amd/csrc/attn.hip
+++ b/dgppo_amd/csrc/attn.hip
@@ -102,36 +102,77 @@
   a.Xo_raw = Xo_raw; a.Wo = Wo; a.ldwo = ldwo; a.bo = bo;
   return 0;
 }
+static bool attn_xo_rows_ok(const dgppo_env_cfg& c, const Topo& t, int F, int H, int Kp) { return attn_xo_ok(t, F, H, Kp) && attn_bd_rows_ok(c); }
+static int32_t attn_set_xo_rows(AttnArgs& a, const float* Xa_raw, const char* who) {
+  DGPPO_REQUIRE(Xa_raw && (reinterpret_cast<uintptr_t>(Xa_raw) & 15) == 0 && (reinterpret_cast<uintptr_t>(a.Xo_raw) & 15) == 0,
+                "%s: Xa_raw and Xo_raw must be 16-byte aligned", who);
+  a.Xa_raw = Xa_raw;
+  return 0;
+}
+static int32_t attn_fwd_xo_any(const char* who, bool rows, const dgppo_env_cfg* cfg, int32_t F, int32_t H, int32_t Kp, const float* qt,
+                               const float* Xa, const float* Xa_raw, const float* Xo_raw, const float* Wo, int32_t ldwo, const float* bo,
+                               const float* efeat, const float* emask, float* zcat, float* attn, int32_t G, void* stream) {
+  AttnArgs a{};
+  int32_t rc = attn_check(cfg, F, H, Kp, G, a);
+  if (rc) return rc;
+  if (rows) DGPPO_REQUIRE(attn_xo_rows_ok(*cfg, a.t, F, H, Kp), "%s: no such kernel for this configuration (ask dgppo_attn_xo_rows_supported)", who);
+  if (G == 0) return 0;
+  DGPPO_REQUIRE(qt && Xa && Xo_raw && Wo && bo && (rows || efeat) && emask && zcat, "%s: NULL operand", who);
+  DGPPO_REQUIRE(ldwo >= 32, "%s: ldwo=%d < 32", who, ldwo);
+  rc = attn_set_xo(a, Xo_raw, Wo, ldwo, bo, who);
+  if (rc) return rc;
+  if (rows && (rc = attn_set_xo_rows(a, Xa_raw, who))) return rc;
+  attn_set_fwd(a, qt, Xa, nullptr, rows ? nullptr : efeat, emask, zcat, attn);
+  return attn_launch(AttnFamily::BD, a, stream, false, who);
+}
+static int32_t attn_bwd_xo_any(const char* who, bool rows, const dgppo_env_cfg* cfg, int32_t F, int32_t H, int32_t Kp, const float* dzcat,
+                               const float* attn, const float* qt, const float* Xa, const float* Xa_raw, const float* Xo_raw,
+                               const float* Wo, int32_t ldwo, const float* bo, const float* efeat, float* dqt, float* dXa, float* dXo,
+                               int32_t relu_xo, int32_t G, void* stream) {
+  AttnArgs a{};
+  int32_t rc = attn_check(cfg, F, H, Kp, G, a);
+  if (rc) return rc;
+  if (rows) DGPPO_REQUIRE(attn_xo_rows_ok(*cfg, a.t, F, H, Kp), "%s: no such kernel for this configuration (ask dgppo_attn_xo_rows_supported)", who);
+  if (G == 0) return 0;
+  DGPPO_REQUIRE(dzcat && attn && qt && Xa && Xo_raw && Wo && bo && (rows || efeat) && dqt, "%s: NULL operand", who);
+  DGPPO_REQUIRE(ldwo >= 32, "%s: ldwo=%d < 32", who, ldwo);
+  DGPPO_REQUIRE(!(dXo && !dXa), "%s: dXo needs dXa", who);
+  rc = attn_set_xo(a, Xo_raw, Wo, ldwo, bo, who);
+  if (rc) return rc;
+  if (rows && (rc = attn_set_xo_rows(a, Xa_raw, who))) return rc;
+  attn_set_bwd(a, dzcat, attn, qt, Xa, nullptr, rows ? nullptr : efeat, dqt, dXa, dXo);
+  a.relu_xo = (relu_xo && dXo) ? 1 : 0;
+  return attn_launch(AttnFamily::BD, a, stream, true, who);
+}
 extern "C" int32_t dgppo_attn_fwd_xo(const dgppo_env_cfg* cfg, int32_t F, int32_t H, int32_t Kp, const float* qt, const float* Xa,
                                      const float* Xo_raw, const float* Wo, int32_t ldwo, const float* bo, const float* efeat,
                                      const float* emask, float* zcat, float* attn, int32_t G, void* stream) {
-  AttnArgs a{};
-  int32_t rc = attn_check(cfg, F, H, Kp, G, a);
-  if (rc) return rc;
-  if (G == 0) return 0;
-  DGPPO_REQUIRE(qt && Xa && Xo_raw && Wo && bo && efeat && emask && zcat, "attn_fwd_xo: NULL operand");
-  DGPPO_REQUIRE(ldwo >= 32, "attn_fwd_xo: ldwo=%d < 32", ldwo);
-  rc = attn_set_xo(a, Xo_raw, Wo, ldwo, bo, "attn_fwd_xo");
-  if (rc) return rc;
-  attn_set_fwd(a, qt, Xa, nullptr, efeat, emask, zcat, attn);
-  return attn_launch(AttnFamily::BD, a, stream, false, "attn_fwd_xo");
+  return attn_fwd_xo_any("attn_fwd_xo", false, cfg, F, H, Kp, qt, Xa, nullptr, Xo_raw, Wo, ldwo, bo, efeat, emask, zcat, attn, G, stream);
 }
 extern "C" int32_t dgppo_attn_bwd_xo(const dgppo_env_cfg* cfg, int32_t F, int32_t H, int32_t Kp, const float* dzcat,
                                      const float* attn, const float* qt, const float* Xa, const float* Xo_raw, const float* Wo,
                                      int32_t ldwo, const float* bo, const float* efeat, float* dqt, float* dXa, float* dXo,
                                      int32_t relu_xo, int32_t G, void* stream) {
-  AttnArgs a{};
-  int32_t rc = attn_check(cfg, F, H, Kp, G, a);
-  if (rc) return rc;
-  if (G == 0) return 0;
-  DGPPO_REQUIRE(dzcat && attn && qt && Xa && Xo_raw && Wo && bo && efeat && dqt, "attn_bwd_xo: NULL operand");
-  DGPPO_REQUIRE(ldwo >= 32, "attn_bwd_xo: ldwo=%d < 32", ldwo);
-  DGPPO_REQUIRE(!(dXo && !dXa), "attn_bwd_xo: dXo needs dXa");
-  rc = attn_set_xo(a, Xo_raw, Wo, ldwo, bo, "attn_bwd_xo");
-  if (rc) return rc;
-  attn_set_bwd(a, dzcat, attn, qt, Xa, nullptr, efeat, dqt, dXa, dXo);
-  a.relu_xo = (relu_xo && dXo) ? 1 : 0;
-  return attn_launch(AttnFamily::BD, a, stream, true, "attn_bwd_xo");
+  return attn_bwd_xo_any("attn_bwd_xo", false, cfg, F, H, Kp, dzcat, attn, qt, Xa, nullptr, Xo_raw, Wo, ldwo, bo, efeat, dqt, dXa, dXo,
+                         relu_xo, G, stream);
+}
+
+extern "C" int32_t dgppo_attn_xo_rows_supported(const dgppo_env_cfg* cfg, int32_t F, int32_t H, int32_t Kp) {
+  AttnArgs a{};
+  if (attn_check(cfg, F, H, Kp, 0, a)) return 0;
+  return attn_xo_rows_ok(*cfg, a.t, F, H, Kp) ? 1 : 0;
+}
+extern "C" int32_t dgppo_attn_fwd_xo_rows(const dgppo_env_cfg* cfg, int32_t F, int32_t H, int32_t Kp, const float* qt, const float* Xa,
+                                          const float* Xa_raw, const float* Xo_raw, const float* Wo, int32_t ldwo, const float* bo,
+                                          const float* emask, float* zcat, float* attn, int32_t G, void* stream) {
+  return attn_fwd_xo_any("attn_fwd_xo_rows", true, cfg, F, H, Kp, qt, Xa, Xa_raw, Xo_raw, Wo, ldwo, bo, nullptr, emask, zcat, attn, G, stream);
+}
+extern "C" int32_t dgppo_attn_bwd_xo_rows(const dgppo_env_cfg* cfg, int32_t F, int32_t H, int32_t Kp, const float* dzcat,
+                                          const float* attn, const float* qt, const float* Xa, const float* Xa_raw, const float* Xo_raw,
+                                          const float* Wo, int32_t ldwo, const float* bo, float* dqt, float* dXa, float* dXo,
+                                          int32_t relu_xo, int32_t G, void* stream) {
+  return attn_bwd_xo_any("attn_bwd_xo_rows", true, cfg, F, H, Kp, dzcat, attn, qt, Xa, Xa_raw, Xo_raw, Wo, ldwo, bo, nullptr, dqt, dXa, dXo,
+                         relu_xo, G, stream);
 }
 
 static bool attn_rows_ok(const dgppo_env_cfg& c, const Topo& t, int F, int H, int Kp) {
@@ -174,28 +215,46 @@
 }
 
 extern "C" int64_t dgppo_attn_xo_workspace_bytes(int32_t G) { return G < 0 ? 0 : (int64_t)G * ABD_DW_STRIDE * (int64_t)sizeof(float); }
+static int32_t attn_bwd_xo_dw_any(const char* who, bool rows, const dgppo_env_cfg* cfg, int32_t F, int32_t H, int32_t Kp,
+                                  const float* dzcat, const float* attn, const float* qt, const float* Xa, const float* Xa_raw,
+                                  const float* Xo_raw, const float* Wo, int32_t ldwo, const float* bo, const float* efeat, float* dqt,
+                                  float* dXa, float* dWo, int32_t lddwo, float* dbo, float* workspace, int64_t workspace_bytes,
+                                  int32_t G, void* stream) {
+  AttnArgs a{};
+  int32_t rc = attn_check(cfg, F, H, Kp, G, a);
+  if (rc) return rc;
+  if (rows) DGPPO_REQUIRE(attn_xo_rows_ok(*cfg, a.t, F, H, Kp), "%s: no such kernel for this configuration (ask dgppo_attn_xo_rows_supported)", who);
+  if (G == 0) return 0;
+  DGPPO_REQUIRE(dzcat && attn && qt && Xa && Xo_raw && Wo && bo && (rows || efeat) && dqt && dXa && dWo && dbo && workspace,
+                "%s: NULL operand", who);
+  DGPPO_REQUIRE(ldwo >= 32 && lddwo >= 32, "%s: ldwo=%d lddwo=%d < 32", who, ldwo, lddwo);
+  DGPPO_REQUIRE(workspace_bytes >= dgppo_attn_xo_workspace_bytes(G) && (reinterpret_cast<uintptr_t>(workspace) & 15) == 0,
+                "%s: workspace too small or not 16-byte aligned", who);
+  rc = attn_set_xo(a, Xo_raw, Wo, ldwo, bo, who);
+  if (rc) return rc;
+  if (rows && (rc = attn_set_xo_rows(a, Xa_raw, who))) return rc;
+  attn_set_bwd(a, dzcat, attn, qt, Xa, nullptr, rows ? nullptr : efeat, dqt, dXa, nullptr);
+  a.relu_xo = 1;
+  a.dwo_slab = workspace;
+  const bool launched = launch_attn_bd(a, (hipStream_t)stream, true);
+  DGPPO_REQUIRE(launched, "%s: dispatch failed", who);
+  launch_attn_xo_dw_reduce(workspace, G, dWo, lddwo, dbo, (hipStream_t)stream);
+  DGPPO_LAUNCH_CHECK();
+  return 0;
+}
 extern "C" int32_t dgppo_attn_bwd_xo_dw(const dgppo_env_cfg* cfg, int32_t F, int32_t H, int32_t Kp, const float* dzcat,
                                         const float* attn, const float* qt, const float* Xa, const float* Xo_raw, const float* Wo,
                                         int32_t ldwo, const float* bo, const float* efeat, float* dqt, float* dXa, float* dWo,
                                         int32_t lddwo, float* dbo, float* workspace, int64_t workspace_bytes, int32_t G,
                                         void* stream) {
-  AttnArgs a{};
-  int32_t rc = attn_check(cfg, F, H, Kp, G, a);
-  if (rc) return rc;
-  if (G == 0) return 0;
-  DGPPO_REQUIRE(dzcat && attn && qt && Xa && Xo_raw && Wo && bo && efeat && dqt && dXa && dWo && dbo && workspace,
-                "attn_bwd_xo_dw: NULL operand");
-  DGPPO_REQUIRE(ldwo >= 32 && lddwo >= 32, "attn_bwd_xo_dw: ldwo=%d lddwo=%d < 32", ldwo, lddwo);
-  DGPPO_REQUIRE(workspace_bytes >= dgppo_attn_xo_workspace_bytes(G) && (reinterpret_cast<uintptr_t>(workspace) & 15) == 0,
-                "attn_bwd_xo_dw: workspace too small or not 16-byte aligned");
-  rc = attn_set_xo(a, Xo_raw, Wo, ldwo, bo, "attn_bwd_xo_dw");
-  if (rc) return rc;
-  attn_set_bwd(a, dzcat, attn, qt, Xa, nullptr, efeat, dqt, dXa, nullptr);
-  a.relu_xo = 1;
-  a.dwo_slab = workspace;
-  const bool launched = launch_attn_bd(a, (hipStream_t)stream, true);
-  DGPPO_REQUIRE(launched, "attn_bwd_xo_dw: dispatch failed");
-  launch_attn_xo_dw_reduce(workspace, G, dWo, lddwo, dbo, (hipStream_t)stream);
-  DGPPO_LAUNCH_CHECK();
-  return 0;
-}
+  return attn_bwd_xo_dw_any("attn_bwd_xo_dw", false, cfg, F, H, Kp, dzcat, attn, qt, Xa, nullptr, Xo_raw, Wo, ldwo, bo, efeat, dqt, dXa,
+                            dWo, lddwo, dbo, workspace, workspace_bytes, G, stream);
+}
+extern "C" int32_t dgppo_attn_bwd_xo_dw_rows(const dgppo_env_cfg* cfg, int32_t F, int32_t H, int32_t Kp, const float* dzcat,
+                                             const float* attn, const float* qt, const float* Xa, const float* Xa_raw,
+                                             const float* Xo_raw, const float* Wo, int32_t ldwo, const float* bo, float* dqt, float* dXa,
+                                             float* dWo, int32_t lddwo, float* dbo, float* workspace, int64_t workspace_bytes,
+                                             int32_t G, void* stream) {
+  return attn_bwd_xo_dw_any("attn_bwd_xo_dw_rows", true, cfg, F, H, Kp, dzcat, attn, qt, Xa, Xa_raw, Xo_raw, Wo, ldwo, bo, nullptr, dqt,
+                            dXa, dWo, lddwo, dbo, workspace, workspace_bytes, G, stream);
+}
diff --git a/dgppo_amd/csrc/attn_bd.hip b/dgppo_amd/csrc/attn_bd.hip
--- a/dgppo_amd/csrc/attn_bd.hip
+++ b/dgppo_amd/csrc/attn_bd.hip
@@ -120,8 +120,17 @@
   return (j < NSH) ? slot_of(t, j, ic) : -1;
 }
 
-template <int PS, bool HITS, int AB, bool XOF>
+template <int PS, bool HITS>
+__device__ __forceinline__ float4 abd_sender4(const float* xa_raw, const float* xo_raw, const Topo& t, int NSH, int ic, int p, int sub) {
+  if (HITS && p == PS) return *reinterpret_cast<const float4*>(xo_raw + (t.ng + ic * 8 + sub) * ABD_KR);
+  int j = p * 8 + sub;
+  j = j < NSH ? j : NSH - 1;
+  return *reinterpret_cast<const float4*>(j < t.n ? xa_raw + j * ABD_KR : xo_raw + (j - t.n) * ABD_KR);
+}
+
+template <int PS, bool HITS, int AB, bool XOF, bool ROWS>
 __global__ void __launch_bounds__(128) attn_fwd_bd_kernel(AttnArgs a) {
+  static_assert(XOF || !ROWS, "the rows mode needs the raw rows of the other nodes");
   extern __shared__ float4 abd_sm[];
   using L = AbdLds<PS, HITS>;
   constexpr int F = 32, NSP = L::NSP, PC = L::PC, PL = L::PL, NPR = PS + (HITS ? 1 : 0), Wd = F + 4;
@@ -154,7 +163,8 @@
   const float* raw = XOF ? a.Xo_raw + (size_t)g * (Ns - n) * ABD_KR : nullptr;
   const int li_ = lane & 15, lq_ = lane >> 4;
   const float* mk = a.emask + (size_t)g * n * S;
-  const float4* ef4 = reinterpret_cast<const float4*>(a.efeat + (size_t)g * n * S * 4);
+  const float4* ef4 = ROWS ? nullptr : reinterpret_cast<const float4*>(a.efeat + (size_t)g * n * S * 4);
+  const float* xar = ROWS ? a.Xa_raw + (size_t)g * n * ABD_KR : nullptr;
   float* at = a.attn + (size_t)g * n * S * H;
 #pragma unroll
   for (int ab = 0; ab < AB; ++ab) {
@@ -162,6 +172,8 @@
     const bool live = i < n;
     const int ic = live ? i : n - 1;
     float4 vh[HITS ? 8 : 1], vq[4];
+    float4 xi = make_float4(0.f, 0.f, 0.f, 0.f);
+    if constexpr (ROWS) xi = *reinterpret_cast<const float4*>(xar + ic * ABD_KR);
     if constexpr (XOF) abd_xo_load<GT, HITS>(xo, a, raw, NSH - n, t.ng, ab * 64, n * 8, li_, lq_, ab == 0);
     if constexpr (HITS && !XOF) {
 #pragma unroll
@@ -187,14 +199,20 @@
       slot[p] = live ? sl : -1;
       const int sc = sl < 0 ? 0 : sl;
       mkv[p] = mk[ic * S + sc];
-      efv[p] = ef4[ic * S + sc];
+      if constexpr (ROWS) efv[p] = abd_sender4<PS, HITS>(xar, raw, t, NSH, ic, p, sub);
+      else efv[p] = ef4[ic * S + sc];
     }
     ASTAMP(1);
     int pin = 0;
 #pragma unroll
     for (int p = 0; p < NPR; ++p) pin |= __float_as_int(mkv[p]) | f4bits(efv[p]);
+    if constexpr (ROWS) pin |= f4bits(xi);
     if constexpr (XOF) pin |= abd_xo_bits<GT>(xo, HITS);
     const int pin0 = opaque_zero(pin);
+    if constexpr (ROWS) {
+#pragma unroll
+      for (int p = 0; p < NPR; ++p) efv[p] = edge_from_rows(t, slot[p] < 0 ? 0 : slot[p], xi, efv[p]);
+    }
     if (ab == 0) {
 #pragma unroll
       for (int p = 0; p < PS; ++p) {
@@ -323,15 +341,17 @@
   ASTAMP(6);
 }
 
-template <int PS, bool HITS, bool XOF>
+template <int PS, bool HITS, bool XOF, bool ROWS>
 struct AbdFwdRegs {
   float4 vs[PS], vq[4], vh[(HITS && !XOF) ? 8 : 1];
   AbdXoRegs<(PS * 8 + 15) / 16> xo;
   float mkv[PS + (HITS ? 1 : 0)];
   float4 efv[PS + (HITS ? 1 : 0)];
+  float4 xi[ROWS ? 1 : 0];
 };
-template <int PS, bool HITS, bool XOF>
+template <int PS, bool HITS, bool XOF, bool ROWS>
 __global__ void __launch_bounds__(128) attn_fwd_bdp_kernel(AttnArgs a) {
+  static_assert(XOF || !ROWS, "the rows mode needs the raw rows of the other nodes");
   extern __shared__ float4 abd_sm[];
   using L = AbdLds<PS, HITS>;
   constexpr int F = 32, NSP = L::NSP, PC = L::PC, PL = L::PL, NPR = PS + (HITS ? 1 : 0), Wd = F + 4, GT = (NSP + 15) / 16;
@@ -358,7 +378,7 @@
     slot[p] = live ? sl : -1;
     sc[p] = sl < 0 ? 0 : sl;
   }
-  using Regs = AbdFwdRegs<PS, HITS, XOF>;
+  using Regs = AbdFwdRegs<PS, HITS, XOF, ROWS>;
   auto load = [&](int gg, Regs& R) {
     const float4* Xa4 = reinterpret_cast<const float4*>(a.Xa + (size_t)gg * n * F);
     const float4* Xo4 = reinterpret_cast<const float4*>(a.Xo + (size_t)gg * (Ns - n) * F);
@@ -387,19 +407,35 @@
       R.vq[k] = qt4[(ri * H + rh) * 8 + sub];
     }
     const float* mk = a.emask + (size_t)gg * n * S;
-    const float4* ef4 = reinterpret_cast<const float4*>(a.efeat + (size_t)gg * n * S * 4);
-#pragma unroll
-    for (int p = 0; p < NPR; ++p) {
-      R.mkv[p] = mk[ic * S + sc[p]];
-      R.efv[p] = ef4[ic * S + sc[p]];
+    if constexpr (ROWS) {
+      const float* xar = a.Xa_raw + (size_t)gg * n * ABD_KR;
+      const float* raw = a.Xo_raw + (size_t)gg * (Ns - n) * ABD_KR;
+      R.xi[0] = *reinterpret_cast<const float4*>(xar + ic * ABD_KR);
+#pragma unroll
+      for (int p = 0; p < NPR; ++p) {
+        R.mkv[p] = mk[ic * S + sc[p]];
+        R.efv[p] = abd_sender4<PS, HITS>(xar, raw, t, NSH, ic, p, sub);
+      }
+    } else {
+      const float4* ef4 = reinterpret_cast<const float4*>(a.efeat + (size_t)gg * n * S * 4);
+#pragma unroll
+      for (int p = 0; p < NPR; ++p) {
+        R.mkv[p] = mk[ic * S + sc[p]];
+        R.efv[p] = ef4[ic * S + sc[p]];
+      }
     }
   };
   auto stage = [&](Regs& R) {
     int pin = 0;
 #pragma unroll
     for (int p = 0; p < NPR; ++p) pin |= __float_as_int(R.mkv[p]) | f4bits(R.efv[p]);
+    if constexpr (ROWS) pin |= f4bits(R.xi[0]);
     if constexpr (XOF) pin |= abd_xo_bits<GT>(R.xo, HITS);
     const int pin0 = opaque_zero(pin);
+    if constexpr (ROWS) {
+#pragma unroll
+      for (int p = 0; p < NPR; ++p) R.efv[p] = edge_from_rows(t, sc[p], R.xi[0], R.efv[p]);
+    }
 #pragma unroll
     for (int p = 0; p < PS; ++p) {
       float4 v = R.vs[p];
@@ -538,8 +574,9 @@
   }
 }
 
-template <int PS, bool HITS, int AB, bool XOF>
+template <int PS, bool HITS, int AB, bool XOF, bool ROWS>
 __global__ void __launch_bounds__(64) attn_bwd_bd_kernel(AttnArgs a) {
+  static_assert(XOF || !ROWS, "the rows mode needs the raw rows of the other nodes");
   extern __shared__ float4 abd_sm[];
   using L = AbdLds<PS, HITS>;
   constexpr int F = 32, NSP = L::NSP, PC = L::PC, PL = L::PL, PTL = L::PTL, NPR = PS + (HITS ? 1 : 0), Wd = F + 4;
@@ -591,7 +628,8 @@
     for (int ft = 0; ft < 2; ++ft) dxs[rt][ft] = f32x4g{0.f, 0.f, 0.f, 0.f};
   f32x4g dwacc[2] = {f32x4g{0.f, 0.f, 0.f, 0.f}, f32x4g{0.f, 0.f, 0.f, 0.f}};
   float rbg[NSP / 4];
-  const float4* ef4 = reinterpret_cast<const float4*>(a.efeat + (size_t)g * n * S * 4);
+  const float4* ef4 = ROWS ? nullptr : reinterpret_cast<const float4*>(a.efeat + (size_t)g * n * S * 4);
+  const float* xar = ROWS ? a.Xa_raw + (size_t)g * n * ABD_KR : nullptr;
   const float* at = a.attn + (size_t)g * n * S * H;
 #pragma unroll
   for (int ab = 0; ab < AB; ++ab) {
@@ -599,6 +637,8 @@
     const bool live = i < n;
     const int ic = live ? i : n - 1;
     float4 vh[HITS ? 8 : 1], vz[5];
+    float4 xi = make_float4(0.f, 0.f, 0.f, 0.f);
+    if constexpr (ROWS) xi = *reinterpret_cast<const float4*>(xar + ic * ABD_KR);
     if constexpr (XOF) abd_xo_load<GT, HITS>(xo, a, raw, NSH - n, t.ng, ab * 64, n * 8, li_, lq_, ab == 0);
     float rbh[HITS ? 16 : 1];
     if constexpr (XOF && HITS) {
@@ -645,7 +685,8 @@
       const int sl = abd_slot<PS, HITS>(t, NSH, ic, p, sub);
       slot[p] = live ? sl : -1;
       const int sc = sl < 0 ? 0 : sl;
-      efv[p] = ef4[ic * S + sc];
+      if constexpr (ROWS) efv[p] = abd_sender4<PS, HITS>(xar, raw, t, NSH, ic, p, sub);
+      else efv[p] = ef4[ic * S + sc];
 #pragma unroll
       for (int h = 0; h < 4; ++h) av[p][h] = at[(ic * S + sc) * H + (h < H ? h : H - 1)];
     }
@@ -697,7 +738,12 @@
         for (int s_ = 0; s_ < NSP / 4; ++s_) pin |= __float_as_int(rbg[s_]);
       }
     }
+    if constexpr (ROWS) pin |= f4bits(xi);
     const int pin0 = opaque_zero(pin);
+    if constexpr (ROWS) {
+#pragma unroll
+      for (int p = 0; p < NPR; ++p) efv[p] = edge_from_rows(t, slot[p] < 0 ? 0 : slot[p], xi, efv[p]);
+    }
     if (ab == 0) {
 #pragma unroll
       for (int p = 0; p < PS; ++p) {
@@ -940,31 +986,33 @@
   PS = (nsh + 7) / 8;
   return PS >= 1 && PS <= 4;
 }
-template <int PS, bool HITS, int AB, bool XOF>
+bool attn_bd_rows_ok(const dgppo_env_cfg& c) { return c.state_dim == 4 && !cfg_is_vmas(c) && !cfg_is_bicycle(c); }
+template <int PS, bool HITS, int AB, bool XOF, bool ROWS>
 static void launch_attn_bd_x(const AttnArgs& a, hipStream_t s, bool bwd) {
   using L = AbdLds<PS, HITS>;
-  if (bwd) { hipLaunchKernelGGL((attn_bwd_bd_kernel<PS, HITS, AB, XOF>), dim3(a.G), dim3(64), sizeof(float) * L::BWD, s, a); return; }
+  if (bwd) { hipLaunchKernelGGL((attn_bwd_bd_kernel<PS, HITS, AB, XOF, ROWS>), dim3(a.G), dim3(64), sizeof(float) * L::BWD, s, a); return; }
   if constexpr (AB == 1) {
     static thread_local int cap = 0;
     if (cap == 0) {
       int per_cu = 0, dev = 0, cus = 256;
-      if (hipOccupancyMaxActiveBlocksPerMultiprocessor(&per_cu, reinterpret_cast<const void*>(&attn_fwd_bdp_kernel<PS, HITS, XOF>), 128,
+      if (hipOccupancyMaxActiveBlocksPerMultiprocessor(&per_cu, reinterpret_cast<const void*>(&attn_fwd_bdp_kernel<PS, HITS, XOF, ROWS>), 128,
                                                        sizeof(float) * 2 * L::FWD) != hipSuccess || per_cu < 1) per_cu = 1;
       if (hipGetDevice(&dev) != hipSuccess || hipDeviceGetAttribute(&cus, hipDeviceAttributeMultiprocessorCount, dev) != hipSuccess ||
           cus < 1) cus = 256;
       cap = per_cu * cus;
     }
     if ((a.G + 1) / 2 > 2 * cap) {
-      hipLaunchKernelGGL((attn_fwd_bdp_kernel<PS, HITS, XOF>), dim3(cap), dim3(128), sizeof(float) * 2 * L::FWD, s, a);
+      hipLaunchKernelGGL((attn_fwd_bdp_kernel<PS, HITS, XOF, ROWS>), dim3(cap), dim3(128), sizeof(float) * 2 * L::FWD, s, a);
       return;
     }
   }
-  hipLaunchKernelGGL((attn_fwd_bd_kernel<PS, HITS, AB, XOF>), dim3((a.G + 1) / 2), dim3(128), sizeof(float) * 2 * L::FWD, s, a);
+  hipLaunchKernelGGL((attn_fwd_bd_kernel<PS, HITS, AB, XOF, ROWS>), dim3((a.G + 1) / 2), dim3(128), sizeof(float) * 2 * L::FWD, s, a);
 }
 template <int PS, bool HITS, int AB>
 static void launch_attn_bd_one(const AttnArgs& a, hipStream_t s, bool bwd) {
-  if (a.Xo_raw != nullptr) launch_attn_bd_x<PS, HITS, AB, true>(a, s, bwd);
-  else launch_attn_bd_x<PS, HITS, AB, false>(a, s, bwd);
+  if (a.Xo_raw != nullptr && a.Xa_raw != nullptr) launch_attn_bd_x<PS, HITS, AB, true, true>(a, s, bwd);
+  else if (a.Xo_raw != nullptr) launch_attn_bd_x<PS, HITS, AB, true, false>(a, s, bwd);
+  else launch_attn_bd_x<PS, HITS, AB, false, false>(a, s, bwd);
 }
 bool launch_attn_bd(const AttnArgs& a, hipStream_t s, bool bwd) {
   int PS = 0;
diff --git a/dgppo_amd/csrc/attn_slot8.hip b/dgppo_amd/csrc/attn_slot8.hip
--- a/dgppo_amd/csrc/attn_slot8.hip
+++ b/dgppo_amd/csrc/attn_slot8.hip
@@ -27,11 +27,6 @@
 #pragma unroll
   for (int j = 0; j < SJ; ++j) w[j] *= inv;
 }
-__device__ inline float4 slot8_edge(const Topo& t, int sl, float4 xi, float4 xs) {
-  const bool hit = t.lidar && sl >= t.n + t.gs;
-  return make_float4(__fsub_rn(xi.x, xs.x), __fsub_rn(xi.y, xs.y), hit ? 0.0f : __fsub_rn(xi.z, xs.z), hit ? 0.0f : __fsub_rn(xi.w, xs.w));
-}
-
 template <int H, int NPA, int SJ, bool ROWS>
 __global__ void __launch_bounds__(256) attn_fwd_slot8_kernel(AttnArgs a) {
   constexpr int F = 8, Wd = F + 4;
@@ -73,7 +68,7 @@
       const int nd = sender_node(t, i, sl);
       const float4* xp = reinterpret_cast<const float4*>((nd < n ? Xa : Xo) + (size_t)nd * F);
       x[j][0] = xp[0]; x[j][1] = xp[1];
-      if constexpr (ROWS) e[j] = slot8_edge(t, sl, xi, x[j][0]);
+      if constexpr (ROWS) e[j] = edge_from_rows(t, sl, xi, x[j][0]);
       else e[j] = reinterpret_cast<const float4*>(ef)[i * S + sl];
       m[j] = mk[i * S + sl];
     }
@@ -150,7 +145,7 @@
       const int nd = sender_node(t, i, sl);
       const float4* xp = reinterpret_cast<const float4*>((nd < n ? Xa : Xo) + (size_t)nd * F);
       x[j][0] = xp[0]; x[j][1] = xp[1];
-      if constexpr (ROWS) e[j] = slot8_edge(t, sl, xi, x[j][0]);
+      if constexpr (ROWS) e[j] = edge_from_rows(t, sl, xi, x[j][0]);
       else e[j] = reinterpret_cast<const float4*>(ef)[i * S + sl];
       if constexpr (RECOMP) {
         m[j] = mk[i * S + sl];
diff --git a/dgppo_amd/csrc/env_step.hip b/dgppo_amd/csrc/env_step.hip
--- a/dgppo_amd/csrc/env_step.hip
+++ b/dgppo_amd/csrc/env_step.hip
@@ -742,7 +742,7 @@
   DGPPO_REQUIRE(agent && goal && obst && hits && ray_cos && ray_sin, "env_act_step_feats: NULL state operand");
   DGPPO_REQUIRE(ms && action && next_agent && next_hits && reward && cost, "env_act_step_feats: NULL operand");
   DGPPO_REQUIRE(!sample || (eps && log_pi), "env_act_step_feats(sample): eps and log_pi must not be NULL");
-  DGPPO_REQUIRE(!Xa || (Xo && efeat && emask), "env_act_step_feats: Xa needs Xo, efeat and emask");
+  DGPPO_REQUIRE(!Xa || (Xo && emask), "env_act_step_feats: Xa needs Xo and emask");
   DGPPO_REQUIRE(!qt0 || (Mcat && cvec), "env_act_step_feats: qt0 needs Mcat and cvec");
   auto al16 = [](const void* p) { return (((uintptr_t)p) & 15) == 0; };
   DGPPO_REQUIRE(al16(agent) && al16(goal) && al16(obst) && al16(hits) && al16(next_agent) && al16(next_hits),
diff --git a/dgppo_amd/csrc/env_wave.hip b/dgppo_amd/csrc/env_wave.hip
--- a/dgppo_amd/csrc/env_wave.hip
+++ b/dgppo_amd/csrc/env_wave.hip
@@ -859,7 +859,7 @@
               e = make_float4(lx, ly, 0.0f, 0.0f);
               mask = lx * lx + ly * ly < a.thr2_lidar;
             }
-            reinterpret_cast<float4*>(f.efeat)[(size_t)b * NE + idx] = e;
+            if (f.efeat != nullptr) reinterpret_cast<float4*>(f.efeat)[(size_t)b * NE + idx] = e;
           }
           const unsigned long long bits = __builtin_amdgcn_ballot_w64(mask);
           const int i4 = base + 4 * lane;
diff --git a/dgppo_amd/csrc/graph_feats.hip b/dgppo_amd/csrc/graph_feats.hip
--- a/dgppo_amd/csrc/graph_feats.hip
+++ b/dgppo_amd/csrc/graph_feats.hip
@@ -148,7 +148,7 @@
             mask = dist_rn(__fsub_rn(xi[0], xo[0]), __fsub_rn(xi[1], xo[1])) < c.obs_mask_radius;
           }
         }
-        reinterpret_cast<float4*>(a.efeat)[(size_t)g * nE + idx] = f;
+        if (a.efeat != nullptr) reinterpret_cast<float4*>(a.efeat)[(size_t)g * nE + idx] = f;
         if (!a.vecM) a.emask[(size_t)g * nE + idx] = mask ? 1.0f : 0.0f;
       }
       if (a.vecM) {
@@ -193,7 +193,7 @@
   DGPPO_REFUSE_VMAS(cfg, "dgppo_graph_feats", "dgppo_vmas_graph_feats");
   DGPPO_REQUIRE(n_env >= 0 && n_time >= 0, "graph_feats: negative counts");
   if (n_env == 0 || n_time == 0) return 0;
-  DGPPO_REQUIRE(agent && goal && Xa && efeat && emask, "graph_feats: NULL operand");
+  DGPPO_REQUIRE(agent && goal && Xa && emask, "graph_feats: NULL operand");
   DGPPO_REQUIRE(Fp >= cfg->node_dim && Fp <= 32, "graph_feats: Fp must be in [node_dim, 32]");
   FeatArgs a;
   a.cfg = *cfg; a.t = make_topo(*cfg);
diff --git a/dgppo_amd/csrc/nn_attn.h b/dgppo_amd/csrc/nn_attn.h
--- a/dgppo_amd/csrc/nn_attn.h
+++ b/dgppo_amd/csrc/nn_attn.h
@@ -19,6 +19,11 @@
   return 0.0f;
 }
 
+__device__ inline float4 edge_from_rows(const Topo& t, int sl, float4 xi, float4 xs) {
+  const bool hit = t.lidar && sl >= t.n + t.gs;
+  return make_float4(__fsub_rn(xi.x, xs.x), __fsub_rn(xi.y, xs.y), hit ? 0.0f : __fsub_rn(xi.z, xs.z), hit ? 0.0f : __fsub_rn(xi.w, xs.w));
+}
+
 #define ABD_DW_STRIDE 320
 struct AttnArgs {
   Topo t;
@@ -37,6 +42,7 @@
   int relu_xo;
   int G;
   const float* Xo_raw; const float* Wo; const float* bo; int ldwo;
+  const float* Xa_raw;
   float* dwo_slab;
   int TI;
 };
@@ -89,6 +95,7 @@
 bool attn_slot8_rows_ok(const dgppo_env_cfg& c, const Topo& t, int F, int H);
 bool launch_attn_slot8(const AttnArgs& a, hipStream_t s, bool bwd);
 bool attn_bd_shape(const Topo& t, int F, int H, int& PS, bool& hits);
+bool attn_bd_rows_ok(const dgppo_env_cfg& c);
 bool launch_attn_bd(const AttnArgs& a, hipStream_t s, bool bwd);
 void launch_attn_xo_dw_reduce(const float* slab, int G, float* dWo, int lddwo, float* dbo, hipStream_t s);
 int32_t launch_attn_tiled(AttnArgs& a, hipStream_t s, bool bwd);
diff --git a/dgppo_amd/engine.py b/dgppo_amd/engine.py
--- a/dgppo_amd/engine.py
+++ b/dgppo_amd/engine.py
@@ -151,6 +151,7 @@
         self.HC = self.policy.carry_dim
         self.opt = {k: OptState(net.layout.size, device) for k, net in self.nets.items()}
         self.arena = nets.Arena(device)
+        self.efeat_needed = any(net.needs_efeat() for net in built.values())
         self.allreduce = allreduce
         self.world, self.rank = int(world), int(rank)
         assert self.world >= 1 and (allreduce is not None or self.world == 1), "world > 1 needs an allreduce"
@@ -226,7 +227,7 @@
             net.prepare()
 
     def _feats(self, tag, st: OE.State, n_env, n_time=1, slots=1, env_ids=None):
-        f = nets.GraphFeats(self.cfg, n_env * n_time, self.arena, tag)
+        f = nets.GraphFeats(self.cfg, n_env * n_time, self.arena, tag, efeat=self.efeat_needed)
         return f.compute_record(st.step, slots, st.env, env_ids, n_env, n_time)
 
     def _rollout_steps(self, ro: RolloutData, eps, B: int, stochastic: bool, start: int = 0):
diff --git a/dgppo_amd/nets.py b/dgppo_amd/nets.py
--- a/dgppo_amd/nets.py
+++ b/dgppo_amd/nets.py
@@ -95,19 +95,25 @@
 
 class GraphFeats:
 
-    def __init__(self, cfg: N.EnvCfg, G: int, arena: Arena, tag: str):
+    def __init__(self, cfg: N.EnvCfg, G: int, arena: Arena, tag: str, efeat: bool = True):
         self.cfg, self.G = cfg, G
         n, S = cfg.n_agents, cfg.fan_in
         self.n_other = cfg.num_nodes - 1 - n
         self.Fp = input_width(cfg)
         self.Xa = arena.get(f"{tag}.Xa0", G * n, self.Fp)
         self.Xo = arena.get(f"{tag}.Xo0", max(G * self.n_other, 1), self.Fp)[:G * self.n_other]
-        self.efeat = arena.get(f"{tag}.efeat", G * n, S, 4)
+        self.efeat = arena.get(f"{tag}.efeat", G * n, S, 4) if efeat else None
         self.emask = arena.get(f"{tag}.emask", G * n, S)
         self.edges_from_rows = False
 
+    def _need_efeat(self, who: str):
+        if self.efeat is None:
+            raise ValueError(f"{who}: these features were built without an efeat buffer, and this producer writes one")
+
     def compute(self, agent, agent_se, agent_st, goal, obst, hits, hits_se, hits_st, env_ids, n_env, n_time):
         assert n_env * n_time == self.G
+        if self.efeat is None and self.cfg.state_dim != 4:
+            raise ValueError("compute: only the kinds with a 4-float state can do without efeat")
         K.graph_feats(self.cfg, agent, agent_se, agent_st, goal, obst, hits, hits_se, hits_st, env_ids, n_env, n_time,
                       self.Xa, self.Xo if self.n_other > 0 else None, self.efeat, self.emask, self.Fp)
         self.edges_from_rows = self.cfg.state_dim == 4
@@ -128,6 +134,7 @@
         cfg, n = self.cfg, self.cfg.n_agents
         if cfg.is_vmas:
             raise ValueError("compute_sweep: VMASReverseTransport has no sweep entry point")
+        self._need_efeat("compute_sweep")
         K.graph_feats_sweep(cfg, step["agent"], n * cfg.state_dim, env["goal"], env.get("obst"), step.get("hits"),
                             n * cfg.top_k * 2, ray_cos, ray_sin, frame_ids, n_frames, agent_id, xs, ys, self.Xa,
                             self.Xo if self.n_other > 0 else None, self.efeat, self.emask, self.Fp, hits_out, frame_max)
@@ -138,6 +145,7 @@
         cfg, n = self.cfg, self.cfg.n_agents
         if cfg.is_vmas:
             raise ValueError("compute_action_sweep: VMASReverseTransport has no sweep entry point")
+        self._need_efeat("compute_action_sweep")
         K.graph_feats_action_sweep(cfg, step["agent"], n * cfg.state_dim, env["goal"], env.get("obst"), step.get("hits"),
                                    n * cfg.top_k * 2, frame_ids, n_frames, agent_id, us, vs, self.Xa,
                                    self.Xo if self.n_other > 0 else None, self.efeat, self.emask, self.Fp, frame_max)
@@ -147,6 +155,7 @@
     def compute_team_action_sweep(self, st, nst, a_pol, us, vs):
         if self.cfg.is_vmas:
             raise ValueError("compute_team_action_sweep: VMASReverseTransport has no sweep entry point")
+        self._need_efeat("compute_team_action_sweep")
         K.graph_feats_team_action_sweep(self.cfg, st.step["agent"], nst.step["agent"], st.env["goal"], st.env.get("obst"),
                                         nst.step.get("hits"), a_pol, us, vs, self.Xa, self.Xo if self.n_other > 0 else None,
                                         self.efeat, self.emask, self.Fp)
@@ -155,6 +164,7 @@
 
     def compute_vmas(self, agent, agent_se, agent_st, body, body_se, body_st, scene, env_ids, n_env, n_time):
         assert n_env * n_time == self.G
+        self._need_efeat("compute_vmas")
         K.vmas_graph_feats(self.cfg, agent, agent_se, agent_st, body, body_se, body_st, scene, env_ids, n_env, n_time,
                            self.Xa, self.efeat, self.emask, self.Fp)
         self.edges_from_rows = False
@@ -234,6 +244,22 @@
                     K.attn_xo_supported(self.cfg, fp1, H_HEADS, kp1))
         return getattr(self, key)
 
+    def _layer1_rows_ok(self) -> bool:
+        key = "_l1_rows_ok"
+        if not hasattr(self, key):
+            ok = self.lean_attn0 and self._xo_fusable(0)
+            if ok:
+                f1, fp1, d1, kp1 = self.dims[1]
+                ok = K.attn_xo_rows_supported(self.cfg, fp1, H_HEADS, kp1)
+            setattr(self, key, bool(ok))
+        return getattr(self, key)
+
+    def _xo_rows(self, l: int, feats: "GraphFeats") -> bool:
+        return l == 1 and feats.edges_from_rows and self._layer1_rows_ok()
+
+    def needs_efeat(self) -> bool:
+        return not (self.lean_attn0 and (self.gnn_layers == 1 or self._layer1_rows_ok()))
+
     def zero_grads(self):
         self.grads.zero_()
 
@@ -255,9 +281,14 @@
                 K.dense_fwd(Xa, self.pp(f"gnn{l}.Mcat"), self.pp(f"gnn{l}.cvec"), qt)
             zcat = A.get(f"{tag}.zcat{l}", R, kp)
             lean = l == 0 and self.lean_attn0 and feats.edges_from_rows
+            rows = xo_fused is not None and self._xo_rows(l, feats)
+            if not (lean or rows) and feats.efeat is None:
+                raise ValueError(f"Net.forward: layer {l} reads efeat, and these features were built without it")
             attn = A.get(f"{tag}.attn{l}", R, cfg.fan_in, H_HEADS) if train and not lean else None
             if lean:
                 K.attn_fwd_rows(cfg, fp, H_HEADS, kp, qt, Xa, Xo if Ro > 0 else None, feats.emask, zcat, None, G)
+            elif rows:
+                K.attn_fwd_xo_rows(cfg, fp, H_HEADS, kp, qt, Xa, feats.Xa, xo_fused[0], xo_fused[1], xo_fused[2], feats.emask, zcat, attn, G)
             elif xo_fused is not None:
                 K.attn_fwd_xo(cfg, fp, H_HEADS, kp, qt, Xa, xo_fused[0], xo_fused[1], xo_fused[2], feats.efeat, feats.emask, zcat, attn, G)
             else:
@@ -267,7 +298,7 @@
             Xa_n = A.get(f"{tag}.Xa{l + 1}", R, d)
             K.dense_fwd(zcat, self.pp(f"gnn{l}.Wout"), self.p(f"gnn{l}.bu"), Xa_n, act=1)
             act[f"Xa{l}"], act[f"Xo{l}"], act[f"qt{l}"], act[f"zcat{l}"], act[f"attn{l}"] = Xa, Xo, qt, zcat, attn
-            act[f"lean{l}"] = lean
+            act[f"lean{l}"], act[f"rows{l}"] = lean, rows
             if l < self.gnn_layers - 1 and Ro > 0:
                 if self._xo_fusable(l):
                     xo_fused = (Xo, self.pp(f"gnn{l}.Wout")[:fp], self.p(f"gnn{l}.bu"))
@@ -561,9 +592,16 @@
                                 act[f"Xo{l}"] if Ro > 0 else None, dqt, G)
             elif xf is not None and dXa_l is not None and not more_dXo:
                 ws = A.get(f"{tag}.xo_ws", K.attn_xo_workspace_floats(G), 1).view(-1)
-                K.attn_bwd_xo_dw(cfg, fp, H_HEADS, kp, dz, act[f"attn{l}"], act[f"qt{l}"], act[f"Xa{l}"], xf[0], xf[1], xf[2],
-                                 feats.efeat, dqt, dXa_l, self.pg(f"gnn{l - 1}.Wout")[:self.dims[l - 1][1]], self.g(f"gnn{l - 1}.bu"), ws, G)
+                if act.get(f"rows{l}"):
+                    K.attn_bwd_xo_dw_rows(cfg, fp, H_HEADS, kp, dz, act[f"attn{l}"], act[f"qt{l}"], act[f"Xa{l}"], feats.Xa, xf[0], xf[1],
+                                          xf[2], dqt, dXa_l, self.pg(f"gnn{l - 1}.Wout")[:self.dims[l - 1][1]], self.g(f"gnn{l - 1}.bu"), ws, G)
+                else:
+                    K.attn_bwd_xo_dw(cfg, fp, H_HEADS, kp, dz, act[f"attn{l}"], act[f"qt{l}"], act[f"Xa{l}"], xf[0], xf[1], xf[2],
+                                     feats.efeat, dqt, dXa_l, self.pg(f"gnn{l - 1}.Wout")[:self.dims[l - 1][1]], self.g(f"gnn{l - 1}.bu"), ws, G)
                 dXo_l = None
+            elif xf is not None and act.get(f"rows{l}"):
+                K.attn_bwd_xo_rows(cfg, fp, H_HEADS, kp, dz, act[f"attn{l}"], act[f"qt{l}"], act[f"Xa{l}"], feats.Xa, xf[0], xf[1], xf[2],
+                                   dqt, dXa_l, dXo_l, G, relu_xo=(dXo_l is not None and not more_dXo))
             elif xf is not None:
                 K.attn_bwd_xo(cfg, fp, H_HEADS, kp, dz, act[f"attn{l}"], act[f"qt{l}"], act[f"Xa{l}"], xf[0], xf[1], xf[2],
                               feats.efeat, dqt, dXa_l, dXo_l, G, relu_xo=(dXo_l is not None and not more_dXo))
diff --git a/dgppo_amd/ops_env.py b/dgppo_amd/ops_env.py
--- a/dgppo_amd/ops_env.py
+++ b/dgppo_amd/ops_env.py
@@ -277,7 +277,8 @@
         S = cfg.fan_in
         N.expect_shape(Xa, (B * n, Fp), "Xa")
         N.expect_shape(Xo, (B * (cfg.num_nodes - 1 - n), Fp), "Xo")
-        N.expect_shape(efeat, (B * n, S, 4), "efeat")
+        if efeat is not None:
+            N.expect_shape(efeat, (B * n, S, 4), "efeat")
         N.expect_shape(emask, (B * n, S), "emask")
     if qt0 is not None:
         N.expect_shape(Mcat, (Fp, H * Fp), "Mcat")
diff --git a/dgppo_amd/ops_nn.py b/dgppo_amd/ops_nn.py
--- a/dgppo_amd/ops_nn.py
+++ b/dgppo_amd/ops_nn.py
@@ -253,7 +253,8 @@
     N.expect_shape(Xa, (G * n, Fp), "Xa")
     if n_other > 0:
         N.expect_shape(Xo, (G * n_other, Fp), "Xo")
-    N.expect_shape(efeat, (G * n, S, 4), "efeat")
+    if efeat is not None:
+        N.expect_shape(efeat, (G * n, S, 4), "efeat")
     N.expect_shape(emask, (G * n, S), "emask")
     _check_strided("graph_feats", "agent", agent, agent_se, agent_st, (n, cfg.state_dim), env_ids, n_env, n_time)
     if hits is not None:
@@ -680,6 +681,60 @@
                                       _p(bo), _p(efeat), _p(dqt), _p(dXa), _wo_ptr(dWo), _wo_ld(dWo), _p(dbo), _p(workspace),
                                       C.c_int64(workspace.numel() * 4), G, N.stream_ptr())
     N.check(rc, "dgppo_attn_bwd_xo_dw")
+
+
+def attn_xo_rows_supported(cfg, F, H, Kp) -> bool:
+    return bool(N.lib().dgppo_attn_xo_rows_supported(C.byref(cfg), F, H, Kp))
+
+
+def _xo_rows_operands(cfg, G, Xa_raw, Xo_raw):
+    n = cfg.n_agents
+    N.expect_shape(Xa_raw, (G * n, 8), "Xa_raw")
+    N.expect_shape(Xo_raw, (G * (cfg.num_nodes - 1 - n), 8), "Xo_raw")
+
+
+def attn_fwd_xo_rows(cfg, F, H, Kp, qt, Xa, Xa_raw, Xo_raw, Wo, bo, emask, zcat, attn, G):
+    n, S = cfg.n_agents, cfg.fan_in
+    N.expect_shape(qt, (G * n, H * F), "qt")
+    N.expect_shape(Xa, (G * n, F), "Xa")
+    N.expect_shape(emask, (G * n, S), "emask")
+    N.expect_shape(zcat, (G * n, Kp), "zcat")
+    _xo_rows_operands(cfg, G, Xa_raw, Xo_raw)
+    N.expect_shape(bo, (32,), "bo")
+    if attn is not None:
+        N.expect_shape(attn, (G * n, S, H), "attn")
+    FLOPS[0] += 2.0 * G * n * H * S * (2 * F + 4) + 2.0 * G * (cfg.num_nodes - 1 - n) * 8 * 32 + 4.0 * G * n * S
+    rc = N.lib().dgppo_attn_fwd_xo_rows(C.byref(cfg), F, H, Kp, _p(qt), _p(Xa), _p(Xa_raw), _p(Xo_raw), _wo_ptr(Wo), _wo_ld(Wo),
+                                        _p(bo), _p(emask), _p(zcat), _p(attn), G, N.stream_ptr())
+    N.check(rc, "dgppo_attn_fwd_xo_rows")
+
+
+def attn_bwd_xo_rows(cfg, F, H, Kp, dzcat, attn, qt, Xa, Xa_raw, Xo_raw, Wo, bo, dqt, dXa, dXo, G, relu_xo: bool = False):
+    n = cfg.n_agents
+    N.expect_shape(dzcat, (G * n, Kp), "dzcat")
+    N.expect_shape(dqt, (G * n, H * F), "dqt")
+    _xo_rows_operands(cfg, G, Xa_raw, Xo_raw)
+    if dXa is not None:
+        N.expect_shape(dXa, (G * n, F), "dXa")
+    FLOPS[0] += 4.0 * G * n * H * cfg.fan_in * (2 * F + 4) + 2.0 * G * (cfg.num_nodes - 1 - n) * 8 * 32 + 4.0 * G * n * cfg.fan_in
+    rc = N.lib().dgppo_attn_bwd_xo_rows(C.byref(cfg), F, H, Kp, _p(dzcat), _p(attn), _p(qt), _p(Xa), _p(Xa_raw), _p(Xo_raw),
+                                        _wo_ptr(Wo), _wo_ld(Wo), _p(bo), _p(dqt), _p(dXa), _p(dXo), int(relu_xo), G,
+                                        N.stream_ptr())
+    N.check(rc, "dgppo_attn_bwd_xo_rows")
+
+
+def attn_bwd_xo_dw_rows(cfg, F, H, Kp, dzcat, attn, qt, Xa, Xa_raw, Xo_raw, Wo, bo, dqt, dXa, dWo, dbo, workspace, G):
+    n = cfg.n_agents
+    N.expect_shape(dzcat, (G * n, Kp), "dzcat")
+    N.expect_shape(dqt, (G * n, H * F), "dqt")
+    N.expect_shape(dXa, (G * n, F), "dXa")
+    _xo_rows_operands(cfg, G, Xa_raw, Xo_raw)
+    N.expect_shape(dbo, (32,), "dbo")
+    FLOPS[0] += 4.0 * G * n * H * cfg.fan_in * (2 * F + 4) + 4.0 * G * (cfg.num_nodes - 1 - n) * 8 * 32 + 4.0 * G * n * cfg.fan_in
+    rc = N.lib().dgppo_attn_bwd_xo_dw_rows(C.byref(cfg), F, H, Kp, _p(dzcat), _p(attn), _p(qt), _p(Xa), _p(Xa_raw), _p(Xo_raw),
+                                           _wo_ptr(Wo), _wo_ld(Wo), _p(bo), _p(dqt), _p(dXa), _wo_ptr(dWo), _wo_ld(dWo), _p(dbo),
+                                           _p(workspace), C.c_int64(workspace.numel() * 4), G, N.stream_ptr())
+    N.check(rc, "dgppo_attn_bwd_xo_dw_rows")
 
 
 def gnn_prep(Wq, bq, Wk, Wv, bv, We, Wu, Mcat, cvec, Wout, F, Fp, D, H, Kp):
diff --git a/include/dgppo_hip.h b/include/dgppo_hip.h
--- a/include/dgppo_hip.h
+++ b/include/dgppo_hip.h
@@ -257,6 +257,18 @@
                              const float* attn, const float* qt, const float* Xa, const float* Xo_raw, const float* Wo,
                              int32_t ldwo, const float* bo, const float* efeat, float* dqt, float* dXa, float* dWo,
                              int32_t lddwo, float* dbo, float* workspace, int64_t workspace_bytes, int32_t G, void* stream);
+int32_t dgppo_attn_xo_rows_supported(const dgppo_env_cfg* cfg, int32_t F, int32_t H, int32_t Kp);
+int32_t dgppo_attn_fwd_xo_rows(const dgppo_env_cfg* cfg, int32_t F, int32_t H, int32_t Kp, const float* qt, const float* Xa,
+                               const float* Xa_raw, const float* Xo_raw, const float* Wo, int32_t ldwo, const float* bo,
+                               const float* emask, float* zcat, float* attn, int32_t G, void* stream);
+int32_t dgppo_attn_bwd_xo_rows(const dgppo_env_cfg* cfg, int32_t F, int32_t H, int32_t Kp, const float* dzcat,
+                               const float* attn, const float* qt, const float* Xa, const float* Xa_raw, const float* Xo_raw,
+                               const float* Wo, int32_t ldwo, const float* bo, float* dqt, float* dXa, float* dXo,
+                               int32_t relu_xo, int32_t G, void* stream);
+int32_t dgppo_attn_bwd_xo_dw_rows(const dgppo_env_cfg* cfg, int32_t F, int32_t H, int32_t Kp, const float* dzcat,
+                                  const float* attn, const float* qt, const float* Xa, const float* Xa_raw, const float* Xo_raw,
+                                  const float* Wo, int32_t ldwo, const float* bo, float* dqt, float* dXa, float* dWo,
+                                  int32_t lddwo, float* dbo, float* workspace, int64_t workspace_bytes, int32_t G, void* stream);
 
 int32_t dgppo_gnn_prep(const float* Wq, const float* bq, const float* Wk, const float* Wv, const float* bv,
                        const float* We, const float* Wu, float* Mcat, float* cvec, float* Wout, int32_t F, int32_t Fp,
```

Measured after the change: 4.657 million (median of 6 runs). +1.3%, better.
